# alehdaghi/vq-vae-2-pytorch

Measured on AMD Instinct MI355X. Metric: images/sec VQ-VAE-2 256px train step, higher is better.
Workload: dtype f32; 1 GPU; configs[1]: 256x256 FFHQ-shaped synthetic, default two-level VQ-VAE-2, batch 32/GPU; global_batch=32, image=256, n_embed=512, parallelism=dp1

## Files before the change

include/vq2.h:

```cpp
#ifndef VQ2_H
#define VQ2_H

#include <stddef.h>
#include <stdint.h>

#ifdef __cplusplus
extern "C" {
#endif

#define VQ2_OK 0
#define VQ2_ERR_INVALID 1
#define VQ2_ERR_UNSUPPORTED 2
#define VQ2_ERR_WORKSPACE 3
#define VQ2_ERR_LAUNCH 4

typedef void *vq2_stream_t;

#define VQ2_API_VERSION 6

int vq2_version(void);
const char *vq2_last_error(void);

int vq2_prof_enable(int level);
int vq2_prof_report(char *buf, size_t cap);

typedef struct vq2_conv_desc {
    int32_t N, H, W, Ci;
    int32_t Co;
    int32_t KH, KW, stride, pad;
    int32_t transposed;
    int32_t ldx, ldy;
    int32_t Cir, Cor;
} vq2_conv_desc;

#define VQ2_RELU_IN 1
#define VQ2_RELU_OUT 2

#define VQ2_PACK_FWD 0
#define VQ2_PACK_DGRAD 1
int vq2_pack_weight(const vq2_conv_desc *d, int which, const float *w, float *packed, vq2_stream_t stream);

typedef struct vq2_pack_job {
    const float *w;
    float *packed;
    int64_t offset;
    int64_t numel;
    int32_t Or, Ir, Op, Ip, KH, KW, mode, reserved;
} vq2_pack_job;
int vq2_pack_job_init(const vq2_conv_desc *d, int which, const float *w, float *packed, vq2_pack_job *job);
int vq2_pack_weights_batched(const vq2_pack_job *jobs_dev, int32_t njobs, int64_t total, vq2_stream_t stream);

int vq2_conv_fwd(const vq2_conv_desc *d, int flags, const float *x, const float *wp, const float *bias,
                 const float *residual, int32_t ldres, float *y, vq2_stream_t stream);

int vq2_resblock_supported(int32_t C, int32_t Cm);
int vq2_resblock_fwd(int32_t N, int32_t H, int32_t W, int32_t C, int32_t Cm, int flags, const float *x, int32_t ldx,
                     const float *w1p, const float *b1, const float *w2p, const float *b2, float *r, int32_t ldr,
                     float *y, int32_t ldy, vq2_stream_t stream);

size_t vq2_resblock_w2_workspace_bytes(int32_t N, int32_t H, int32_t W, int32_t C, int32_t Cm);
int vq2_resblock_bwd_data(int32_t N, int32_t H, int32_t W, int32_t C, int32_t Cm, const float *g, int32_t ldg,
                          const float *r, int32_t ldr, const float *x, int32_t ldx, const float *w2d, const float *w1d,
                          float *dh, int32_t lddh, float *dx, int32_t lddx, void *w2_ws, vq2_stream_t stream);

int vq2_conv_dgrad(const vq2_conv_desc *d, const float *dy, const float *wp, const float *mask, int32_t ldmask,
                   const float *residual, int32_t ldres, float *dx, int32_t lddx, vq2_stream_t stream);
#define VQ2_MASK_AFTER_RESIDUAL 4
int vq2_conv_dgrad_ex(const vq2_conv_desc *d, int flags, const float *dy, const float *wp, const float *mask,
                      int32_t ldmask, const float *residual, int32_t ldres, float *dx, int32_t lddx,
                      vq2_stream_t stream);

size_t vq2_conv_wgrad_workspace_bytes(const vq2_conv_desc *d);
int vq2_conv_wgrad(const vq2_conv_desc *d, int flags, const float *x, const float *dy, float *dw, float *db, void *ws,
                   size_t ws_bytes, vq2_stream_t stream);

typedef struct vq2_wgrad_job {
    const float *ws;
    float *dw;
    const float *bias_ws;
    float *db;
    int64_t unit_offset;
    int32_t O, I, Or, Ir, taps, S, n_units_w, n_units_b;
    int32_t swapped;
    int32_t bias_splits;
} vq2_wgrad_job;
int vq2_conv_wgrad_partial(const vq2_conv_desc *d, int flags, const float *x, const float *dy, float *db, void *ws,
                           size_t ws_bytes, vq2_stream_t stream);
int vq2_wgrad_job_init(const vq2_conv_desc *d, const void *ws, float *dw, float *db, vq2_wgrad_job *job);
int vq2_wgrad_reduce_batched(const vq2_wgrad_job *jobs_dev, int32_t njobs, int64_t total_units, vq2_stream_t stream);
int vq2_resblock_w2_job_init(int32_t N, int32_t H, int32_t W, int32_t C, int32_t Cm, const void *ws, float *dw, float *db,
                             vq2_wgrad_job *job);

size_t vq2_colsum_workspace_bytes(int64_t rows, int32_t C);
int vq2_colsum(const float *dy, int64_t rows, int32_t C, int32_t ld, float *db, void *ws, size_t ws_bytes,
               vq2_stream_t stream);

int vq2_nchw_to_nhwc(const float *src, float *dst, int32_t N, int32_t C, int32_t H, int32_t W, int32_t ld,
                     vq2_stream_t stream);
int vq2_nhwc_to_nchw(const float *src, float *dst, int32_t N, int32_t C, int32_t H, int32_t W, int32_t ld,
                     vq2_stream_t stream);

#define VQ2_U8_HWC 0
#define VQ2_U8_CHW 1
int vq2_u8_to_nhwc4(const uint8_t *src, int layout, int32_t N, int32_t C, int32_t Hs, int32_t Ws, int32_t y0,
                    int32_t x0, int32_t H, int32_t W, const float *lut ,
                    float *dst , vq2_stream_t stream);
int vq2_nhwc_to_u8(const float *src, int32_t ld, int32_t N, int32_t C, int32_t H, int32_t W,
                   const float *inv_s , const float *mean , uint8_t *dst, int layout,
                   int32_t Hc, int32_t Wc, int64_t pitch, int32_t cols, int32_t pad, int64_t image_pitch, vq2_stream_t stream);
int vq2_relu_bwd(const float *dy, int32_t lddy, const float *y, int32_t ldy, float *g, int32_t ldg, int64_t pixels,
                 int32_t C, vq2_stream_t stream);
int vq2_slice_copy(const float *src, int32_t lds, float *dst, int32_t ldd, int64_t pixels, int32_t C,
                   int accumulate, vq2_stream_t stream);

int vq2_vq_prepare(const float *embed, float *embedT, float *enorm, int32_t D, int32_t K, vq2_stream_t stream);
size_t vq2_vq_fwd_workspace_floats(int64_t M, int32_t D, int32_t K);
int vq2_vq_fwd(const float *x, int32_t ldx, const float *embed, const float *embedT, const float *enorm, int64_t M,
               int32_t D, int32_t K, int64_t *idx, float *out, int32_t ldo, float *ws, vq2_stream_t stream);
size_t vq2_vq_stats_workspace_bytes(int64_t M, int32_t D, int32_t K);
int vq2_vq_stats(const float *x, int32_t ldx, const int64_t *idx, int64_t M, int32_t D, int32_t K, float *counts,
                 float *sumsT, void *ws, size_t ws_bytes, vq2_stream_t stream);
int vq2_vq_loss(const float *loss_partial, int64_t M, int32_t D, float *diff, vq2_stream_t stream);
int vq2_vq_bwd(const float *g_out, int32_t ldg, const float *g_diff, const float *x, int32_t ldx,
               const int64_t *idx, const float *embedT, int64_t M, int32_t D, int32_t K, float *dx, int32_t lddx,
               vq2_stream_t stream);
int vq2_vq_ema_update(float *embed, float *cluster_size, float *embed_avg, const float *counts, const float *sumsT,
                      int32_t D, int32_t K, double decay, double eps, float *scratch ,
                      vq2_stream_t stream);
int vq2_vq_ema_update_prepare(float *embed, float *cluster_size, float *embed_avg, const float *counts,
                              const float *sumsT, int32_t D, int32_t K, double decay, double eps, float *scratch,
                              float *embedT, float *enorm, vq2_stream_t stream);
int vq2_vq_gather(const int64_t *idx, const float *embedT, int64_t M, int32_t D, int32_t K, float *out, int32_t ldo,
                  vq2_stream_t stream);

int vq2_instnorm_stats(const float *x, int32_t ldx, int32_t N, int64_t HW, int32_t C, double eps, float *mean,
                       float *rstd, vq2_stream_t stream);
int vq2_adain_fwd(const float *x, int32_t ldx, const float *mean, const float *rstd, const float *h, int32_t N,
                  int64_t HW, int32_t C, int flags, float *y, int32_t ldy, vq2_stream_t stream);
int vq2_adain_bwd(const float *dy, int32_t lddy, const float *y, int32_t ldy, const float *x, int32_t ldx,
                  const float *mean, const float *rstd, const float *h, int32_t N, int64_t HW, int32_t C, float *dh,
                  float *dx, int32_t lddx, vq2_stream_t stream);

size_t vq2_mse_workspace_bytes(int64_t numel);
int vq2_mse_fwd_bwd(const float *a, const float *b, int64_t numel, int64_t denom, const float *gscale, float *loss,
                    float *grad, void *ws, size_t ws_bytes, vq2_stream_t stream);
int vq2_stage1_loss(const float *a, const float *b, int64_t numel, int64_t denom, const float *latent, float weight,
                    float *recon, float *total, float *grad, void *ws, size_t ws_bytes, vq2_stream_t stream);
int vq2_adam_step(float *p, const float *g, float *m, float *v, int64_t n, double lr, double beta1, double beta2,
                  double eps, int32_t step, double grad_scale, vq2_stream_t stream);
int vq2_axpby(const float *a, const float *b, float alpha, float *dst, int64_t n, vq2_stream_t stream);
int vq2_scale(const float *src, const float *scalar, float alpha, float *dst, int64_t n, vq2_stream_t stream);

size_t vq2_sse_workspace_bytes(int32_t N, int32_t H, int32_t W, int32_t ld);
int vq2_sse_per_image(const float *a, const float *b, int32_t N, int32_t H, int32_t W, int32_t ld, float *sse, void *ws,
                      size_t ws_bytes, vq2_stream_t stream);
int vq2_index_hist(const int64_t *idx, int64_t M, int32_t K, int64_t *counts, int32_t *flag, vq2_stream_t stream);
int vq2_eval_accumulate(const float *sse, int32_t N, int64_t elems_per_image, const float *diff, double *acc,
                        vq2_stream_t stream);

#define VQ2_COMM_ID_BYTES 128
int vq2_comm_unique_id(void *id);
int vq2_comm_init(const void *id, int32_t rank, int32_t world);
int vq2_comm_world(void);
int vq2_comm_rank(void);
int vq2_comm_allreduce_sum(float *buf, int64_t count, vq2_stream_t stream);
int vq2_comm_broadcast(float *buf, int64_t count, int32_t root, vq2_stream_t stream);
int vq2_comm_destroy(void);

int vq2_debug_mfma_peak(float *scratch, int32_t blocks, int32_t iters, vq2_stream_t stream);
int vq2_debug_mfma_peak16(float *scratch, int32_t blocks, int32_t iters, vq2_stream_t stream);

#ifdef __cplusplus
}
#endif
#endif
```

vq-vae-2-pytorch_amd/_lib.py:

```python
import ctypes as C
import os

_HERE = os.path.dirname(os.path.abspath(__file__))
LIB_PATH = os.environ.get("VQ2_LIB") or os.path.join(_HERE, "libvq2.so")

c_f32p = C.c_void_p
c_stream = C.c_void_p


class ConvDesc(C.Structure):
    _fields_ = [(n, C.c_int32) for n in
                ("N", "H", "W", "Ci", "Co", "KH", "KW", "stride", "pad", "transposed", "ldx", "ldy", "Cir", "Cor")]


class PackJob(C.Structure):
    _fields_ = [("w", C.c_void_p), ("packed", C.c_void_p), ("offset", C.c_int64), ("numel", C.c_int64)] + \
               [(n, C.c_int32) for n in ("Or", "Ir", "Op", "Ip", "KH", "KW", "mode", "reserved")]


class WgradJob(C.Structure):
    _fields_ = [("ws", C.c_void_p), ("dw", C.c_void_p), ("bias_ws", C.c_void_p), ("db", C.c_void_p),
                ("unit_offset", C.c_int64)] + \
               [(n, C.c_int32) for n in ("O", "I", "Or", "Ir", "taps", "S", "n_units_w", "n_units_b", "swapped", "bias_splits")]


def _load():
    if not os.path.exists(LIB_PATH):
        raise ImportError(
            f"{LIB_PATH} not found: build it with `python -c 'import __graft_entry__ as g; g.build()'` "
            "(vq-vae-2-pytorch_amd/csrc/build.sh).  There is no CPU or eager fallback for this path.")
    import torch
    lib = C.CDLL(LIB_PATH)
    P, I32, I64, SZ, F, D = C.c_void_p, C.c_int32, C.c_int64, C.c_size_t, C.c_float, C.c_double
    DP = C.POINTER(ConvDesc)
    sig = {
        "vq2_version": (C.c_int, []),
        "vq2_last_error": (C.c_char_p, []),
        "vq2_prof_enable": (C.c_int, [C.c_int]),
        "vq2_prof_report": (C.c_int, [C.c_char_p, SZ]),
        "vq2_pack_weight": (C.c_int, [DP, C.c_int, P, P, P]),
        "vq2_pack_job_init": (C.c_int, [DP, C.c_int, P, P, C.POINTER(PackJob)]),
        "vq2_pack_weights_batched": (C.c_int, [P, I32, I64, P]),
        "vq2_conv_fwd": (C.c_int, [DP, C.c_int, P, P, P, P, I32, P, P]),
        "vq2_conv_dgrad": (C.c_int, [DP, P, P, P, I32, P, I32, P, I32, P]),
        "vq2_conv_dgrad_ex": (C.c_int, [DP, C.c_int, P, P, P, I32, P, I32, P, I32, P]),
        "vq2_conv_wgrad_workspace_bytes": (SZ, [DP]),
        "vq2_conv_wgrad": (C.c_int, [DP, C.c_int, P, P, P, P, P, SZ, P]),
        "vq2_conv_wgrad_partial": (C.c_int, [DP, C.c_int, P, P, P, P, SZ, P]),
        "vq2_wgrad_job_init": (C.c_int, [DP, P, P, P, C.POINTER(WgradJob)]),
        "vq2_wgrad_reduce_batched": (C.c_int, [P, I32, I64, P]),
        "vq2_colsum_workspace_bytes": (SZ, [I64, I32]),
        "vq2_colsum": (C.c_int, [P, I64, I32, I32, P, P, SZ, P]),
        "vq2_nchw_to_nhwc": (C.c_int, [P, P, I32, I32, I32, I32, I32, P]),
        "vq2_nhwc_to_nchw": (C.c_int, [P, P, I32, I32, I32, I32, I32, P]),
        "vq2_u8_to_nhwc4": (C.c_int, [P, C.c_int, I32, I32, I32, I32, I32, I32, I32, I32, P, P, P]),
        "vq2_nhwc_to_u8": (C.c_int, [P, I32, I32, I32, I32, I32, C.POINTER(F), C.POINTER(F), P, C.c_int, I32, I32, I64, I32,
                                     I32, I64, P]),
        "vq2_sse_workspace_bytes": (SZ, [I32, I32, I32, I32]),
        "vq2_sse_per_image": (C.c_int, [P, P, I32, I32, I32, I32, P, P, SZ, P]),
        "vq2_index_hist": (C.c_int, [P, I64, I32, P, P, P]),
        "vq2_eval_accumulate": (C.c_int, [P, I32, I64, P, P, P]),
        "vq2_relu_bwd": (C.c_int, [P, I32, P, I32, P, I32, I64, I32, P]),
        "vq2_resblock_supported": (C.c_int, [I32, I32]),
        "vq2_resblock_bwd_data": (C.c_int, [I32, I32, I32, I32, I32, P, I32, P, I32, P, I32, P, P, P, I32, P, I32, P, P]),
        "vq2_resblock_w2_workspace_bytes": (SZ, [I32, I32, I32, I32, I32]),
        "vq2_resblock_w2_job_init": (C.c_int, [I32, I32, I32, I32, I32, P, P, P, C.POINTER(WgradJob)]),
        "vq2_resblock_fwd": (C.c_int, [I32, I32, I32, I32, I32, C.c_int, P, I32, P, P, P, P, P, I32, P, I32, P]),
        "vq2_slice_copy": (C.c_int, [P, I32, P, I32, I64, I32, C.c_int, P]),
        "vq2_vq_prepare": (C.c_int, [P, P, P, I32, I32, P]),
        "vq2_vq_fwd_workspace_floats": (SZ, [I64, I32, I32]),
        "vq2_vq_fwd": (C.c_int, [P, I32, P, P, P, I64, I32, I32, P, P, I32, P, P]),
        "vq2_vq_stats_workspace_bytes": (SZ, [I64, I32, I32]),
        "vq2_vq_stats": (C.c_int, [P, I32, P, I64, I32, I32, P, P, P, SZ, P]),
        "vq2_vq_loss": (C.c_int, [P, I64, I32, P, P]),
        "vq2_vq_bwd": (C.c_int, [P, I32, P, P, I32, P, P, I64, I32, I32, P, I32, P]),
        "vq2_vq_ema_update": (C.c_int, [P, P, P, P, P, I32, I32, D, D, P, P]),
        "vq2_vq_ema_update_prepare": (C.c_int, [P, P, P, P, P, I32, I32, D, D, P, P, P, P]),
        "vq2_vq_gather": (C.c_int, [P, P, I64, I32, I32, P, I32, P]),
        "vq2_instnorm_stats": (C.c_int, [P, I32, I32, I64, I32, D, P, P, P]),
        "vq2_adain_fwd": (C.c_int, [P, I32, P, P, P, I32, I64, I32, C.c_int, P, I32, P]),
        "vq2_adain_bwd": (C.c_int, [P, I32, P, I32, P, I32, P, P, P, I32, I64, I32, P, P, I32, P]),
        "vq2_mse_workspace_bytes": (SZ, [I64]),
        "vq2_mse_fwd_bwd": (C.c_int, [P, P, I64, I64, P, P, P, P, SZ, P]),
        "vq2_stage1_loss": (C.c_int, [P, P, I64, I64, P, F, P, P, P, P, SZ, P]),
        "vq2_adam_step": (C.c_int, [P, P, P, P, I64, D, D, D, D, I32, D, P]),
        "vq2_axpby": (C.c_int, [P, P, F, P, I64, P]),
        "vq2_scale": (C.c_int, [P, P, F, P, I64, P]),
        "vq2_comm_unique_id": (C.c_int, [P]),
        "vq2_comm_init": (C.c_int, [P, I32, I32]),
        "vq2_comm_world": (C.c_int, []),
        "vq2_comm_rank": (C.c_int, []),
        "vq2_comm_allreduce_sum": (C.c_int, [P, I64, P]),
        "vq2_comm_broadcast": (C.c_int, [P, I64, I32, P]),
        "vq2_comm_destroy": (C.c_int, []),
        "vq2_debug_mfma_peak": (C.c_int, [P, I32, I32, P]),
        "vq2_debug_mfma_peak16": (C.c_int, [P, I32, I32, P]),
    }
    for name, (res, args) in sig.items():
        fn = getattr(lib, name)
        fn.restype = res
        fn.argtypes = args
    return lib, tuple(sig.keys())


def _header_api_version():
    import re
    hdr = os.path.join(os.path.dirname(_HERE), "include", "vq2.h")
    with open(hdr) as f:
        return int(re.search(r"#define\s+VQ2_API_VERSION\s+(\d+)", f.read()).group(1))


lib, EXPORTS = _load()
API_VERSION = _header_api_version()
if lib.vq2_version() != API_VERSION:
    raise ImportError(f"{LIB_PATH} implements ABI revision {lib.vq2_version()} but include/vq2.h declares "
                      f"{API_VERSION}: rebuild the library (vq-vae-2-pytorch_amd/csrc/build.sh)")


def check(code, what=""):
    if code != 0:
        msg = lib.vq2_last_error().decode(errors="replace")
        raise RuntimeError(f"libvq2 {what} failed (code {code}): {msg}")
```

vq-vae-2-pytorch_amd/csrc/vq2_conv.hip:

```cpp
#include "vq2_conv.h"

namespace vq2 {


template <int WAVES_M, int WAVES_N, int MT, int NT, int BK>
__global__ __launch_bounds__(256, (MT * NT == 4) ? (BK == 16 ? 3 : 2) : 1) void conv_gemm_kernel(const ConvGemmParams P) {
    constexpr int LDK = BK + 4;
    constexpr int BM = WAVES_M * MT * 32;
    constexpr int BN = WAVES_N * NT * 32;
    constexpr int KQ = BK / 4;
    constexpr int RPP = 256 / KQ;
    constexpr int A_LD = BM / RPP;
    constexpr int B_LD = (BN + RPP - 1) / RPP;
    static_assert(BM % RPP == 0 && (BN % RPP == 0 || BN < RPP), "tile vs staging shape");
    static_assert(WAVES_M * WAVES_N == 4, "4 waves per workgroup");
    extern __shared__ __attribute__((aligned(16))) float smem[];
    float *As = smem;
    float *Bs = smem + 2 * BM * LDK;

    const int tid = threadIdx.x;
    const int lane = tid & 63;
    const int wave = tid >> 6;
    const int wm = wave / WAVES_N;
    const int wn = wave % WAVES_N;
    const int ntiles = (P.Co + BN - 1) / BN;
    const int mtiles = (P.M + BM - 1) / BM;
    const int vid = xcd_remap(blockIdx.x, gridDim.x);
    const int n0 = (vid % ntiles) * BN;
    const int m0 = ((vid / ntiles) % mtiles) * BM;
    const int phase = vid / (ntiles * mtiles);

    int pad_h = P.pad_h, pad_w = P.pad_w, oh = 0, ow = 0, os = 1;
    const float *wp = P.w;
    if (P.phases == 4) {
        const int ph = phase >> 1, pw = phase & 1;
        pad_h = 1 - ph; pad_w = 1 - pw; oh = ph; ow = pw; os = 2;
        wp += (size_t)phase * P.Co * P.K;
    }

    const int lrow = tid / KQ;
    const int lk = (tid % KQ) * 4;
    int a_pix[A_LD], a_h[A_LD], a_w[A_LD];
    const int HoWo = P.Ho * P.Wo;
#pragma unroll
    for (int j = 0; j < A_LD; ++j) {
        const int m = m0 + lrow + RPP * j;
        if (m < P.M) {
            const int n = m / HoWo;
            const int r = m - n * HoWo;
            const int ho = r / P.Wo;
            const int wo = r - ho * P.Wo;
            a_h[j] = ho * P.stride - pad_h;
            a_w[j] = wo * P.stride - pad_w;
            a_pix[j] = (n * P.H + a_h[j]) * P.W + a_w[j];
        } else {
            a_h[j] = -(1 << 24); a_w[j] = 0; a_pix[j] = 0;
        }
    }
    int kglob = lk;
    int ci, kh, kw;
    {
        const int tap = kglob / P.Ci;
        ci = kglob - tap * P.Ci;
        kh = tap / P.KW;
        kw = tap - kh * P.KW;
    }

    float4 ra0[A_LD], rb0[B_LD];
    auto load_chunk = [&](float4 (&ra)[A_LD], float4 (&rb)[B_LD]) {
        const bool kv = kglob < P.K;
#pragma unroll
        for (int j = 0; j < A_LD; ++j) {
            const bool v = kv && (unsigned)(a_h[j] + kh) < (unsigned)P.H && (unsigned)(a_w[j] + kw) < (unsigned)P.W;
            float4 val = make_float4(0.f, 0.f, 0.f, 0.f);
            if (v) val = *reinterpret_cast<const float4 *>(P.x + (size_t)(a_pix[j] + kh * P.W + kw) * P.ldx + ci);
            ra[j] = val;
        }
#pragma unroll
        for (int j = 0; j < B_LD; ++j) {
            const int co = n0 + lrow + RPP * j;
            float4 val = make_float4(0.f, 0.f, 0.f, 0.f);
            if (kv && co < P.Co && lrow + RPP * j < BN) val = *reinterpret_cast<const float4 *>(wp + (size_t)co * P.K + kglob);
            rb[j] = val;
        }
    };
    auto advance_k = [&]() {
        kglob += BK;
        ci += BK;
        while (ci >= P.Ci) {
            ci -= P.Ci;
            if (++kw == P.KW) { kw = 0; ++kh; }
        }
    };
    auto store_chunk = [&](int buf, const float4 (&ra)[A_LD], const float4 (&rb)[B_LD]) {
        float *a = As + buf * BM * LDK;
        float *b = Bs + buf * BN * LDK;
#pragma unroll
        for (int j = 0; j < A_LD; ++j)
            *reinterpret_cast<float4 *>(a + (lrow + RPP * j) * LDK + lk) = P.relu_in ? relu4(ra[j]) : ra[j];
#pragma unroll
        for (int j = 0; j < B_LD; ++j)
            if (BN % RPP == 0 || lrow + RPP * j < BN) *reinterpret_cast<float4 *>(b + (lrow + RPP * j) * LDK + lk) = rb[j];
    };

    f32x16 acc[MT][NT];
#pragma unroll
    for (int i = 0; i < MT; ++i)
#pragma unroll
        for (int j = 0; j < NT; ++j)
#pragma unroll
            for (int r = 0; r < 16; ++r) acc[i][j][r] = 0.f;

    const int frag_row = lane & 31;
    const int frag_k = 4 * (lane >> 5);
    auto compute = [&](int buf) {
        const float *a = As + buf * BM * LDK + (wm * MT * 32 + frag_row) * LDK + frag_k;
        const float *b = Bs + buf * BN * LDK + (wn * NT * 32 + frag_row) * LDK + frag_k;
        float4 fa[2][MT], fb[2][NT];
#pragma unroll
        for (int i = 0; i < MT; ++i) fa[0][i] = *reinterpret_cast<const float4 *>(a + i * 32 * LDK);
#pragma unroll
        for (int j = 0; j < NT; ++j) fb[0][j] = *reinterpret_cast<const float4 *>(b + j * 32 * LDK);
#pragma unroll
        for (int k8 = 0; k8 < BK / 8; ++k8) {
            const int cur = k8 & 1, nxt = cur ^ 1;
            if (k8 + 1 < BK / 8) {
#pragma unroll
                for (int i = 0; i < MT; ++i) fa[nxt][i] = *reinterpret_cast<const float4 *>(a + i * 32 * LDK + (k8 + 1) * 8);
#pragma unroll
                for (int j = 0; j < NT; ++j) fb[nxt][j] = *reinterpret_cast<const float4 *>(b + j * 32 * LDK + (k8 + 1) * 8);
            }
#define VQ2_MFMA_STEP(C)                                                                                         \
    _Pragma("unroll") for (int i = 0; i < MT; ++i) _Pragma("unroll") for (int j = 0; j < NT; ++j)                 \
        acc[i][j] = __builtin_amdgcn_mfma_f32_32x32x2f32(fa[cur][i].C, fb[cur][j].C, acc[i][j], 0, 0, 0);
            __builtin_amdgcn_s_setprio(1);
            VQ2_MFMA_STEP(x) VQ2_MFMA_STEP(y) VQ2_MFMA_STEP(z) VQ2_MFMA_STEP(w)
            __builtin_amdgcn_s_setprio(0);
#undef VQ2_MFMA_STEP
        }
    };

    const int nchunks = (P.K + BK - 1) / BK;
    load_chunk(ra0, rb0);
    store_chunk(0, ra0, rb0);
    __syncthreads();
    for (int c = 0; c < nchunks; ++c) {
        const int buf = c & 1;
        if (c + 1 < nchunks) {
            advance_k();
            load_chunk(ra0, rb0);
        }
        compute(buf);
        if (c + 1 < nchunks) store_chunk(buf ^ 1, ra0, rb0);
        __syncthreads();
    }

    const float *__restrict__ maskp = P.mask;
    const float *__restrict__ resp = P.res;
    float *__restrict__ yp = P.y;
    const int colq = lane & 31;
    const int rowq = 4 * (lane >> 5);
#pragma unroll
    for (int j = 0; j < NT; ++j) {
        const int co = n0 + (wn * NT + j) * 32 + colq;
        const bool cv = co < P.Co;
        const float bv = (P.bias && co < P.nbias) ? P.bias[co] : 0.f;
#pragma unroll
        for (int i = 0; i < MT; ++i) {
            const int mb = m0 + (wm * MT + i) * 32 + rowq;
#pragma unroll
            for (int rb = 0; rb < 16; rb += 8) {
                int pix[8];
                bool ok[8];
#pragma unroll
                for (int q = 0; q < 8; ++q) {
                    const int r = rb + q;
                    const int m = mb + (r & 3) + 8 * (r >> 2);
                    ok[q] = cv && m < P.M;
                    if (os == 1) {
                        pix[q] = m;
                    } else {
                        const int n = m / HoWo;
                        const int rr = m - n * HoWo;
                        const int ho = rr / P.Wo;
                        const int wo = rr - ho * P.Wo;
                        pix[q] = (n * P.Hy + (ho * os + oh)) * P.Wy + (wo * os + ow);
                    }
                }
                float mk[8], rs[8];
                if (maskp) {
#pragma unroll
                    for (int q = 0; q < 8; ++q) mk[q] = ok[q] ? maskp[(size_t)pix[q] * P.ldm + co] : 0.f;
                }
                if (resp) {
#pragma unroll
                    for (int q = 0; q < 8; ++q) rs[q] = ok[q] ? resp[(size_t)pix[q] * P.ldr + co] : 0.f;
                }
#pragma unroll
                for (int q = 0; q < 8; ++q) {
                    float v = acc[i][j][rb + q] + bv;
                    if (maskp && !P.mask_after) v = (mk[q] > 0.f) ? v : 0.f;
                    if (resp) v += rs[q];
                    if (maskp && P.mask_after) v = (mk[q] > 0.f) ? v : 0.f;
                    v = relu_floor(v, P.relu_out ? 0 : (int)0x80000000);
                    if (ok[q]) yp[(size_t)pix[q] * P.ldy + co] = v;
                }
            }
        }
    }
}



template <int WAVES_M, int WAVES_N, int MT, int NT, int BK, bool PIPE, bool RELU_IN, bool OCC4 = false, bool UNI = OCC4, bool TAPIN = false>
__global__ __launch_bounds__(256, OCC4 ? 4 : ((MT * NT == 4) ? (BK == 16 ? 3 : 2) : 1)) void conv_gemm_fast_kernel(const ConvGemmParams P) {
    constexpr int LDK = BK + 4;
    constexpr int BM = WAVES_M * MT * 32;
    constexpr int BN = WAVES_N * NT * 32;
    constexpr int KQ = BK / 4;
    constexpr int RPP = 256 / KQ;
    constexpr int A_LD = BM / RPP;
    constexpr int B_LD = (BN + RPP - 1) / RPP;
    static_assert(BM % RPP == 0 && (BN % RPP == 0 || BN < RPP), "tile vs staging shape");
    extern __shared__ __attribute__((aligned(16))) float smem[];
    float *As = smem;
    float *Bs = smem + 2 * BM * LDK;
    int *tap_off = reinterpret_cast<int *>(smem + 2 * (BM + BN) * LDK);
    int *tap_khw = tap_off + 32;

    const int tid = threadIdx.x, lane = tid & 63, wave = tid >> 6;
    const int wm = wave / WAVES_N, wn = wave % WAVES_N;
    const int ntiles = (P.Co + BN - 1) / BN;
    const int mtiles = (P.M + BM - 1) / BM;
    const int vid = xcd_remap(blockIdx.x, gridDim.x);
    const int n0 = (vid % ntiles) * BN;
    const int m0 = ((vid / ntiles) % mtiles) * BM;
    const int phase = vid / (ntiles * mtiles);
    int pad_h = P.pad_h, pad_w = P.pad_w, oh = 0, ow = 0, os = 1;
    const float *wp = P.w;
    if (P.phases == 4) {
        const int ph = phase >> 1, pw = phase & 1;
        pad_h = 1 - ph; pad_w = 1 - pw; oh = ph; ow = pw; os = 2;
        wp += (size_t)phase * P.Co * P.K;
    }
    const int ntaps = P.KH * P.KW;
    if (!OCC4 && tid < ntaps) {
        const int kh = tid / P.KW, kw = tid - kh * P.KW;
        tap_off[tid] = (kh * P.W + kw) * P.ldx * 4;
        tap_khw[tid] = kh | (kw << 8);
    }
    const __amdgpu_buffer_rsrc_t rx =
        __builtin_amdgcn_make_buffer_rsrc(const_cast<float *>(P.x), 0, P.N * P.H * P.W * P.ldx * 4, RSRC_FLAGS);
    const __amdgpu_buffer_rsrc_t rw =
        __builtin_amdgcn_make_buffer_rsrc(const_cast<float *>(wp), 0, P.Co * P.K * 4, RSRC_FLAGS);

    const int lrow = tid / KQ;
    const int lk = (tid % KQ) * 4;
    const int HoWo = P.Ho * P.Wo;
    int a_base[A_LD];
    unsigned a_vw[A_LD];
#pragma unroll
    for (int j = 0; j < A_LD; ++j) {
        const int m = m0 + lrow + RPP * j;
        a_base[j] = 0; a_vw[j] = 0;
        if (m < P.M) {
            const int n = m / HoWo;
            const int r = m - n * HoWo;
            const int ho = r / P.Wo;
            const int wo = r - ho * P.Wo;
            const int hb = ho * P.stride - pad_h, wb = wo * P.stride - pad_w;
            a_base[j] = ((n * P.H + hb) * P.W + wb) * P.ldx * 4;
            unsigned hm = 0, wmk = 0;
            for (int q = 0; q < P.KH; ++q) hm |= ((unsigned)(hb + q) < (unsigned)P.H ? 1u : 0u) << q;
            for (int q = 0; q < P.KW; ++q) wmk |= ((unsigned)(wb + q) < (unsigned)P.W ? 1u : 0u) << q;
            for (int q = 0; q < P.KH; ++q)
                if ((hm >> q) & 1u) a_vw[j] |= wmk << (q * P.KW);
        }
    }
    int b_base[B_LD];
#pragma unroll
    for (int j = 0; j < B_LD; ++j) {
        const int co = n0 + lrow + RPP * j;
        b_base[j] = (co < P.Co && lrow + RPP * j < BN) ? co * P.K * 4 : -1;
    }
    int kglob = lk;
    int tap = kglob / P.Ci;
    int ci = kglob - tap * P.Ci;
    const int tstep = BK / P.Ci, cstep = BK - tstep * P.Ci;
    int u_tap = 0, u_kh = 0, u_kw = 0, u_cb = 0;
    bool b_ok[B_LD];
#pragma unroll
    for (int j = 0; j < B_LD; ++j) b_ok[j] = b_base[j] >= 0;
    int a_pen[A_LD];
    auto refresh_pen = [&]() {
#pragma unroll
        for (int j = 0; j < A_LD; ++j) a_pen[j] = ((a_vw[j] >> u_tap) & 1u) ? 0 : (int)0x80000000;
    };
    if (UNI) {
#pragma unroll
        for (int j = 0; j < A_LD; ++j) a_base[j] += lk * 4;
#pragma unroll
        for (int j = 0; j < B_LD; ++j) b_base[j] = b_ok[j] ? b_base[j] + lk * 4 : (int)0x80000000;
        refresh_pen();
    }
    __syncthreads();

    u32x4 ra[A_LD], rb[B_LD];
    int off_a[A_LD], off_b[B_LD];
    const bool k_aligned = (P.K % BK) == 0;
    auto prep_offsets = [&]() {
        if constexpr (UNI) {
            const int koff_s = ((u_kh * P.W + u_kw) * P.ldx + u_cb) * 4;
            const int kb_s = (u_tap * P.Ci + u_cb) * 4;
#pragma unroll
            for (int j = 0; j < A_LD; ++j) off_a[j] = a_base[j] + koff_s + a_pen[j];
#pragma unroll
            for (int j = 0; j < B_LD; ++j) off_b[j] = b_base[j] + kb_s;
            return;
        }
        const bool kv = k_aligned || tap < ntaps;
        const int tsel = kv ? tap : 0;
        const int koff = tap_off[tsel] + ci * 4;
#pragma unroll
        for (int j = 0; j < A_LD; ++j) {
            const bool v = kv && ((a_vw[j] >> tsel) & 1u) != 0u;
            off_a[j] = v ? a_base[j] + koff : OOB;
        }
#pragma unroll
        for (int j = 0; j < B_LD; ++j) off_b[j] = (kv && b_base[j] >= 0) ? b_base[j] + kglob * 4 : OOB;
    };
    auto issue_loads = [&]() {
#pragma unroll
        for (int j = 0; j < A_LD; ++j) ra[j] = __builtin_amdgcn_raw_buffer_load_b128(rx, off_a[j], 0, 0);
#pragma unroll
        for (int j = 0; j < B_LD; ++j) rb[j] = __builtin_amdgcn_raw_buffer_load_b128(rw, off_b[j], 0, 0);
    };
    auto load_chunk = [&]() { prep_offsets(); issue_loads(); };
    auto advance_k = [&]() {
        if constexpr (UNI) {
            if constexpr (TAPIN) {
                u_cb += BK;
                if ((u_cb & 31) == 0) {
                    u_cb -= 32;
                    ++u_tap;
                    if (++u_kw == P.KW) { u_kw = 0; ++u_kh; }
                    if (u_tap == ntaps) { u_tap = 0; u_kh = 0; u_kw = 0; u_cb += 32; }
                    refresh_pen();
                }
                return;
            }
            u_cb += BK;
            if (u_cb >= P.Ci) {
                u_cb = 0; ++u_tap;
                if (++u_kw == P.KW) { u_kw = 0; ++u_kh; }
                refresh_pen();
            }
            return;
        }
        kglob += BK;
        ci += cstep;
        tap += tstep;
        if (ci >= P.Ci) { ci -= P.Ci; ++tap; }
    };
    auto store_chunk = [&](int buf) {
        float *a = As + buf * BM * LDK;
        float *b = Bs + buf * BN * LDK;
#pragma unroll
        for (int j = 0; j < A_LD; ++j) {
            const float4 v = as_f4(ra[j]);
            *reinterpret_cast<float4 *>(a + (lrow + RPP * j) * LDK + lk) = RELU_IN ? relu4(v) : v;
        }
#pragma unroll
        for (int j = 0; j < B_LD; ++j)
            if (BN % RPP == 0 || lrow + RPP * j < BN) *reinterpret_cast<float4 *>(b + (lrow + RPP * j) * LDK + lk) = as_f4(rb[j]);
    };

    f32x16 acc[MT][NT];
#pragma unroll
    for (int i = 0; i < MT; ++i)
#pragma unroll
        for (int j = 0; j < NT; ++j)
#pragma unroll
            for (int r = 0; r < 16; ++r) acc[i][j][r] = 0.f;

    const int frag_row = lane & 31;
    const int frag_k = 4 * (lane >> 5);
    auto compute = [&](int buf, bool prep_next) {
        const float *a = As + buf * BM * LDK + (wm * MT * 32 + frag_row) * LDK + frag_k;
        const float *b = Bs + buf * BN * LDK + (wn * NT * 32 + frag_row) * LDK + frag_k;
        float4 fa[2][MT], fb[2][NT];
#pragma unroll
        for (int i = 0; i < MT; ++i) fa[0][i] = *reinterpret_cast<const float4 *>(a + i * 32 * LDK);
#pragma unroll
        for (int j = 0; j < NT; ++j) fb[0][j] = *reinterpret_cast<const float4 *>(b + j * 32 * LDK);
#pragma unroll
        for (int k8 = 0; k8 < BK / 8; ++k8) {
            const int cur = k8 & 1, nxt = cur ^ 1;
            if (k8 + 1 < BK / 8) {
#pragma unroll
                for (int i = 0; i < MT; ++i) fa[nxt][i] = *reinterpret_cast<const float4 *>(a + i * 32 * LDK + (k8 + 1) * 8);
#pragma unroll
                for (int j = 0; j < NT; ++j) fb[nxt][j] = *reinterpret_cast<const float4 *>(b + j * 32 * LDK + (k8 + 1) * 8);
            }
#define VQ2_MFMA_STEP(C)                                                                                         \
    _Pragma("unroll") for (int i = 0; i < MT; ++i) _Pragma("unroll") for (int j = 0; j < NT; ++j)                 \
        acc[i][j] = __builtin_amdgcn_mfma_f32_32x32x2f32(fa[cur][i].C, fb[cur][j].C, acc[i][j], 0, 0, 0);
            VQ2_MFMA_STEP(x) VQ2_MFMA_STEP(y) VQ2_MFMA_STEP(z) VQ2_MFMA_STEP(w)
#undef VQ2_MFMA_STEP
            if (PIPE && k8 == 0 && prep_next) { advance_k(); prep_offsets(); }
        }
    };

    const int nchunks = (P.K + BK - 1) / BK;
    load_chunk();
    store_chunk(0);
    __syncthreads();
    if constexpr (PIPE) {
        if (nchunks > 1) { advance_k(); prep_offsets(); }
        for (int c = 0; c < nchunks; ++c) {
            const int buf = c & 1;
            if (c + 1 < nchunks) issue_loads();
            compute(buf, c + 2 < nchunks);
            if (c + 1 < nchunks) store_chunk(buf ^ 1);
            __syncthreads();
        }
    } else {
        for (int c = 0; c < nchunks; ++c) {
            const int buf = c & 1;
            if (c + 1 < nchunks) {
                advance_k();
                load_chunk();
            }
            compute(buf, false);
            if (c + 1 < nchunks) store_chunk(buf ^ 1);
            __syncthreads();
        }
    }

    const int ybytes = P.N * P.Hy * P.Wy * 4;
    const __amdgpu_buffer_rsrc_t ry = __builtin_amdgcn_make_buffer_rsrc(P.y, 0, ybytes * P.ldy, RSRC_FLAGS);
    const __amdgpu_buffer_rsrc_t rmk =
        __builtin_amdgcn_make_buffer_rsrc(const_cast<float *>(P.mask ? P.mask : P.y), 0, P.mask ? ybytes * P.ldm : 0, RSRC_FLAGS);
    const __amdgpu_buffer_rsrc_t rrs =
        __builtin_amdgcn_make_buffer_rsrc(const_cast<float *>(P.res ? P.res : P.y), 0, P.res ? ybytes * P.ldr : 0, RSRC_FLAGS);
    const bool has_mask = P.mask != nullptr, has_res = P.res != nullptr;
    const bool mask_first = has_mask && !P.mask_after, mask_last = has_mask && P.mask_after;
    const int colq = lane & 31;
    const int rowq = 4 * (lane >> 5);
    const int ldy4 = P.ldy * 4, ldm4 = P.ldm * 4, ldr4 = P.ldr * 4;
#pragma unroll
    for (int i = 0; i < MT; ++i) {
        const int mt0 = m0 + (wm * MT + i) * 32;
        int pix_lane;
        {
            const int m = mt0 + colq;
            if (os == 1) {
                pix_lane = m;
            } else {
                const int n = m / HoWo;
                const int rr = m - n * HoWo;
                const int ho = rr / P.Wo;
                const int wo = rr - ho * P.Wo;
                pix_lane = (n * P.Hy + (ho * 2 + oh)) * P.Wy + (wo * 2 + ow);
            }
            if (m >= P.M) pix_lane = -1;
        }
#pragma unroll
        for (int j = 0; j < NT; ++j) {
            const int co = n0 + (wn * NT + j) * 32 + colq;
            const bool cv = co < P.Co;
            const float bv = (P.bias && co < P.nbias) ? P.bias[co] : 0.f;
            const int co4 = co * 4;
#pragma unroll
            for (int rb8 = 0; rb8 < 16; rb8 += 8) {
                int pix[8];
                float mk[8], rs[8];
#pragma unroll
                for (int q = 0; q < 8; ++q) {
                    const int r = rb8 + q;
                    const int rr = rowq + (r & 3) + 8 * (r >> 2);
                    pix[q] = (os == 1) ? ((mt0 + rr < P.M) ? mt0 + rr : -1) : __shfl(pix_lane, rr, 64);
                    if (!cv) pix[q] = -1;
                }
                if (has_mask) {
#pragma unroll
                    for (int q = 0; q < 8; ++q)
                        mk[q] = __uint_as_float(__builtin_amdgcn_raw_buffer_load_b32(rmk, pix[q] >= 0 ? pix[q] * ldm4 + co4 : OOB, 0, 0));
                }
                if (has_res) {
#pragma unroll
                    for (int q = 0; q < 8; ++q)
                        rs[q] = __uint_as_float(__builtin_amdgcn_raw_buffer_load_b32(rrs, pix[q] >= 0 ? pix[q] * ldr4 + co4 : OOB, 0, 0));
                }
#pragma unroll
                for (int q = 0; q < 8; ++q) {
                    float v = acc[i][j][rb8 + q] + bv;
                    if (mask_first) v = (mk[q] > 0.f) ? v : 0.f;
                    if (has_res) v += rs[q];
                    if (mask_last) v = (mk[q] > 0.f) ? v : 0.f;
                    v = relu_floor(v, P.relu_out ? 0 : (int)0x80000000);
                    __builtin_amdgcn_raw_buffer_store_b32(__float_as_uint(v), ry, pix[q] >= 0 ? pix[q] * ldy4 + co4 : OOB, 0, 0);
                }
            }
        }
    }
}

template <int WAVES_M, int WAVES_N, int MT, int NT, int BK, bool OCC4 = false>
static int launch_conv_gemm_fast(const ConvGemmParams &P, hipStream_t s) {
    constexpr int BM = WAVES_M * MT * 32, BN = WAVES_N * NT * 32;
    const size_t lds = (size_t)2 * (BM + BN) * (BK + 4) * sizeof(float) + (OCC4 ? 0 : 64 * sizeof(int));
    const unsigned nwg = ((P.M + BM - 1) / BM) * ((P.Co + BN - 1) / BN) * P.phases;
    const long gib = 1L << 30;
    const bool small = (long)P.N * P.H * P.W * P.ldx * 4 < gib && (long)P.Co * P.K * P.phases * 4 < gib;
    const bool uni = small && (OCC4 || (P.Ci % BK == 0 && P.K % BK == 0));
    const bool tap_inner = uni && P.KH * P.KW > 1 && P.Ci > 32 && P.Ci % 32 == 0;
    auto kern = P.relu_in ? (uni ? (tap_inner ? conv_gemm_fast_kernel<WAVES_M, WAVES_N, MT, NT, BK, true, true, OCC4, true, true>
                                              : conv_gemm_fast_kernel<WAVES_M, WAVES_N, MT, NT, BK, true, true, OCC4, true, false>)
                                 : conv_gemm_fast_kernel<WAVES_M, WAVES_N, MT, NT, BK, true, true, OCC4, OCC4>)
                          : (uni ? (tap_inner ? conv_gemm_fast_kernel<WAVES_M, WAVES_N, MT, NT, BK, true, false, OCC4, true, true>
                                              : conv_gemm_fast_kernel<WAVES_M, WAVES_N, MT, NT, BK, true, false, OCC4, true, false>)
                                 : conv_gemm_fast_kernel<WAVES_M, WAVES_N, MT, NT, BK, true, false, OCC4, OCC4>);
    allow_big_lds(kern, lds);
    dim3 grid(nwg);
    const char *name = "conv_gemm";
    if (prof_enabled())
        name = prof_label("conv_gemm<%dx%dx%d>|M=%d,N=%d,K=%d,k%d,s%d,ph%d,%s", BM, BN, BK, P.M, P.Co, P.K, P.KH, P.stride,
                          P.phases, tap_inner ? "tap" : uni ? "uni" : "var");
    ProfScope prof(name, P.flops, P.bytes, s, BM == 128 && BN == 128);
    hipLaunchKernelGGL(kern, grid, dim3(256), lds, s, P);
    return check_launch("conv_gemm_fast_kernel");
}

template <int WAVES_M, int WAVES_N, int MT, int NT, int BK>
static int launch_conv_gemm(const ConvGemmParams &P, hipStream_t s) {
    constexpr int BM = WAVES_M * MT * 32, BN = WAVES_N * NT * 32;
    const size_t lds = (size_t)2 * (BM + BN) * (BK + 4) * sizeof(float);
    auto kern = conv_gemm_kernel<WAVES_M, WAVES_N, MT, NT, BK>;
    allow_big_lds(kern, lds);
    dim3 grid(((P.M + BM - 1) / BM) * ((P.Co + BN - 1) / BN) * P.phases);
    const char *name = "conv_gemm";
    if (prof_enabled())
        name = prof_label("conv_gemm<%dx%dx%d>|M=%d,N=%d,K=%d,k%d,s%d,ph%d,gen", BM, BN, BK, P.M, P.Co, P.K, P.KH, P.stride,
                          P.phases);
    ProfScope prof(name, P.flops, P.bytes, s, BM == 128 && BN == 128 && BK == 32);
    hipLaunchKernelGGL(kern, grid, dim3(256), lds, s, P);
    return check_launch("conv_gemm_kernel");
}

namespace sp {
constexpr int TH = 8, TW = 16, PW = TW + 2, NPATCH = (TH + 2) * PW;
constexpr int CS = 16, LDK = CS + 4;
constexpr int A_F4 = NPATCH * CS / 4;
constexpr int A_FLOATS = NPATCH * LDK;
constexpr int B_ROWS = 4 * 64;
constexpr int B_FLOATS = B_ROWS * LDK;
constexpr size_t LDS_BYTES = (size_t)2 * (A_FLOATS + B_FLOATS) * sizeof(float);
constexpr int SOOB = 0x7F000000;
}

template <bool RELU_IN>
__global__ __launch_bounds__(256, 2) void subpixel_conv_kernel(const ConvGemmParams P) {
    using namespace sp;
    constexpr int A_LD = (A_F4 + 255) / 256;
    extern __shared__ __attribute__((aligned(16))) float smem[];
    float *As = smem;
    float *Bs = smem + 2 * A_FLOATS;
    const int tid = threadIdx.x, lane = tid & 63, wq = tid >> 6;
    const int l31 = lane & 31, fk = 4 * (lane >> 5), rowq = 4 * (lane >> 5);
    const int ncg = P.Co / 64;
    const int tiles_x = (P.W + TW - 1) / TW, tiles_y = (P.H + TH - 1) / TH;
    const int tiles = tiles_x * tiles_y;
    const int vid = xcd_remap(blockIdx.x, gridDim.x);
    const int cg = vid % ncg;
    const int tv = vid / ncg;
    const int n = tv / tiles;
    const int t = tv - n * tiles;
    const int tyi = t / tiles_x;
    const int y0 = tyi * TH, x0 = (t - tyi * tiles_x) * TW;
    const __amdgpu_buffer_rsrc_t rx =
        __builtin_amdgcn_make_buffer_rsrc(const_cast<float *>(P.x), 0, P.N * P.H * P.W * P.ldx * 4, RSRC_FLAGS);
    const __amdgpu_buffer_rsrc_t rw =
        __builtin_amdgcn_make_buffer_rsrc(const_cast<float *>(P.w), 0, 4 * P.Co * P.K * 4, RSRC_FLAGS);

    int a_off[A_LD], b_off[4];
#pragma unroll
    for (int j = 0; j < A_LD; ++j) {
        const int f = tid + 256 * j;
        a_off[j] = SOOB;
        if (f < A_F4) {
            const int pp = f >> 2;
            const int pr = pp / PW, pc = pp - pr * PW;
            const int gy = y0 - 1 + pr, gx = x0 - 1 + pc;
            if ((unsigned)gy < (unsigned)P.H && (unsigned)gx < (unsigned)P.W)
                a_off[j] = ((n * P.H + gy) * P.W + gx) * P.ldx * 4 + (f & 3) * 16;
        }
    }
#pragma unroll
    for (int j = 0; j < 4; ++j) {
        const int row = (tid >> 2) + 64 * j;
        b_off[j] = ((cg * 64 + (row & 63)) * P.K + (row >> 6) * P.Ci) * 4 + (tid & 3) * 16;
    }
    const int st_off = (tid >> 2) * LDK + (tid & 3) * 4;
    const int phase_stride = P.Co * P.K * 4;
    u32x4 ra[A_LD], rb[4];
    auto issue_a = [&](int s) {
#pragma unroll
        for (int j = 0; j < A_LD; ++j) ra[j] = __builtin_amdgcn_raw_buffer_load_b128(rx, a_off[j], s * CS * 4, 0);
    };
    auto issue_b = [&](int s, int ph) {
#pragma unroll
        for (int j = 0; j < 4; ++j) rb[j] = __builtin_amdgcn_raw_buffer_load_b128(rw, b_off[j], ph * phase_stride + s * CS * 4, 0);
    };
    auto store_a = [&](int buf) {
        float *a = As + buf * A_FLOATS + st_off;
#pragma unroll
        for (int j = 0; j < A_LD; ++j)
            if ((j + 1) * 256 <= A_F4 || tid + 256 * j < A_F4) {
                const float4 v = as_f4(ra[j]);
                *reinterpret_cast<float4 *>(a + j * 64 * LDK) = RELU_IN ? relu4(v) : v;
            }
    };
    auto store_b = [&](int buf) {
        float *b = Bs + buf * B_FLOATS + st_off;
#pragma unroll
        for (int j = 0; j < 4; ++j) *reinterpret_cast<float4 *>(b + j * 64 * LDK) = as_f4(rb[j]);
    };

    f32x16 acc[4][2];
#pragma unroll
    for (int p = 0; p < 4; ++p)
#pragma unroll
        for (int j = 0; j < 2; ++j)
#pragma unroll
            for (int r = 0; r < 16; ++r) acc[p][j][r] = 0.f;

    const int txr = l31 < 16 ? l31 : ((l31 + 14) & 15);
    const int a_frag = ((2 * wq + (l31 >> 4)) * PW + txr) * LDK + fk;
    const int b_frag = l31 * LDK + fk;
    const int NS = P.Ci / CS;

    issue_a(0);
    issue_b(0, 0);
    store_a(0);
    store_b(0);
    __syncthreads();
    for (int s = 0; s < NS; ++s) {
        const float *Ab = As + (s & 1) * A_FLOATS + a_frag;
#pragma unroll
        for (int p = 0; p < 4; ++p) {
            const bool last = (s + 1 == NS) && p == 3;
            if (!last) issue_b(p == 3 ? s + 1 : s, (p + 1) & 3);
            if (p == 0 && s + 1 < NS) issue_a(s + 1);
            __builtin_amdgcn_sched_barrier(0);
            {
                const float *Bb = Bs + (p & 1) * B_FLOATS + b_frag;
#pragma unroll
                for (int tap = 0; tap < 4; ++tap) {
                    const float *a = Ab + (((p >> 1) + (tap >> 1)) * PW + (p & 1) + (tap & 1)) * LDK;
                    const float *b = Bb + tap * 64 * LDK;
#pragma unroll
                    for (int k8 = 0; k8 < CS / 8; ++k8) {
                        const float4 fa = *reinterpret_cast<const float4 *>(a + 8 * k8);
#pragma unroll
                        for (int j = 0; j < 2; ++j) {
                            const float4 fb = *reinterpret_cast<const float4 *>(b + j * 32 * LDK + 8 * k8);
                            acc[p][j] = __builtin_amdgcn_mfma_f32_32x32x2f32(fa.x, fb.x, acc[p][j], 0, 0, 0);
                            acc[p][j] = __builtin_amdgcn_mfma_f32_32x32x2f32(fa.y, fb.y, acc[p][j], 0, 0, 0);
                            acc[p][j] = __builtin_amdgcn_mfma_f32_32x32x2f32(fa.z, fb.z, acc[p][j], 0, 0, 0);
                            acc[p][j] = __builtin_amdgcn_mfma_f32_32x32x2f32(fa.w, fb.w, acc[p][j], 0, 0, 0);
                        }
                    }
                }
            }
            __builtin_amdgcn_sched_barrier(0);
            if (!last) store_b((p + 1) & 1);
            if (p == 3 && s + 1 < NS) store_a((s + 1) & 1);
            __syncthreads();
        }
    }

    const int ybytes = P.N * P.Hy * P.Wy * 4;
    const __amdgpu_buffer_rsrc_t ry = __builtin_amdgcn_make_buffer_rsrc(P.y, 0, ybytes * P.ldy, RSRC_FLAGS);
    const __amdgpu_buffer_rsrc_t rmk =
        __builtin_amdgcn_make_buffer_rsrc(const_cast<float *>(P.mask ? P.mask : P.y), 0, P.mask ? ybytes * P.ldm : 0, RSRC_FLAGS);
    const __amdgpu_buffer_rsrc_t rrs =
        __builtin_amdgcn_make_buffer_rsrc(const_cast<float *>(P.res ? P.res : P.y), 0, P.res ? ybytes * P.ldr : 0, RSRC_FLAGS);
    const bool has_mask = P.mask != nullptr, has_res = P.res != nullptr;
    const bool mask_first = has_mask && !P.mask_after, mask_last = has_mask && P.mask_after;
    int pb_lane;
    {
        const int gy = y0 + 2 * wq + (l31 >> 4), gx = x0 + txr;
        pb_lane = (gy < P.H && gx < P.W) ? (n * P.Hy + 2 * gy) * P.Wy + 2 * gx : -1;
    }
    const int ldy4 = P.ldy * 4, ldm4 = P.ldm * 4, ldr4 = P.ldr * 4;
#pragma unroll
    for (int rb8 = 0; rb8 < 16; rb8 += 8) {
        int pb[8];
#pragma unroll
        for (int q = 0; q < 8; ++q) {
            const int r = rb8 + q;
            pb[q] = __shfl(pb_lane, rowq + (r & 3) + 8 * (r >> 2), 64);
        }
#pragma unroll
        for (int p = 0; p < 4; ++p) {
            const int poff = (p >> 1) * P.Wy + (p & 1);
#pragma unroll
            for (int j = 0; j < 2; ++j) {
                const int co = cg * 64 + j * 32 + l31;
                const float bv = (P.bias && co < P.nbias) ? P.bias[co] : 0.f;
                const int co4 = co * 4;
                float mk[8], rs[8];
                if (has_mask) {
#pragma unroll
                    for (int q = 0; q < 8; ++q)
                        mk[q] = __uint_as_float(__builtin_amdgcn_raw_buffer_load_b32(rmk, pb[q] >= 0 ? (pb[q] + poff) * ldm4 + co4 : SOOB, 0, 0));
                }
                if (has_res) {
#pragma unroll
                    for (int q = 0; q < 8; ++q)
                        rs[q] = __uint_as_float(__builtin_amdgcn_raw_buffer_load_b32(rrs, pb[q] >= 0 ? (pb[q] + poff) * ldr4 + co4 : SOOB, 0, 0));
                }
#pragma unroll
                for (int q = 0; q < 8; ++q) {
                    float v = acc[p][j][rb8 + q] + bv;
                    if (mask_first) v = (mk[q] > 0.f) ? v : 0.f;
                    if (has_res) v += rs[q];
                    if (mask_last) v = (mk[q] > 0.f) ? v : 0.f;
                    v = relu_floor(v, P.relu_out ? 0 : (int)0x80000000);
                    __builtin_amdgcn_raw_buffer_store_b32(__float_as_uint(v), ry, pb[q] >= 0 ? (pb[q] + poff) * ldy4 + co4 : SOOB, 0, 0);
                }
            }
        }
    }
}

static int launch_subpixel(const ConvGemmParams &P, hipStream_t s) {
    const int tiles = ((P.W + sp::TW - 1) / sp::TW) * ((P.H + sp::TH - 1) / sp::TH);
    dim3 grid(P.N * tiles * (P.Co / 64));
    const char *name = "subpixel_conv";
    if (prof_enabled()) name = prof_label("subpixel_conv|M=%d,N=%d,K=%d,ph4", P.M, P.Co, P.K);
    ProfScope prof(name, P.flops, P.bytes, s);
    auto kern = P.relu_in ? subpixel_conv_kernel<true> : subpixel_conv_kernel<false>;
    allow_big_lds(kern, sp::LDS_BYTES);
    hipLaunchKernelGGL(kern, grid, dim3(256), sp::LDS_BYTES, s, P);
    return check_launch("subpixel_conv_kernel");
}

namespace c4 {
constexpr int TH = 8, TW = 16;
constexpr int PH = 2 * TH + 2, PW = 2 * TW + 2;
constexpr int NP = PH * PW;
constexpr int P_LD = (NP + 255) / 256;
constexpr int COOB = 0x7F000000;
}

template <bool HAS_MASK, bool C4>
__global__ __launch_bounds__(256, 3) void conv_k4s2_c4_kernel(const ConvGemmParams P) {
    using namespace c4;
    __shared__ float4 patch[NP];
    const int tid = threadIdx.x, lane = tid & 63, wq = tid >> 6;
    const int l31 = lane & 31, h = lane >> 5;
    const int tiles_x = (P.Wo + TW - 1) / TW, tiles_y = (P.Ho + TH - 1) / TH;
    const int tiles = tiles_x * tiles_y, total = P.N * tiles;
    const __amdgpu_buffer_rsrc_t rx = __builtin_amdgcn_make_buffer_rsrc(const_cast<float *>(P.x), 0, P.N * P.H * P.W * P.ldx * 4, RSRC_FLAGS);
    const __amdgpu_buffer_rsrc_t rw = __builtin_amdgcn_make_buffer_rsrc(const_cast<float *>(P.w), 0, 64 * 64 * 4, RSRC_FLAGS);
    const int ybytes = P.N * P.Ho * P.Wo * 4;
    const __amdgpu_buffer_rsrc_t ry = __builtin_amdgcn_make_buffer_rsrc(P.y, 0, ybytes * P.ldy, RSRC_FLAGS);
    const __amdgpu_buffer_rsrc_t rmk = __builtin_amdgcn_make_buffer_rsrc(const_cast<float *>(HAS_MASK ? P.mask : P.y), 0,
                                                                         HAS_MASK ? ybytes * P.ldm : 0, RSRC_FLAGS);
    float4 wf[2][8];
#pragma unroll
    for (int j = 0; j < 2; ++j)
#pragma unroll
        for (int k8 = 0; k8 < 8; ++k8)
            wf[j][k8] = as_f4(__builtin_amdgcn_raw_buffer_load_b128(rw, ((j * 32 + l31) * 64 + 8 * k8 + 4 * h) * 4, 0, 0));
    __shared__ __attribute__((aligned(16))) float bias_s[64];
    if (tid < 64) bias_s[tid] = (P.bias && tid < P.nbias) ? P.bias[tid] : 0.f;
    const bool relu_in = P.relu_in != 0;
    u32x4 pr[P_LD];
    auto tile_of = [&](int v, int &n, int &y0, int &x0) {
        n = v / tiles;
        const int t = v - n * tiles;
        const int tyi = t / tiles_x;
        y0 = tyi * TH; x0 = (t - tyi * tiles_x) * TW;
    };
    auto issue_patch = [&](int v) {
        int n, y0, x0;
        tile_of(v, n, y0, x0);
#pragma unroll
        for (int q = 0; q < P_LD; ++q) {
            const int f = tid + 256 * q;
            const int prow = f / PW, pcol = f - prow * PW;
            const int gy = 2 * y0 - 1 + prow, gx = 2 * x0 - 1 + pcol;
            const bool ok = v < total && f < NP && (unsigned)gy < (unsigned)P.H && (unsigned)gx < (unsigned)P.W;
            pr[q] = __builtin_amdgcn_raw_buffer_load_b128(rx, ok ? ((n * P.H + gy) * P.W + gx) * P.ldx * 4 : COOB, 0, 0);
        }
    };
    auto store_patch = [&]() {
#pragma unroll
        for (int q = 0; q < P_LD; ++q) {
            const int f = tid + 256 * q;
            if (f < NP) patch[f] = relu_in ? relu4(as_f4(pr[q])) : as_f4(pr[q]);
        }
    };
    const int TPW = P.c4_tpw;
    const int v0 = xcd_remap(blockIdx.x, gridDim.x) * TPW;
    issue_patch(v0);
    const int ty = 2 * wq + (l31 >> 4), tx = l31 & 15;
    for (int it = 0; it < TPW; ++it) {
        const int v = v0 + it;
        if (v >= total) break;
        store_patch();
        __syncthreads();
        if (it + 1 < TPW) issue_patch(v + 1);
        int n, y0, x0;
        tile_of(v, n, y0, x0);
        f32x16 acc[2];
#pragma unroll
        for (int j = 0; j < 2; ++j)
#pragma unroll
            for (int r = 0; r < 16; ++r) acc[j][r] = 0.f;
        u32x4 mk[2][4];
        if (HAS_MASK) {
            const int oy = y0 + ty, ox = x0 + tx;
            const bool pv = oy < P.Ho && ox < P.Wo;
            const int pix = (n * P.Ho + oy) * P.Wo + ox;
#pragma unroll
            for (int j = 0; j < 2; ++j)
#pragma unroll
                for (int g = 0; g < 4; ++g)
                    mk[j][g] = __builtin_amdgcn_raw_buffer_load_b128(rmk, pv ? pix * P.ldm * 4 + (32 * j + 8 * g + 4 * h) * 4 : COOB, 0, 0);
            __builtin_amdgcn_sched_barrier(0);
        }
#pragma unroll
        for (int k8 = 0; k8 < 8; ++k8) {
            const float4 a = patch[(2 * ty + (k8 >> 1)) * PW + 2 * tx + 2 * (k8 & 1) + h];
#pragma unroll
            for (int j = 0; j < 2; ++j) {
                if (HAS_MASK) {
                    acc[j] = __builtin_amdgcn_mfma_f32_32x32x2f32(wf[j][k8].x, a.x, acc[j], 0, 0, 0);
                    acc[j] = __builtin_amdgcn_mfma_f32_32x32x2f32(wf[j][k8].y, a.y, acc[j], 0, 0, 0);
                    acc[j] = __builtin_amdgcn_mfma_f32_32x32x2f32(wf[j][k8].z, a.z, acc[j], 0, 0, 0);
                    if (C4) acc[j] = __builtin_amdgcn_mfma_f32_32x32x2f32(wf[j][k8].w, a.w, acc[j], 0, 0, 0);
                } else {
                    acc[j] = __builtin_amdgcn_mfma_f32_32x32x2f32(a.x, wf[j][k8].x, acc[j], 0, 0, 0);
                    acc[j] = __builtin_amdgcn_mfma_f32_32x32x2f32(a.y, wf[j][k8].y, acc[j], 0, 0, 0);
                    acc[j] = __builtin_amdgcn_mfma_f32_32x32x2f32(a.z, wf[j][k8].z, acc[j], 0, 0, 0);
                    if (C4) acc[j] = __builtin_amdgcn_mfma_f32_32x32x2f32(a.w, wf[j][k8].w, acc[j], 0, 0, 0);
                }
            }
        }
        const int relu_floor_bits = P.relu_out ? 0 : (int)0x80000000;
        if (HAS_MASK) {
            const int oy = y0 + ty, ox = x0 + tx;
            const bool pv = oy < P.Ho && ox < P.Wo;
            const int pix = (n * P.Ho + oy) * P.Wo + ox;
#pragma unroll
            for (int j = 0; j < 2; ++j)
#pragma unroll
                for (int g = 0; g < 4; ++g) {
                    const int co4 = (32 * j + 8 * g + 4 * h) * 4;
                    const float4 bv = *reinterpret_cast<const float4 *>(bias_s + 32 * j + 8 * g + 4 * h);
                    float4 o = make_float4(acc[j][4 * g] + bv.x, acc[j][4 * g + 1] + bv.y, acc[j][4 * g + 2] + bv.z,
                                           acc[j][4 * g + 3] + bv.w);
                    if (HAS_MASK) {
                        const float4 m = as_f4(mk[j][g]);
                        o.x = m.x > 0.f ? o.x : 0.f; o.y = m.y > 0.f ? o.y : 0.f; o.z = m.z > 0.f ? o.z : 0.f; o.w = m.w > 0.f ? o.w : 0.f;
                    }
                    o.x = relu_floor(o.x, relu_floor_bits); o.y = relu_floor(o.y, relu_floor_bits);
                    o.z = relu_floor(o.z, relu_floor_bits); o.w = relu_floor(o.w, relu_floor_bits);
                    u32x4 u;
                    u.x = __float_as_uint(o.x); u.y = __float_as_uint(o.y); u.z = __float_as_uint(o.z); u.w = __float_as_uint(o.w);
                    __builtin_amdgcn_raw_buffer_store_b128(u, ry, pv ? pix * P.ldy * 4 + co4 : COOB, 0, 0);
                }
        } else {
#pragma unroll
            for (int r = 0; r < 16; ++r) {
                const int pp = 4 * h + (r & 3) + 8 * (r >> 2);
                const int oy = y0 + 2 * wq + (pp >> 4), ox = x0 + (pp & 15);
                const bool pv = oy < P.Ho && ox < P.Wo;
                const int pix = (n * P.Ho + oy) * P.Wo + ox;
#pragma unroll
                for (int j = 0; j < 2; ++j) {
                    const int co4 = (32 * j + l31) * 4;
                    float v = acc[j][r] + bias_s[32 * j + l31];
                    if (HAS_MASK) {
                        const float m = __uint_as_float(__builtin_amdgcn_raw_buffer_load_b32(rmk, pv ? pix * P.ldm * 4 + co4 : COOB, 0, 0));
                        v = m > 0.f ? v : 0.f;
                    }
                    v = relu_floor(v, relu_floor_bits);
                    __builtin_amdgcn_raw_buffer_store_b32(__float_as_uint(v), ry, pv ? pix * P.ldy * 4 + co4 : COOB, 0, 0);
                }
            }
        }
        __syncthreads();
    }
}

namespace k64 {
constexpr int KC = 64, LDW = KC + 4;
constexpr int X_FLOATS = 32 * LDW;
constexpr int NWAVES = 8;
template <int NB> constexpr size_t lds_bytes() { return (size_t)(NB * 32 * LDW + NWAVES * X_FLOATS) * sizeof(float); }
}

template <int NB, bool RELU_IN>
__global__ __launch_bounds__(512, 2) void conv1x1_k64_kernel(const ConvGemmParams P) {
    using namespace k64;
    extern __shared__ __attribute__((aligned(16))) float smem[];
    float *Ws = smem;
    const int tid = threadIdx.x, lane = tid & 63, wave = tid >> 6;
    float *Xs = smem + NB * 32 * LDW + wave * X_FLOATS;

    const __amdgpu_buffer_rsrc_t rx =
        __builtin_amdgcn_make_buffer_rsrc(const_cast<float *>(P.x), 0, P.M * P.ldx * 4, RSRC_FLAGS);
    const __amdgpu_buffer_rsrc_t rw =
        __builtin_amdgcn_make_buffer_rsrc(const_cast<float *>(P.w), 0, P.Co * KC * 4, RSRC_FLAGS);
    for (int it = tid; it < NB * 32 * 16; it += 64 * NWAVES) {
        const u32x4 v = __builtin_amdgcn_raw_buffer_load_b128(rw, it * 16, 0, 0);
        *reinterpret_cast<float4 *>(Ws + (it >> 4) * LDW + (it & 15) * 4) = as_f4(v);
    }
    const int nblk = (P.M + 31) / 32, gw = blockIdx.x * NWAVES + wave, nwaves = gridDim.x * NWAVES;
    const int srow = lane >> 4, sq = lane & 15;
    u32x4 rx8[8];
    auto load_block = [&](int b) {
#pragma unroll
        for (int j = 0; j < 8; ++j) {
            const int m = b * 32 + srow + 4 * j;
            rx8[j] = __builtin_amdgcn_raw_buffer_load_b128(rx, (b < nblk && m < P.M) ? (m * P.ldx + 4 * sq) * 4 : OOB, 0, 0);
        }
    };
    auto store_block = [&](float *xs) {
#pragma unroll
        for (int j = 0; j < 8; ++j) {
            const float4 v = as_f4(rx8[j]);
            *reinterpret_cast<float4 *>(xs + (srow + 4 * j) * LDW + 4 * sq) = RELU_IN ? relu4(v) : v;
        }
    };
    const int ybytes = P.M * 4;
    const __amdgpu_buffer_rsrc_t ry = __builtin_amdgcn_make_buffer_rsrc(P.y, 0, ybytes * P.ldy, RSRC_FLAGS);
    const __amdgpu_buffer_rsrc_t rmk =
        __builtin_amdgcn_make_buffer_rsrc(const_cast<float *>(P.mask ? P.mask : P.y), 0, P.mask ? ybytes * P.ldm : 0, RSRC_FLAGS);
    const __amdgpu_buffer_rsrc_t rrs =
        __builtin_amdgcn_make_buffer_rsrc(const_cast<float *>(P.res ? P.res : P.y), 0, P.res ? ybytes * P.ldr : 0, RSRC_FLAGS);
    const bool has_mask = P.mask != nullptr, has_res = P.res != nullptr;
    const bool mask_first = has_mask && !P.mask_after, mask_last = has_mask && P.mask_after;
    const int colq = lane & 31, rowq = 4 * (lane >> 5), fk = 4 * (lane >> 5);
    const int ldy4 = P.ldy * 4, ldm4 = P.ldm * 4, ldr4 = P.ldr * 4;
    const int relu_bits = P.relu_out ? 0 : (int)0x80000000;
    float bv[NB];
#pragma unroll
    for (int j = 0; j < NB; ++j) bv[j] = (P.bias && j * 32 + colq < P.nbias) ? P.bias[j * 32 + colq] : 0.f;

    load_block(gw);
    __syncthreads();
    for (int b = gw; b < nblk; b += nwaves) {
        float *xs = Xs;
        store_block(xs);
        load_block(b + nwaves);
        f32x16 acc[NB];
#pragma unroll
        for (int j = 0; j < NB; ++j)
#pragma unroll
            for (int r = 0; r < 16; ++r) acc[j][r] = 0.f;
        const float *a = xs + colq * LDW + fk;
        const float *w = Ws + colq * LDW + fk;
#pragma unroll
        for (int k8 = 0; k8 < KC / 8; ++k8) {
            const float4 fa = *reinterpret_cast<const float4 *>(a + 8 * k8);
#pragma unroll
            for (int j = 0; j < NB; ++j) {
                const float4 fb = *reinterpret_cast<const float4 *>(w + j * 32 * LDW + 8 * k8);
                acc[j] = __builtin_amdgcn_mfma_f32_32x32x2f32(fa.x, fb.x, acc[j], 0, 0, 0);
                acc[j] = __builtin_amdgcn_mfma_f32_32x32x2f32(fa.y, fb.y, acc[j], 0, 0, 0);
                acc[j] = __builtin_amdgcn_mfma_f32_32x32x2f32(fa.z, fb.z, acc[j], 0, 0, 0);
                acc[j] = __builtin_amdgcn_mfma_f32_32x32x2f32(fa.w, fb.w, acc[j], 0, 0, 0);
            }
        }
        const int m0 = b * 32;
#pragma unroll
        for (int j = 0; j < NB; ++j) {
            const int co4 = (j * 32 + colq) * 4;
#pragma unroll
            for (int rb8 = 0; rb8 < 16; rb8 += 8) {
                int pix[8];
                float mk[8], rs[8];
#pragma unroll
                for (int q = 0; q < 8; ++q) {
                    const int r = rb8 + q;
                    const int m = m0 + rowq + (r & 3) + 8 * (r >> 2);
                    pix[q] = m < P.M ? m : -1;
                }
                if (has_mask) {
#pragma unroll
                    for (int q = 0; q < 8; ++q)
                        mk[q] = __uint_as_float(__builtin_amdgcn_raw_buffer_load_b32(rmk, pix[q] >= 0 ? pix[q] * ldm4 + co4 : OOB, 0, 0));
                }
                if (has_res) {
#pragma unroll
                    for (int q = 0; q < 8; ++q)
                        rs[q] = __uint_as_float(__builtin_amdgcn_raw_buffer_load_b32(rrs, pix[q] >= 0 ? pix[q] * ldr4 + co4 : OOB, 0, 0));
                }
#pragma unroll
                for (int q = 0; q < 8; ++q) {
                    float v = acc[j][rb8 + q] + bv[j];
                    if (mask_first) v = (mk[q] > 0.f) ? v : 0.f;
                    if (has_res) v += rs[q];
                    if (mask_last) v = (mk[q] > 0.f) ? v : 0.f;
                    v = relu_floor(v, relu_bits);
                    __builtin_amdgcn_raw_buffer_store_b32(__float_as_uint(v), ry, pix[q] >= 0 ? pix[q] * ldy4 + co4 : OOB, 0, 0);
                }
            }
        }
    }
}

static bool conv_k64_ok(const ConvGemmParams &P) {
    const long gib = 1L << 30;
    return P.phases == 1 && P.KH == 1 && P.KW == 1 && P.stride == 1 && P.pad_h == 0 && P.pad_w == 0 && P.Ci == 64 &&
           P.K == 64 && P.Co % 32 == 0 && P.Co >= 64 && P.Co <= 192 && P.M >= 16384 && P.ldx % 4 == 0 &&
           (long)P.M * P.ldx * 4 < gib && (long)P.M * P.ldy * 4 < gib && (long)P.M * (P.ldm > P.ldr ? P.ldm : P.ldr) * 4 < gib;
}

template <int NB>
static int launch_conv_k64_nb(const ConvGemmParams &P, hipStream_t s) {
    auto kern = P.relu_in ? conv1x1_k64_kernel<NB, true> : conv1x1_k64_kernel<NB, false>;
    const size_t lds = k64::lds_bytes<NB>();
    allow_big_lds(kern, lds);
    const int nblk = (P.M + 31) / 32;
    int grid = 256;
    if (grid * k64::NWAVES > nblk) grid = (nblk + k64::NWAVES - 1) / k64::NWAVES;
    const char *name = "conv1x1_k64";
    if (prof_enabled()) name = prof_label("conv1x1_k64|M=%d,N=%d,K=64", P.M, P.Co);
    ProfScope prof(name, P.flops, P.bytes, s);
    hipLaunchKernelGGL(kern, dim3(grid), dim3(64 * k64::NWAVES), lds, s, P);
    return check_launch("conv1x1_k64_kernel");
}

static int launch_conv_k64(const ConvGemmParams &P, hipStream_t s) {
    switch (P.Co / 32) {
        case 2: return launch_conv_k64_nb<2>(P, s);
        case 3: return launch_conv_k64_nb<3>(P, s);
        case 4: return launch_conv_k64_nb<4>(P, s);
        case 5: return launch_conv_k64_nb<5>(P, s);
        default: return launch_conv_k64_nb<6>(P, s);
    }
}

static bool conv_c4_ok(const ConvGemmParams &P) {
    const long big = 0x7F000000L / 4;
    return P.phases == 1 && P.KH == 4 && P.KW == 4 && P.stride == 2 && P.pad_h == 1 && P.pad_w == 1 && P.Ci == 4 &&
           P.Co == 64 && !P.res && P.H % 2 == 0 && P.W % 2 == 0 && P.ldy % 4 == 0 && (!P.mask || P.ldm % 4 == 0) &&
           (long)P.N * P.H * P.W * P.ldx < big && (long)P.N * P.Ho * P.Wo * (P.ldy > P.ldm ? P.ldy : P.ldm) < big &&
           (reinterpret_cast<uintptr_t>(P.y) & 15u) == 0 && (!P.mask || (reinterpret_cast<uintptr_t>(P.mask) & 15u) == 0);
}

static int launch_conv_c4(const ConvGemmParams &P, hipStream_t s) {
    const int tiles = ((P.Wo + c4::TW - 1) / c4::TW) * ((P.Ho + c4::TH - 1) / c4::TH) * P.N;
    const char *name = "conv_k4s2_c4";
    if (prof_enabled()) name = prof_label("conv_k4s2_c4|M=%d,N=%d,K=%d%s", P.M, P.Co, P.K, P.mask ? ",mask" : "");
    ProfScope prof(name, P.flops, P.bytes, s);
    const bool c4 = !(P.ci_real > 0 && P.ci_real <= 3);
    auto kern = P.mask ? (c4 ? conv_k4s2_c4_kernel<true, true> : conv_k4s2_c4_kernel<true, false>)
                       : (c4 ? conv_k4s2_c4_kernel<false, true> : conv_k4s2_c4_kernel<false, false>);
    ConvGemmParams Q = P;
    Q.c4_tpw = P.mask ? 8 : 4;
    hipLaunchKernelGGL(kern, dim3((tiles + Q.c4_tpw - 1) / Q.c4_tpw), dim3(256), 0, s, Q);
    return check_launch("conv_k4s2_c4_kernel");
}

static int run_conv_gemm(const ConvGemmParams &P, hipStream_t s) {
    const long wgs128 = (long)((P.M + 127) / 128) * ((P.Co + 127) / 128) * P.phases;
    const long lim = (1L << 29);
    const bool fast_ok = forms() > FORMS_GENERAL && P.KH * P.KW <= 32 && (long)P.N * P.H * P.W * P.ldx < lim &&
                         (long)P.N * P.Hy * P.Wy * P.ldy < lim && (long)P.N * P.Hy * P.Wy * (P.ldm > P.ldr ? P.ldm : P.ldr) < lim &&
                         (long)P.Co * P.K * P.phases < lim;
    if (fast_ok && conv_c4_ok(P)) return launch_conv_c4(P, s);
    if (fast_ok && conv_k64_ok(P)) return launch_conv_k64(P, s);
    if (fast_ok && wino3_ok(P)) return launch_wino3(P, s);
    const long big = 0x7F000000L / 4;
    const long sp_wgs = (long)P.N * ((P.W + sp::TW - 1) / sp::TW) * ((P.H + sp::TH - 1) / sp::TH) * (P.Co / 64);
    if (fast_ok && P.phases == 4 && P.Co % 64 == 0 && P.Ci % 16 == 0 && P.K == 4 * P.Ci &&
        (sp_wgs >= 512 || P.K >= 512) &&
        (long)P.N * P.H * P.W * P.ldx < big && (long)P.N * P.Hy * P.Wy * P.ldy < big &&
        (long)P.N * P.Hy * P.Wy * (P.ldm > P.ldr ? P.ldm : P.ldr) < big)
        return launch_subpixel(P, s);
    if (fast_ok) {
        if (wgs128 < 400 && P.Co > 32) {
            if (P.Co > 64) return launch_conv_gemm_fast<2, 2, 1, 2, 32>(P, s);
            return launch_conv_gemm_fast<2, 2, 1, 1, 32>(P, s);
        }
        if (P.Co > 64) {
            if (P.K <= 64) {
                if (P.Co > 128 && P.Co <= 192) return launch_conv_gemm_fast<2, 2, 1, 3, 16>(P, s);
                return launch_conv_gemm_fast<2, 2, 1, 2, 16>(P, s);
            }
            const bool below_gib = (long)P.N * P.H * P.W * P.ldx * 4 < (1L << 30) && (long)P.Co * P.K * P.phases * 4 < (1L << 30);
            if (P.Ci % 16 == 0 && below_gib && wgs128 > 512 && wgs128 <= 1024) return launch_conv_gemm_fast<2, 2, 2, 2, 16, true>(P, s);
            return launch_conv_gemm_fast<2, 2, 2, 2, 32>(P, s);
        }
        if (P.Co > 32) return launch_conv_gemm_fast<2, 2, 2, 1, 16>(P, s);
        return launch_conv_gemm_fast<4, 1, 1, 1, 32>(P, s);
    }
    if (wgs128 < 400 && P.Co > 32) {
        if (P.Co > 64) return launch_conv_gemm<2, 2, 1, 2, 16>(P, s);
        return launch_conv_gemm<2, 2, 1, 1, 16>(P, s);
    }
    if (P.Co > 64) return launch_conv_gemm<2, 2, 2, 2, 32>(P, s);
    if (P.Co > 32) return launch_conv_gemm<2, 2, 2, 1, 16>(P, s);
    return launch_conv_gemm<4, 1, 1, 1, 16>(P, s);
}

typedef float f32x4m __attribute__((ext_vector_type(4)));
namespace ctm {
constexpr int TH = 16, TW = 32, PW = TW + 2, NP = (TH + 2) * PW;
constexpr int CS = 8, LD = CS + 4;
constexpr int X_FLOATS = NP * LD, W_FLOATS = 64 * LD;
constexpr size_t LDS_BYTES = (size_t)2 * (X_FLOATS + W_FLOATS) * sizeof(float);
constexpr int COOB = 0x7F000000;
}

__global__ __launch_bounds__(256, 2) void convT_small_mfma_kernel(const float *__restrict__ x, int ldx,
                                                                  const float *__restrict__ wk,
                                                                  const float *__restrict__ bias, int nbias,
                                                                  float *__restrict__ y, int ldy, int N, int H, int W, int Ci,
                                                                  int relu_in) {
    using namespace ctm;
    extern __shared__ __attribute__((aligned(16))) float smem[];
    float *Xs = smem;
    float *Ws = smem + 2 * X_FLOATS;
    const int tid = threadIdx.x, lane = tid & 63, wq = tid >> 6;
    const int tiles_x = (W + TW - 1) / TW, tiles_y = (H + TH - 1) / TH;
    const int vid = xcd_remap(blockIdx.x, gridDim.x);
    const int n = vid / (tiles_x * tiles_y);
    const int tt = vid - n * tiles_x * tiles_y;
    const int i0 = (tt / tiles_x) * TH, j0 = (tt % tiles_x) * TW;
    const __amdgpu_buffer_rsrc_t rx = __builtin_amdgcn_make_buffer_rsrc(const_cast<float *>(x), 0, N * H * W * ldx * 4, RSRC_FLAGS);
    const __amdgpu_buffer_rsrc_t rw = __builtin_amdgcn_make_buffer_rsrc(const_cast<float *>(wk), 0, 64 * Ci * 4, RSRC_FLAGS);

    constexpr int QPR = CS / 4;
    constexpr int X_F4 = NP * QPR;
    constexpr int X_LD = (X_F4 + 255) / 256;
    int x_off[X_LD];
#pragma unroll
    for (int j = 0; j < X_LD; ++j) {
        const int f = tid + 256 * j;
        x_off[j] = COOB;
        if (f < X_F4) {
            const int pp = f / QPR;
            const int gi = i0 - 1 + pp / PW, gj = j0 - 1 + pp % PW;
            if ((unsigned)gi < (unsigned)H && (unsigned)gj < (unsigned)W) x_off[j] = ((n * H + gi) * W + gj) * ldx * 4 + (f % QPR) * 16;
        }
    }
    const bool w_act = tid < 64 * QPR;
    const int w_off = w_act ? (tid / QPR) * Ci * 4 + (tid % QPR) * 16 : COOB;
    const int st_off = (tid / QPR) * LD + (tid % QPR) * 4;
    u32x4 rxv[X_LD], rwv;
    auto issue = [&](int s) {
#pragma unroll
        for (int j = 0; j < X_LD; ++j) rxv[j] = __builtin_amdgcn_raw_buffer_load_b128(rx, x_off[j], s * CS * 4, 0);
        rwv = __builtin_amdgcn_raw_buffer_load_b128(rw, w_off, s * CS * 4, 0);
    };
    auto store = [&](int buf) {
        float *xs = Xs + buf * X_FLOATS + st_off;
#pragma unroll
        for (int j = 0; j < X_LD; ++j)
            if ((j + 1) * 256 <= X_F4 || tid + 256 * j < X_F4) {
                const float4 v = as_f4(rxv[j]);
                *reinterpret_cast<float4 *>(xs + j * (256 / QPR) * LD) = relu_in ? relu4(v) : v;
            }
        if (w_act) *reinterpret_cast<float4 *>(Ws + buf * W_FLOATS + st_off) = as_f4(rwv);
    };

    f32x4m acc[2][4];
#pragma unroll
    for (int u = 0; u < 2; ++u)
#pragma unroll
        for (int p = 0; p < 4; ++p) acc[u][p] = f32x4m{0.f, 0.f, 0.f, 0.f};
    const int a_base = ((4 * wq + (lane >> 5)) * PW + (lane & 31)) * LD;
    const int b_base = (lane & 3) * LD;
    const int NS = Ci / CS;
    issue(0);
    store(0);
    __syncthreads();
    for (int s = 0; s < NS; ++s) {
        const int buf = s & 1;
        if (s + 1 < NS) issue(s + 1);
        __builtin_amdgcn_sched_barrier(0);
        const float *xs = Xs + buf * X_FLOATS + a_base;
        const float *ws = Ws + buf * W_FLOATS + b_base;
#pragma unroll
        for (int kq = 0; kq < QPR; ++kq) {
            float4 av[2][9];
#pragma unroll
            for (int u = 0; u < 2; ++u)
#pragma unroll
                for (int nb = 0; nb < 9; ++nb)
                    av[u][nb] = *reinterpret_cast<const float4 *>(xs + ((2 * u + nb / 3) * PW + nb % 3) * LD + kq * 4);
#pragma unroll
            for (int ph = 0; ph < 2; ++ph)
#pragma unroll
                for (int pw = 0; pw < 2; ++pw)
#pragma unroll
                    for (int a = 0; a < 2; ++a)
#pragma unroll
                        for (int b = 0; b < 2; ++b) {
                            const int tap = (3 - 2 * a - ph) * 4 + (3 - 2 * b - pw);
                            const float4 bv = *reinterpret_cast<const float4 *>(ws + tap * 4 * LD + kq * 4);
#pragma unroll
                            for (int u = 0; u < 2; ++u) {
                                const float4 xv = av[u][(ph + a) * 3 + pw + b];
                                f32x4m c = acc[u][ph * 2 + pw];
                                c = __builtin_amdgcn_mfma_f32_4x4x1f32(xv.x, bv.x, c, 0, 0, 0);
                                c = __builtin_amdgcn_mfma_f32_4x4x1f32(xv.y, bv.y, c, 0, 0, 0);
                                c = __builtin_amdgcn_mfma_f32_4x4x1f32(xv.z, bv.z, c, 0, 0, 0);
                                c = __builtin_amdgcn_mfma_f32_4x4x1f32(xv.w, bv.w, c, 0, 0, 0);
                                acc[u][ph * 2 + pw] = c;
                            }
                        }
        }
        __builtin_amdgcn_sched_barrier(0);
        if (s + 1 < NS) store(buf ^ 1);
        __syncthreads();
    }
    const __amdgpu_buffer_rsrc_t ry = __builtin_amdgcn_make_buffer_rsrc(y, 0, N * 4 * H * W * ldy * 4, RSRC_FLAGS);
    const int co = lane & 3;
    const float bvs = (bias && co < nbias) ? bias[co] : 0.f;
#pragma unroll
    for (int u = 0; u < 2; ++u)
#pragma unroll
        for (int r = 0; r < 4; ++r) {
            const int pos = (lane & ~3) + r;
            const int gi = i0 + 4 * wq + 2 * u + (pos >> 5), gj = j0 + (pos & 31);
            const bool ok = gi < H && gj < W;
#pragma unroll
            for (int p = 0; p < 4; ++p) {
                const int pix = (n * 2 * H + 2 * gi + (p >> 1)) * (2 * W) + 2 * gj + (p & 1);
                __builtin_amdgcn_raw_buffer_store_b32(__float_as_uint(acc[u][p][r] + bvs), ry, ok ? (pix * ldy + co) * 4 : COOB, 0, 0);
            }
        }
}

static bool use_convT_small(const vq2_conv_desc *d) {
    return d->transposed && d->Co == 4 && d->Cor >= 1 && d->Cor <= 3 && d->Ci % 16 == 0;
}

static int check_desc(const vq2_conv_desc *d) {
    VQ2_REQUIRE(d != nullptr, "conv desc is null");
    if (int e = check_forms()) return e;
    VQ2_REQUIRE(d->N > 0 && d->H > 0 && d->W > 0 && d->Ci > 0 && d->Co > 0, "conv desc: non-positive dims");
    VQ2_REQUIRE(d->Ci % 4 == 0 && d->Co % 4 == 0, "conv desc: Ci=%d, Co=%d must be multiples of 4", d->Ci, d->Co);
    VQ2_REQUIRE(d->ldx >= d->Ci && d->ldx % 4 == 0, "conv desc: ldx=%d must be >= Ci and a multiple of 4", d->ldx);
    VQ2_REQUIRE(d->ldy >= d->Co && d->ldy % 4 == 0, "conv desc: ldy=%d must be >= Co and a multiple of 4", d->ldy);
    VQ2_REQUIRE(d->Cir >= 0 && d->Cir <= d->Ci && d->Cor >= 0 && d->Cor <= d->Co, "conv desc: Cir/Cor out of range");
    if (d->transposed) {
        VQ2_REQUIRE(d->KH == 4 && d->KW == 4 && d->stride == 2 && d->pad == 1,
                    "conv-transpose supports k4 s2 p1 only (vqvae.py:150-160,191-193)");
    } else {
        VQ2_REQUIRE(d->KH >= 1 && d->KH <= 7 && d->KW == d->KH, "conv: square kernel 1..7 required");
        VQ2_REQUIRE(d->stride == 1 || d->stride == 2, "conv: stride 1 or 2");
        VQ2_REQUIRE(d->pad >= 0 && d->pad < d->KH, "conv: 0 <= pad < KH");
        VQ2_REQUIRE(d->H + 2 * d->pad >= d->KH && d->W + 2 * d->pad >= d->KW, "conv: kernel larger than padded input");
        if (d->stride == 2) VQ2_REQUIRE(d->KH == 4 && d->pad == 1 && d->H % 2 == 0 && d->W % 2 == 0,
                                        "stride-2 conv supports k4 p1 on even sizes (vqvae.py:105,107,114)");
    }
    int Ho, Wo;
    if (d->transposed) { Ho = 2 * d->H; Wo = 2 * d->W; }
    else { Ho = (d->H + 2 * d->pad - d->KH) / d->stride + 1; Wo = (d->W + 2 * d->pad - d->KW) / d->stride + 1; }
    const int64_t lim = (int64_t)1 << 31;
    VQ2_REQUIRE((int64_t)d->N * d->H * d->W * d->ldx < lim && (int64_t)d->N * Ho * Wo * d->ldy < lim,
                "conv: tensor exceeds 2^31 elements (int32 indexing)");
    return VQ2_OK;
}

static void out_dims(const vq2_conv_desc *d, int &Ho, int &Wo) {
    if (d->transposed) { Ho = 2 * d->H; Wo = 2 * d->W; }
    else { Ho = (d->H + 2 * d->pad - d->KH) / d->stride + 1; Wo = (d->W + 2 * d->pad - d->KW) / d->stride + 1; }
}

}

using namespace vq2;

static int pack_job_of(const vq2_conv_desc *d, int which, vq2_pack_job *j) {
    const int cir = d->Cir ? d->Cir : d->Ci, cor = d->Cor ? d->Cor : d->Co;
    j->KH = d->KH; j->KW = d->KW;
    if (which == VQ2_PACK_FWD && use_convT_small(d)) {
        j->mode = 3; j->Or = d->Ci; j->Ir = cor; j->Op = d->Ci; j->Ip = 4;
    } else if (!d->transposed) {
        j->Or = cor; j->Ir = cir; j->Op = d->Co; j->Ip = d->Ci;
        j->mode = (which == VQ2_PACK_FWD) ? 0 : ((d->stride == 1) ? 1 : 2);
    } else {
        j->Or = cir; j->Ir = cor; j->Op = d->Ci; j->Ip = d->Co;
        j->mode = (which == VQ2_PACK_FWD) ? 2 : 0;
    }
    j->numel = (int64_t)j->Op * j->Ip * j->KH * j->KW;
    return VQ2_OK;
}

__device__ __forceinline__ float pack_elem(const float *__restrict__ w, int t, int Or, int Ir, int Op, int Ip, int KH,
                                           int KW, int mode) {
    const int taps = KH * KW;
    int o, i, kh, kw;
    if (mode == 0) {
        i = t % Ip; const int tap = (t / Ip) % taps; o = t / (Ip * taps);
        kh = tap / KW; kw = tap % KW;
    } else if (mode == 1) {
        o = t % Op; const int tapf = (t / Op) % taps; i = t / (Op * taps);
        kh = KH - 1 - tapf / KW; kw = KW - 1 - tapf % KW;
    } else if (mode == 2) {
        o = t % Op; const int ab = (t / Op) % 4; i = (t / (Op * 4)) % Ip; const int phase = t / (Op * 4 * Ip);
        kh = 3 - 2 * (ab >> 1) - (phase >> 1); kw = 3 - 2 * (ab & 1) - (phase & 1);
    } else {
        o = t % Op; i = (t / Op) % 4; const int tap = t / (4 * Op);
        kh = tap / 4; kw = tap % 4;
    }
    return (o < Or && i < Ir) ? w[((o * Ir + i) * KH + kh) * KW + kw] : 0.f;
}

__global__ __launch_bounds__(256) void pack_batched_kernel(const vq2_pack_job *__restrict__ jobs, int njobs, int64_t total) {
    for (int64_t g = (int64_t)blockIdx.x * 256 + threadIdx.x; g < total; g += (int64_t)gridDim.x * 256) {
        int lo = 0, hi = njobs - 1;
        while (lo < hi) {
            const int mid = (lo + hi + 1) >> 1;
            if (jobs[mid].offset <= g) lo = mid; else hi = mid - 1;
        }
        const vq2_pack_job j = jobs[lo];
        const int t = (int)(g - j.offset);
        j.packed[t] = pack_elem(j.w, t, j.Or, j.Ir, j.Op, j.Ip, j.KH, j.KW, j.mode);
    }
}

extern "C" int vq2_pack_job_init(const vq2_conv_desc *d, int which, const float *w, float *packed, vq2_pack_job *job) {
    if (int e = check_desc(d)) return e;
    VQ2_REQUIRE(w && packed && job, "pack_job_init: null pointer");
    VQ2_REQUIRE(which == VQ2_PACK_FWD || which == VQ2_PACK_DGRAD, "pack_job_init: bad `which`");
    job->w = w; job->packed = packed; job->offset = 0;
    return pack_job_of(d, which, job);
}

extern "C" int vq2_pack_weights_batched(const vq2_pack_job *jobs_dev, int32_t njobs, int64_t total, vq2_stream_t stream) {
    VQ2_REQUIRE(jobs_dev && njobs > 0 && total > 0, "pack_weights_batched: bad arguments");
    const int64_t b = (total + 255) / 256;
    hipLaunchKernelGGL(pack_batched_kernel, dim3((unsigned)(b > 2048 ? 2048 : b)), dim3(256), 0, to_stream(stream), jobs_dev,
                       njobs, total);
    return check_launch("pack_batched_kernel");
}

__global__ void pack_single_kernel(const float *__restrict__ w, float *__restrict__ p, int Or, int Ir, int Op, int Ip,
                                   int KH, int KW, int mode, int total) {
    for (int t = blockIdx.x * blockDim.x + threadIdx.x; t < total; t += gridDim.x * blockDim.x)
        p[t] = pack_elem(w, t, Or, Ir, Op, Ip, KH, KW, mode);
}

extern "C" int vq2_pack_weight(const vq2_conv_desc *d, int which, const float *w, float *packed, vq2_stream_t stream) {
    vq2_pack_job j;
    if (int e = vq2_pack_job_init(d, which, w, packed, &j)) return e;
    const int total = (int)j.numel;
    const int blocks = (total + 255) / 256 < 1024 ? (total + 255) / 256 : 1024;
    hipLaunchKernelGGL(pack_single_kernel, dim3(blocks), dim3(256), 0, to_stream(stream), w, packed, j.Or, j.Ir, j.Op, j.Ip,
                       j.KH, j.KW, j.mode, total);
    return check_launch("pack_single_kernel");
}

extern "C" int vq2_conv_fwd(const vq2_conv_desc *d, int flags, const float *x, const float *wp, const float *bias,
                            const float *residual, int32_t ldres, float *y, vq2_stream_t stream) {
    if (int e = check_desc(d)) return e;
    VQ2_REQUIRE(x && wp && y, "conv_fwd: null pointer");
    VQ2_REQUIRE(aligned16(x) && aligned16(wp) && aligned16(y), "conv_fwd: pointers must be 16-byte aligned");
    VQ2_REQUIRE(!residual || (ldres >= d->Co), "conv_fwd: ldres < Co");
    if (use_convT_small(d)) {
        if (residual || (flags & VQ2_RELU_OUT) || d->N > 65535)
            return set_error(VQ2_ERR_UNSUPPORTED, "conv_fwd: a conv-transpose to <= 3 channels takes neither a residual nor "
                             "ReLU-out, and at most 65535 images per launch (split the batch)");
        if (!((double)d->N * 4 * d->H * d->W * d->ldy * 4 < (double)ctm::COOB && (double)d->N * d->H * d->W * d->ldx * 4 < (double)ctm::COOB))
            return set_error(VQ2_ERR_UNSUPPORTED, "conv_fwd: a conv-transpose to <= 4 channels is limited to tensors below %d bytes "
                             "(split the batch)", ctm::COOB);
        hipStream_t s = to_stream(stream);
        const int cor = d->Cor ? d->Cor : d->Co;
        const char *name = "convT_small";
        if (prof_enabled()) name = prof_label("convT_small|N=%d,H=%d,W=%d,Ci=%d", d->N, d->H, d->W, d->Ci);
        ProfScope prof(name, 2.0 * d->N * d->H * d->W * 16.0 * d->Ci * cor,
                       4.0 * ((double)d->N * d->H * d->W * d->Ci + 4.0 * d->N * d->H * d->W * cor), s);
        const int g = ((d->W + ctm::TW - 1) / ctm::TW) * ((d->H + ctm::TH - 1) / ctm::TH) * d->N;
        allow_big_lds(convT_small_mfma_kernel, ctm::LDS_BYTES);
        hipLaunchKernelGGL(convT_small_mfma_kernel, dim3(g), dim3(256), ctm::LDS_BYTES, s, x, d->ldx, wp, bias, cor, y,
                           d->ldy, d->N, d->H, d->W, d->Ci, (flags & VQ2_RELU_IN) != 0);
        return check_launch("convT_small_mfma_kernel");
    }
    ConvGemmParams P{};
    P.x = x; P.w = wp; P.bias = bias; P.mask = nullptr; P.res = residual; P.y = y;
    P.N = d->N; P.H = d->H; P.W = d->W; P.Ci = d->Ci; P.ldx = d->ldx;
    P.Co = d->Co; P.ldy = d->ldy; P.ldr = ldres; P.ldm = 0;
    P.relu_in = (flags & VQ2_RELU_IN) != 0; P.relu_out = (flags & VQ2_RELU_OUT) != 0;
    P.nbias = d->Cor ? d->Cor : d->Co;
    P.ci_real = d->Cir ? d->Cir : d->Ci;
    out_dims(d, P.Hy, P.Wy);
    if (!d->transposed) {
        P.KH = d->KH; P.KW = d->KW; P.stride = d->stride; P.pad_h = P.pad_w = d->pad;
        P.Ho = P.Hy; P.Wo = P.Wy; P.phases = 1;
    } else {
        P.KH = 2; P.KW = 2; P.stride = 1; P.pad_h = P.pad_w = 1;
        P.Ho = d->H; P.Wo = d->W; P.phases = 4;
    }
    P.K = P.KH * P.KW * P.Ci; P.M = P.N * P.Ho * P.Wo;
    {
        const double cir = d->Cir ? d->Cir : d->Ci, cor = d->Cor ? d->Cor : d->Co;
        const double pix_in = (double)d->N * d->H * d->W, pix_out = (double)d->N * P.Hy * P.Wy;
        const double macs = d->transposed ? pix_in * 16.0 * cir * cor : pix_out * d->KH * d->KW * cir * cor;
        P.flops = 2.0 * macs;
        P.bytes = 4.0 * (pix_in * cir + pix_out * cor * (residual ? 2.0 : 1.0) + cir * cor * d->KH * d->KW);
    }
    return run_conv_gemm(P, to_stream(stream));
}

extern "C" int vq2_conv_dgrad(const vq2_conv_desc *d, const float *dy, const float *wp, const float *mask,
                              int32_t ldmask, const float *residual, int32_t ldres, float *dx, int32_t lddx,
                              vq2_stream_t stream) {
    return vq2_conv_dgrad_ex(d, 0, dy, wp, mask, ldmask, residual, ldres, dx, lddx, stream);
}

extern "C" int vq2_conv_dgrad_ex(const vq2_conv_desc *d, int flags, const float *dy, const float *wp, const float *mask,
                                 int32_t ldmask, const float *residual, int32_t ldres, float *dx, int32_t lddx,
                                 vq2_stream_t stream) {
    if (int e = check_desc(d)) return e;
    VQ2_REQUIRE((flags & ~VQ2_MASK_AFTER_RESIDUAL) == 0, "conv_dgrad: unknown flag");
    VQ2_REQUIRE(dy && wp && dx, "conv_dgrad: null pointer");
    VQ2_REQUIRE(aligned16(dy) && aligned16(wp) && aligned16(dx), "conv_dgrad: pointers must be 16-byte aligned");
    VQ2_REQUIRE(lddx >= d->Ci && lddx % 4 == 0, "conv_dgrad: lddx=%d must be >= Ci and a multiple of 4", lddx);
    VQ2_REQUIRE((!mask || ldmask >= d->Ci) && (!residual || ldres >= d->Ci), "conv_dgrad: ldmask/ldres < Ci");
    int Hy, Wy;
    out_dims(d, Hy, Wy);
    ConvGemmParams P{};
    P.x = dy; P.w = wp; P.bias = nullptr; P.mask = mask; P.res = residual; P.y = dx;
    P.N = d->N; P.H = Hy; P.W = Wy; P.Ci = d->Co; P.ldx = d->ldy;
    P.Co = d->Ci; P.ldy = lddx; P.ldm = ldmask; P.ldr = ldres;
    P.relu_in = 0; P.relu_out = 0;
    P.ci_real = d->Cor ? d->Cor : d->Co;
    P.mask_after = (flags & VQ2_MASK_AFTER_RESIDUAL) != 0;
    P.Hy = d->H; P.Wy = d->W;
    if (!d->transposed && d->stride == 1) {
        P.KH = d->KH; P.KW = d->KW; P.stride = 1; P.pad_h = P.pad_w = d->KH - 1 - d->pad;
        P.Ho = d->H; P.Wo = d->W; P.phases = 1;
    } else if (!d->transposed) {
        P.KH = 2; P.KW = 2; P.stride = 1; P.pad_h = P.pad_w = 1;
        P.Ho = Hy; P.Wo = Wy; P.phases = 4;
    } else {
        P.KH = 4; P.KW = 4; P.stride = 2; P.pad_h = P.pad_w = 1;
        P.Ho = d->H; P.Wo = d->W; P.phases = 1;
    }
    P.K = P.KH * P.KW * P.Ci; P.M = P.N * P.Ho * P.Wo;
    {
        const double cir = d->Cir ? d->Cir : d->Ci, cor = d->Cor ? d->Cor : d->Co;
        const double pix_in = (double)d->N * d->H * d->W, pix_out = (double)d->N * Hy * Wy;
        const double macs = d->transposed ? pix_in * 16.0 * cir * cor : pix_out * d->KH * d->KW * cir * cor;
        P.flops = 2.0 * macs;
        P.bytes = 4.0 * (pix_out * cor + pix_in * cir * (1.0 + (mask ? 1.0 : 0.0) + (residual ? 1.0 : 0.0)) +
                         cir * cor * d->KH * d->KW);
    }
    return run_conv_gemm(P, to_stream(stream));
}
```

vq-vae-2-pytorch_amd/csrc/vq2_elem.hip:

```cpp
#include "vq2_common.h"

namespace vq2 {

static inline int grid_for(int64_t work_items, int cap = 4096) {
    int64_t b = (work_items + 255) / 256;
    return (int)(b < 1 ? 1 : (b > cap ? cap : b));
}

__global__ __launch_bounds__(256) void nchw_to_nhwc_kernel(const float *__restrict__ src, float *__restrict__ dst, int C,
                                                           int HW, int ld) {
    __shared__ float tile[32][33];
    const int n = blockIdx.z, p0 = blockIdx.x * 32, c0 = blockIdx.y * 32;
    const int tx = threadIdx.x & 31, ty = threadIdx.x >> 5;
    for (int j = ty; j < 32; j += 8) {
        const int c = c0 + j, p = p0 + tx;
        tile[j][tx] = (c < C && p < HW) ? src[((size_t)n * C + c) * HW + p] : 0.f;
    }
    __syncthreads();
    for (int j = ty; j < 32; j += 8) {
        const int p = p0 + j, c = c0 + tx;
        if (p < HW && c < ld) dst[((size_t)n * HW + p) * ld + c] = tile[tx][j];
    }
}

__global__ __launch_bounds__(256) void nhwc_to_nchw_kernel(const float *__restrict__ src, float *__restrict__ dst, int C,
                                                           int HW, int ld) {
    __shared__ float tile[32][33];
    const int n = blockIdx.z, p0 = blockIdx.x * 32, c0 = blockIdx.y * 32;
    const int tx = threadIdx.x & 31, ty = threadIdx.x >> 5;
    for (int j = ty; j < 32; j += 8) {
        const int p = p0 + j, c = c0 + tx;
        tile[j][tx] = (p < HW && c < C) ? src[((size_t)n * HW + p) * ld + c] : 0.f;
    }
    __syncthreads();
    for (int j = ty; j < 32; j += 8) {
        const int c = c0 + j, p = p0 + tx;
        if (c < C && p < HW) dst[((size_t)n * C + c) * HW + p] = tile[tx][j];
    }
}

__global__ void nchw_to_nhwc4_kernel(const float *__restrict__ src, float4 *__restrict__ dst, int C, int64_t HW,
                                     int64_t total) {
    for (int64_t g = (int64_t)blockIdx.x * blockDim.x + threadIdx.x; g < total; g += (int64_t)gridDim.x * blockDim.x) {
        const int64_t n = g / HW, p = g - n * HW;
        const float *s = src + n * C * HW + p;
        float4 v = make_float4(0.f, 0.f, 0.f, 0.f);
        v.x = s[0];
        if (C > 1) v.y = s[HW];
        if (C > 2) v.z = s[2 * HW];
        if (C > 3) v.w = s[3 * HW];
        dst[g] = v;
    }
}

__global__ void nhwc4_to_nchw_kernel(const float4 *__restrict__ src, float *__restrict__ dst, int C, int64_t HW,
                                     int64_t total) {
    for (int64_t g = (int64_t)blockIdx.x * blockDim.x + threadIdx.x; g < total; g += (int64_t)gridDim.x * blockDim.x) {
        const int64_t n = g / HW, p = g - n * HW;
        const float4 v = src[g];
        float *d = dst + n * C * HW + p;
        d[0] = v.x;
        if (C > 1) d[HW] = v.y;
        if (C > 2) d[2 * HW] = v.z;
        if (C > 3) d[3 * HW] = v.w;
    }
}

__global__ void relu_bwd_kernel(const float *__restrict__ dy, int lddy, const float *__restrict__ y, int ldy,
                                float *__restrict__ g, int ldg, int64_t pixels, int C4) {
    const int64_t total = pixels * C4;
    for (int64_t t = (int64_t)blockIdx.x * blockDim.x + threadIdx.x; t < total; t += (int64_t)gridDim.x * blockDim.x) {
        const int64_t p = t / C4;
        const int c = (int)(t - p * C4) * 4;
        const float4 a = *reinterpret_cast<const float4 *>(dy + p * lddy + c);
        const float4 b = *reinterpret_cast<const float4 *>(y + p * ldy + c);
        float4 o;
        o.x = b.x > 0.f ? a.x : 0.f; o.y = b.y > 0.f ? a.y : 0.f; o.z = b.z > 0.f ? a.z : 0.f; o.w = b.w > 0.f ? a.w : 0.f;
        *reinterpret_cast<float4 *>(g + p * ldg + c) = o;
    }
}

__global__ void slice_copy_kernel(const float *__restrict__ src, int lds_, float *__restrict__ dst, int ldd,
                                  int64_t pixels, int C4, int accumulate) {
    const int64_t total = pixels * C4;
    for (int64_t t = (int64_t)blockIdx.x * blockDim.x + threadIdx.x; t < total; t += (int64_t)gridDim.x * blockDim.x) {
        const int64_t p = t / C4;
        const int c = (int)(t - p * C4) * 4;
        float4 v = *reinterpret_cast<const float4 *>(src + p * lds_ + c);
        float4 *o = reinterpret_cast<float4 *>(dst + p * ldd + c);
        if (accumulate) { const float4 w = *o; v.x += w.x; v.y += w.y; v.z += w.z; v.w += w.w; }
        *o = v;
    }
}

constexpr int MSE_BLOCKS = 1024;

__global__ __launch_bounds__(256) void mse_partial_kernel(const float *__restrict__ a, const float *__restrict__ b,
                                                          int64_t n, float coef, const float *__restrict__ gscale,
                                                          float *__restrict__ grad, float *__restrict__ part) {
    __shared__ float wsum[4];
    const float gs = coef * (gscale ? gscale[0] : 1.f);
    float s = 0.f;
    const int64_t n4 = n / 4;
    for (int64_t i = (int64_t)blockIdx.x * 256 + threadIdx.x; i < n4; i += (int64_t)gridDim.x * 256) {
        const float4 x = reinterpret_cast<const float4 *>(a)[i], y = reinterpret_cast<const float4 *>(b)[i];
        const float d0 = x.x - y.x, d1 = x.y - y.y, d2 = x.z - y.z, d3 = x.w - y.w;
        s += d0 * d0; s += d1 * d1; s += d2 * d2; s += d3 * d3;
        if (grad) reinterpret_cast<float4 *>(grad)[i] = make_float4(gs * d0, gs * d1, gs * d2, gs * d3);
    }
    if (blockIdx.x == 0 && threadIdx.x < (n & 3)) {
        const int64_t i = n4 * 4 + threadIdx.x;
        const float d = a[i] - b[i];
        s += d * d;
        if (grad) grad[i] = gs * d;
    }
    s = wave_sum(s);
    if ((threadIdx.x & 63) == 0) wsum[threadIdx.x >> 6] = s;
    __syncthreads();
    if (threadIdx.x == 0) part[blockIdx.x] = (wsum[0] + wsum[1]) + (wsum[2] + wsum[3]);
}

__global__ void mse_final_kernel(const float *__restrict__ part, int nparts, float denom, float *__restrict__ loss,
                                 const float *__restrict__ latent, float weight, float *__restrict__ total) {
    __shared__ float red[256];
    float s = 0.f;
    for (int i = threadIdx.x; i < nparts; i += 256) s += part[i];
    red[threadIdx.x] = s;
    __syncthreads();
    for (int o = 128; o > 0; o >>= 1) {
        if ((int)threadIdx.x < o) red[threadIdx.x] += red[threadIdx.x + o];
        __syncthreads();
    }
    if (threadIdx.x == 0) {
        const float l = red[0] / denom;
        loss[0] = l;
        if (latent) total[0] = l + weight * latent[0];
    }
}

__global__ void adam_kernel(float *__restrict__ p, const float *__restrict__ g, float *__restrict__ m,
                            float *__restrict__ v, int64_t n, float w1, float b2, float w2, float bc2_sqrt, float eps,
                            float neg_step, float gscale) {
    for (int64_t i = (int64_t)blockIdx.x * blockDim.x + threadIdx.x; i < n; i += (int64_t)gridDim.x * blockDim.x) {
        const float gi = g[i] * gscale;
        float mi = m[i], vi = v[i];
        mi = mi + w1 * (gi - mi);
        vi = vi * b2 + (w2 * gi) * gi;
        const float denom = sqrtf(vi) / bc2_sqrt + eps;
        p[i] = p[i] + neg_step * (mi / denom);
        m[i] = mi;
        v[i] = vi;
    }
}

__global__ void axpby_kernel(const float *__restrict__ a, const float *__restrict__ b, float alpha,
                             float *__restrict__ dst, int64_t n) {
    for (int64_t i = (int64_t)blockIdx.x * blockDim.x + threadIdx.x; i < n; i += (int64_t)gridDim.x * blockDim.x)
        dst[i] = a[i] + alpha * b[i];
}

__global__ void scale_kernel(const float *__restrict__ src, const float *__restrict__ scalar, float alpha,
                             float *__restrict__ dst, int64_t n) {
    const float s = scalar[0] * alpha;
    for (int64_t i = (int64_t)blockIdx.x * blockDim.x + threadIdx.x; i < n; i += (int64_t)gridDim.x * blockDim.x)
        dst[i] = src[i] * s;
}

constexpr int U8_TILE = 1024;

struct U8Params {
    const uint8_t *src; const float *lut; float4 *dst;
    int64_t total;
    int64_t ntiles;
    int C, H, W, Hs, Ws, y0, x0;
};

template <int LAYOUT>
__device__ __forceinline__ int64_t u8_src_offset(const U8Params &P, int64_t grow, int x) {
    const int64_t n = grow / P.H;
    const int y = (int)(grow - n * P.H) + P.y0;
    if (LAYOUT == VQ2_U8_HWC) return ((n * P.Hs + y) * P.Ws + P.x0 + x) * P.C;
    return (n * P.C * P.Hs + y) * P.Ws + P.x0 + x;
}

template <int LAYOUT, bool DWORD>
__global__ __launch_bounds__(256) void u8_to_nhwc4_kernel(const U8Params P) {
    __shared__ float lut[4 * 256];
    __shared__ uint32_t stage[DWORD ? U8_TILE : 1];
    const int t = threadIdx.x, C = P.C;
    for (int i = t; i < C * 256; i += 256) lut[i] = P.lut[i];
    __syncthreads();
    const int64_t plane = (int64_t)P.Hs * P.Ws;
    for (int64_t tile = blockIdx.x; tile < P.ntiles; tile += gridDim.x) {
        const int64_t tile0 = tile * U8_TILE;
        if (DWORD) {
            if (LAYOUT == VQ2_U8_HWC) {
                const uint32_t rowb = (uint32_t)P.W * C;
                const int64_t s0 = tile0 * C, row0 = s0 / rowb;
                const uint32_t off0 = (uint32_t)(s0 - row0 * rowb);
                for (int k = 0; k < C; ++k) {
                    const uint32_t d = t + 256 * k;
                    if (s0 + 4 * (int64_t)d < P.total * C) {
                        const uint32_t u = off0 + 4 * d, r = u / rowb;
                        const int64_t o = u8_src_offset<LAYOUT>(P, row0 + r, 0) + (u - r * rowb);
                        stage[d] = *reinterpret_cast<const uint32_t *>(P.src + o);
                    }
                }
            } else if (tile0 + 4 * t < P.total) {
                const int64_t row0 = tile0 / P.W;
                const uint32_t u = (uint32_t)(tile0 - row0 * P.W) + 4 * t, r = u / (uint32_t)P.W;
                const int64_t o = u8_src_offset<LAYOUT>(P, row0 + r, (int)(u - r * (uint32_t)P.W));
                for (int c = 0; c < C; ++c)
                    stage[c * (U8_TILE / 4) + t] = *reinterpret_cast<const uint32_t *>(P.src + o + c * plane);
            }
            __syncthreads();
        }
        const uint8_t *sb = reinterpret_cast<const uint8_t *>(stage);
#pragma unroll
        for (int j = 0; j < U8_TILE / 256; ++j) {
            const int q = j * 256 + t;
            const int64_t g = tile0 + q;
            if (g >= P.total) break;
            uint32_t b[4] = {0, 0, 0, 0};
            if (DWORD) {
                for (int c = 0; c < C; ++c) b[c] = LAYOUT == VQ2_U8_HWC ? sb[q * C + c] : sb[c * U8_TILE + q];
            } else {
                const int64_t grow = g / P.W;
                const int64_t o = u8_src_offset<LAYOUT>(P, grow, (int)(g - grow * P.W));
                for (int c = 0; c < C; ++c) b[c] = P.src[o + (LAYOUT == VQ2_U8_HWC ? c : c * plane)];
            }
            float4 v = make_float4(0.f, 0.f, 0.f, 0.f);
            v.x = lut[b[0]];
            if (C > 1) v.y = lut[256 + b[1]];
            if (C > 2) v.z = lut[512 + b[2]];
            if (C > 3) v.w = lut[768 + b[3]];
            P.dst[g] = v;
        }
        if (DWORD) __syncthreads();
    }
}

}

using namespace vq2;

static const char NCHW4_LABEL[] = "nchw_to_nhwc4|N=%d,H=%d,W=%d,C=%d";
static const char U8_LABEL[] = "u8_to_nhwc4|N=%d,H=%d,W=%d,C=%d,%s,%s";

extern "C" int vq2_nchw_to_nhwc(const float *src, float *dst, int32_t N, int32_t C, int32_t H, int32_t W, int32_t ld,
                                vq2_stream_t stream) {
    VQ2_REQUIRE(src && dst && N > 0 && C > 0 && H > 0 && W > 0 && ld >= C, "nchw_to_nhwc: bad arguments");
    if (ld == 4 && aligned16(dst)) {
        const int64_t HW4 = (int64_t)H * W, total = HW4 * N;
        ProfScope prof(prof_level() ? prof_label(NCHW4_LABEL, N, H, W, C) : "", 0.0, (double)total * (4 * C + 16),
                       to_stream(stream));
        hipLaunchKernelGGL(nchw_to_nhwc4_kernel, dim3(grid_for(total)), dim3(256), 0, to_stream(stream), src,
                           reinterpret_cast<float4 *>(dst), C, HW4, total);
        return check_launch("nchw_to_nhwc4_kernel");
    }
    VQ2_REQUIRE(N <= 65535, "nchw_to_nhwc: batch > 65535");
    const int HW = H * W;
    dim3 grid((HW + 31) / 32, (ld + 31) / 32, N);
    hipLaunchKernelGGL(nchw_to_nhwc_kernel, grid, dim3(256), 0, to_stream(stream), src, dst, C, HW, ld);
    return check_launch("nchw_to_nhwc_kernel");
}

extern "C" int vq2_u8_to_nhwc4(const uint8_t *src, int layout, int32_t N, int32_t C, int32_t Hs, int32_t Ws, int32_t y0,
                               int32_t x0, int32_t H, int32_t W, const float *lut, float *dst, vq2_stream_t stream) {
    VQ2_REQUIRE(src && lut && dst, "u8_to_nhwc4: null pointer");
    VQ2_REQUIRE(layout == VQ2_U8_HWC || layout == VQ2_U8_CHW, "u8_to_nhwc4: layout %d is neither VQ2_U8_HWC nor VQ2_U8_CHW", layout);
    VQ2_REQUIRE(C >= 1 && C <= 4, "u8_to_nhwc4: %d channels (1..4 fit the 4-float pixel)", C);
    VQ2_REQUIRE(N > 0 && Hs > 0 && Ws > 0 && H > 0 && W > 0, "u8_to_nhwc4: non-positive dimension");
    VQ2_REQUIRE(y0 >= 0 && x0 >= 0 && (int64_t)y0 + H <= Hs && (int64_t)x0 + W <= Ws,
                "u8_to_nhwc4: crop %dx%d at (%d, %d) leaves the %dx%d source", H, W, y0, x0, Hs, Ws);
    VQ2_REQUIRE(aligned16(dst), "u8_to_nhwc4: dst must be 16-byte aligned");
    VQ2_REQUIRE((int64_t)Ws * C < (1 << 30), "u8_to_nhwc4: source rows of 2^30 bytes and more are not supported");
    U8Params P;
    P.src = src; P.lut = lut; P.dst = reinterpret_cast<float4 *>(dst);
    P.total = (int64_t)N * H * W;
    P.ntiles = (P.total + U8_TILE - 1) / U8_TILE;
    P.C = C; P.H = H; P.W = W; P.Hs = Hs; P.Ws = Ws; P.y0 = y0; P.x0 = x0;
    const bool hwc = layout == VQ2_U8_HWC;
    const int unit = hwc ? C : 1;
    const bool dword = (reinterpret_cast<uintptr_t>(src) & 3u) == 0 && ((int64_t)W * unit) % 4 == 0 &&
                       ((int64_t)x0 * unit) % 4 == 0 && ((int64_t)Ws * unit) % 4 == 0;
    hipStream_t s = to_stream(stream);
    ProfScope prof(prof_level() ? prof_label(U8_LABEL, N, H, W, C, hwc ? "hwc" : "chw", dword ? "dword" : "byte") : "",
                   0.0, (double)P.total * (C + 16), s);
    const dim3 grid((unsigned)(P.ntiles < 2048 ? P.ntiles : 2048)), block(256);
    if (hwc && dword) hipLaunchKernelGGL((u8_to_nhwc4_kernel<VQ2_U8_HWC, true>), grid, block, 0, s, P);
    else if (hwc) hipLaunchKernelGGL((u8_to_nhwc4_kernel<VQ2_U8_HWC, false>), grid, block, 0, s, P);
    else if (dword) hipLaunchKernelGGL((u8_to_nhwc4_kernel<VQ2_U8_CHW, true>), grid, block, 0, s, P);
    else hipLaunchKernelGGL((u8_to_nhwc4_kernel<VQ2_U8_CHW, false>), grid, block, 0, s, P);
    return check_launch("u8_to_nhwc4_kernel");
}

extern "C" int vq2_nhwc_to_nchw(const float *src, float *dst, int32_t N, int32_t C, int32_t H, int32_t W, int32_t ld,
                                vq2_stream_t stream) {
    VQ2_REQUIRE(src && dst && N > 0 && C > 0 && H > 0 && W > 0 && ld >= C, "nhwc_to_nchw: bad arguments");
    if (ld == 4 && aligned16(src)) {
        const int64_t HW4 = (int64_t)H * W, total = HW4 * N;
        hipLaunchKernelGGL(nhwc4_to_nchw_kernel, dim3(grid_for(total)), dim3(256), 0, to_stream(stream),
                           reinterpret_cast<const float4 *>(src), dst, C, HW4, total);
        return check_launch("nhwc4_to_nchw_kernel");
    }
    VQ2_REQUIRE(N <= 65535, "nhwc_to_nchw: batch > 65535");
    const int HW = H * W;
    dim3 grid((HW + 31) / 32, (C + 31) / 32, N);
    hipLaunchKernelGGL(nhwc_to_nchw_kernel, grid, dim3(256), 0, to_stream(stream), src, dst, C, HW, ld);
    return check_launch("nhwc_to_nchw_kernel");
}

extern "C" int vq2_relu_bwd(const float *dy, int32_t lddy, const float *y, int32_t ldy, float *g, int32_t ldg,
                            int64_t pixels, int32_t C, vq2_stream_t stream) {
    VQ2_REQUIRE(dy && y && g && pixels > 0 && C > 0 && C % 4 == 0, "relu_bwd: need C %% 4 == 0");
    VQ2_REQUIRE(lddy >= C && ldy >= C && ldg >= C && lddy % 4 == 0 && ldy % 4 == 0 && ldg % 4 == 0,
                "relu_bwd: bad pixel strides");
    VQ2_REQUIRE(aligned16(dy) && aligned16(y) && aligned16(g), "relu_bwd: pointers must be 16-byte aligned");
    hipLaunchKernelGGL(relu_bwd_kernel, dim3(grid_for(pixels * (C / 4))), dim3(256), 0, to_stream(stream), dy, lddy, y,
                       ldy, g, ldg, pixels, C / 4);
    return check_launch("relu_bwd_kernel");
}

extern "C" int vq2_slice_copy(const float *src, int32_t lds_, float *dst, int32_t ldd, int64_t pixels, int32_t C,
                              int accumulate, vq2_stream_t stream) {
    VQ2_REQUIRE(src && dst && pixels > 0 && C > 0 && C % 4 == 0 && lds_ >= C && ldd >= C && lds_ % 4 == 0 && ldd % 4 == 0,
                "slice_copy: bad arguments");
    VQ2_REQUIRE(aligned16(src) && aligned16(dst), "slice_copy: pointers must be 16-byte aligned");
    hipLaunchKernelGGL(slice_copy_kernel, dim3(grid_for(pixels * (C / 4))), dim3(256), 0, to_stream(stream), src, lds_,
                       dst, ldd, pixels, C / 4, accumulate);
    return check_launch("slice_copy_kernel");
}

extern "C" size_t vq2_mse_workspace_bytes(int64_t numel) { return numel > 0 ? MSE_BLOCKS * sizeof(float) : 0; }

static int mse_impl(const float *a, const float *b, int64_t numel, int64_t denom, const float *gscale, float *loss,
                    float *grad, const float *latent, float weight, float *total, void *ws, size_t ws_bytes,
                    vq2_stream_t stream);

extern "C" int vq2_mse_fwd_bwd(const float *a, const float *b, int64_t numel, int64_t denom, const float *gscale,
                               float *loss, float *grad, void *ws, size_t ws_bytes, vq2_stream_t stream) {
    return mse_impl(a, b, numel, denom, gscale, loss, grad, nullptr, 0.f, nullptr, ws, ws_bytes, stream);
}

extern "C" int vq2_stage1_loss(const float *a, const float *b, int64_t numel, int64_t denom, const float *latent,
                               float weight, float *recon, float *total, float *grad, void *ws, size_t ws_bytes,
                               vq2_stream_t stream) {
    VQ2_REQUIRE(latent && total, "stage1_loss: null pointer");
    return mse_impl(a, b, numel, denom, nullptr, recon, grad, latent, weight, total, ws, ws_bytes, stream);
}

static int mse_impl(const float *a, const float *b, int64_t numel, int64_t denom, const float *gscale, float *loss,
                    float *grad, const float *latent, float weight, float *total, void *ws, size_t ws_bytes,
                    vq2_stream_t stream) {
    VQ2_REQUIRE(a && b && loss && ws && numel > 0 && denom > 0, "mse: bad arguments");
    VQ2_REQUIRE(aligned16(a) && aligned16(b) && (!grad || aligned16(grad)), "mse: pointers must be 16-byte aligned");
    VQ2_REQUIRE(ws_bytes >= MSE_BLOCKS * sizeof(float), "mse: workspace too small");
    const int blocks = grid_for(numel / 4 + 1, MSE_BLOCKS);
    hipStream_t s = to_stream(stream);
    hipLaunchKernelGGL(mse_partial_kernel, dim3(blocks), dim3(256), 0, s, a, b, numel, (float)(2.0 / (double)denom),
                       gscale, grad, static_cast<float *>(ws));
    if (int e = check_launch("mse_partial_kernel")) return e;
    hipLaunchKernelGGL(mse_final_kernel, dim3(1), dim3(256), 0, s, static_cast<const float *>(ws), blocks,
                       (float)denom, loss, latent, weight, total);
    return check_launch("mse_final_kernel");
}

extern "C" int vq2_adam_step(float *p, const float *g, float *m, float *v, int64_t n, double lr, double beta1,
                             double beta2, double eps, int32_t step, double grad_scale, vq2_stream_t stream) {
    VQ2_REQUIRE(p && g && m && v && n > 0 && step >= 1, "adam: bad arguments");
    const double bc1 = 1.0 - pow(beta1, (double)step);
    const double bc2 = 1.0 - pow(beta2, (double)step);
    const double step_size = lr / bc1;
    const double bc2_sqrt = sqrt(bc2);
    hipLaunchKernelGGL(adam_kernel, dim3(grid_for(n)), dim3(256), 0, to_stream(stream), p, g, m, v, n,
                       (float)(1.0 - beta1), (float)beta2, (float)(1.0 - beta2), (float)bc2_sqrt, (float)eps,
                       (float)(-step_size), (float)grad_scale);
    return check_launch("adam_kernel");
}

extern "C" int vq2_axpby(const float *a, const float *b, float alpha, float *dst, int64_t n, vq2_stream_t stream) {
    VQ2_REQUIRE(a && b && dst && n > 0, "axpby: bad arguments");
    hipLaunchKernelGGL(axpby_kernel, dim3(grid_for(n)), dim3(256), 0, to_stream(stream), a, b, alpha, dst, n);
    return check_launch("axpby_kernel");
}

extern "C" int vq2_scale(const float *src, const float *scalar, float alpha, float *dst, int64_t n,
                         vq2_stream_t stream) {
    VQ2_REQUIRE(src && scalar && dst && n > 0, "scale: bad arguments");
    hipLaunchKernelGGL(scale_kernel, dim3(grid_for(n)), dim3(256), 0, to_stream(stream), src, scalar, alpha, dst, n);
    return check_launch("scale_kernel");
}

__global__ __launch_bounds__(256) void mfma_peak_kernel(float *out, int iters, float seed) {
    f32x16 acc[4];
#pragma unroll
    for (int i = 0; i < 4; ++i)
#pragma unroll
        for (int r = 0; r < 16; ++r) acc[i][r] = 0.f;
    float a = seed + threadIdx.x * 1e-3f, b = seed - threadIdx.x * 2e-3f;
    for (int it = 0; it < iters; ++it) {
#pragma unroll
        for (int u = 0; u < 8; ++u) {
#pragma unroll
            for (int i = 0; i < 4; ++i) acc[i] = __builtin_amdgcn_mfma_f32_32x32x2f32(a, b, acc[i], 0, 0, 0);
            a += 1e-6f;
        }
    }
    float s = 0.f;
#pragma unroll
    for (int i = 0; i < 4; ++i)
#pragma unroll
        for (int r = 0; r < 16; ++r) s += acc[i][r];
    if (s == 123.456f) out[0] = s;
}

typedef float f32x4v __attribute__((ext_vector_type(4)));
__global__ __launch_bounds__(256) void mfma_peak16_kernel(float *out, int iters, float seed) {
    f32x4v acc[16];
#pragma unroll
    for (int i = 0; i < 16; ++i) acc[i] = f32x4v{0.f, 0.f, 0.f, 0.f};
    float a = seed + threadIdx.x * 1e-3f, b = seed - threadIdx.x * 2e-3f;
    for (int it = 0; it < iters; ++it) {
#pragma unroll
        for (int u = 0; u < 4; ++u) {
#pragma unroll
            for (int i = 0; i < 16; ++i) acc[i] = __builtin_amdgcn_mfma_f32_16x16x4f32(a, b, acc[i], 0, 0, 0);
            a += 1e-6f;
        }
    }
    float s = 0.f;
#pragma unroll
    for (int i = 0; i < 16; ++i) s += acc[i][0] + acc[i][1] + acc[i][2] + acc[i][3];
    if (s == 123.456f) out[0] = s;
}

extern "C" int vq2_debug_mfma_peak16(float *scratch, int32_t blocks, int32_t iters, vq2_stream_t stream) {
    VQ2_REQUIRE(scratch && blocks > 0 && iters > 0, "mfma_peak16: bad arguments");
    hipLaunchKernelGGL(mfma_peak16_kernel, dim3(blocks), dim3(256), 0, to_stream(stream), scratch, iters, 0.5f);
    return check_launch("mfma_peak16_kernel");
}

extern "C" int vq2_debug_mfma_peak(float *scratch, int32_t blocks, int32_t iters, vq2_stream_t stream) {
    VQ2_REQUIRE(scratch && blocks > 0 && iters > 0, "mfma_peak: bad arguments");
    hipLaunchKernelGGL(mfma_peak_kernel, dim3(blocks), dim3(256), 0, to_stream(stream), scratch, iters, 0.5f);
    return check_launch("mfma_peak_kernel");
}
```

vq-vae-2-pytorch_amd/ops.py:

```python
from dataclasses import dataclass
import ctypes as C
import os

import torch
from torch.autograd import Function

from ._lib import lib, check, ConvDesc, PackJob, WgradJob

VQ2_RELU_IN = 1
VQ2_RELU_OUT = 2
VQ2_MASK_AFTER_RESIDUAL = 4
PACK_FWD = 0
PACK_DGRAD = 1



def _stream():
    return C.c_void_p(torch.cuda.current_stream().cuda_stream)


def _p(t):
    return None if t is None else C.c_void_p(t.data_ptr())


def ceil4(c):
    return (c + 3) // 4 * 4


def _require_cuda(t, what):
    if not (isinstance(t, torch.Tensor) and t.is_cuda and t.dtype == torch.float32):
        raise RuntimeError(f"vqvae2_amd: {what} must be a float32 tensor on the MI355X (got "
                           f"{getattr(t, 'dtype', type(t))} on {getattr(t, 'device', '?')}); "
                           "this package has no CPU path")


def is_nhwc_dense(t):
    if t.dim() != 4 or t.stride(3) != 1:
        return False
    n, h, w, c = t.shape
    ld = t.stride(2)
    if w == 1:
        ld = t.stride(1) if h > 1 else (t.stride(0) if n > 1 else c)
    return (ld >= c and ld % 4 == 0 and (w == 1 or t.stride(2) == ld) and (h == 1 or t.stride(1) == w * ld)
            and (n == 1 or t.stride(0) == h * w * ld) and t.data_ptr() % 16 == 0)


def ld_of(t):
    n, h, w, c = t.shape
    if w > 1:
        return t.stride(2)
    if h > 1:
        return t.stride(1)
    if n > 1:
        return t.stride(0)
    return c


def as_nhwc(t):
    _require_cuda(t, "activation")
    if is_nhwc_dense(t):
        return t
    return t.contiguous()


def packed(t):
    if t.is_contiguous():
        return t
    t = as_nhwc(t)
    if t.is_contiguous():
        return t
    n, h, w, c = t.shape
    out = torch.empty((n, h, w, c), device=t.device, dtype=torch.float32)
    check(lib.vq2_slice_copy(_p(t), ld_of(t), _p(out), c, n * h * w, c, 0, _stream()), "slice_copy")
    return out


@dataclass(frozen=True)
class ConvSpec:
    transposed: bool
    cin: int
    cout: int
    k: int
    stride: int
    pad: int

    @property
    def ci(self):
        return ceil4(self.cin)

    @property
    def co(self):
        return ceil4(self.cout)

    def out_hw(self, h, w):
        if self.transposed:
            return 2 * h, 2 * w
        return (h + 2 * self.pad - self.k) // self.stride + 1, (w + 2 * self.pad - self.k) // self.stride + 1


def _desc(spec, n, h, w, ldx, ldy):
    d = ConvDesc()
    d.N, d.H, d.W, d.Ci, d.Co = n, h, w, spec.ci, spec.co
    d.KH = d.KW = spec.k
    d.stride, d.pad, d.transposed = spec.stride, spec.pad, int(spec.transposed)
    d.ldx, d.ldy = ldx, ldy
    d.Cir, d.Cor = spec.cin, spec.cout
    return d


def touch_weights(params):
    for p in params:
        p._vq2_epoch = getattr(p, "_vq2_epoch", 0) + 1


def _pack_version(spec, weight):
    return (weight.data_ptr(), weight._version, getattr(weight, "_vq2_epoch", 0), spec)


def packed_weight(spec, weight, which):
    packs = weight.__dict__.setdefault("_vq2_packs", {})
    ver = _pack_version(spec, weight)
    hit = packs.get(which)
    if hit is not None and hit[0] == ver:
        return hit[1]
    _require_cuda(weight, "weight")
    wsrc = weight.detach()
    if not wsrc.is_contiguous():
        wsrc = wsrc.contiguous()
    n = spec.ci * spec.co * spec.k * spec.k
    buf = hit[1] if (hit is not None and hit[1].numel() == n and hit[1].device == weight.device) else \
        torch.empty(n, device=weight.device, dtype=torch.float32)
    d = _desc(spec, 1, max(spec.k, 2), max(spec.k, 2), spec.ci, spec.co)
    check(lib.vq2_pack_weight(C.byref(d), which, _p(wsrc), _p(buf), _stream()), "pack_weight")
    packs[which] = (ver, buf)
    return buf


class PackPlan:

    def __init__(self, layers):
        import numpy as np
        jobs = []
        for spec, weight, needs_dgrad in layers:
            for which in ((PACK_FWD, PACK_DGRAD) if needs_dgrad else (PACK_FWD,)):
                jobs.append((spec, weight, which))
        n = sum(s.ci * s.co * s.k * s.k for s, _, _ in jobs)
        dev = jobs[0][1].device
        self.flat = torch.empty(n, device=dev, dtype=torch.float32)
        self.entries = []
        arr = (PackJob * len(jobs))()
        off = 0
        for i, (spec, weight, which) in enumerate(jobs):
            numel = spec.ci * spec.co * spec.k * spec.k
            buf = self.flat[off:off + numel]
            d = _desc(spec, 1, max(spec.k, 2), max(spec.k, 2), spec.ci, spec.co)
            if not weight.is_contiguous():
                raise RuntimeError("PackPlan: weights must be contiguous")
            check(lib.vq2_pack_job_init(C.byref(d), which, _p(weight), _p(buf), C.byref(arr[i])), "pack_job_init")
            arr[i].offset = off
            assert arr[i].numel == numel
            self.entries.append((spec, weight, which, buf))
            off += numel
        self.total = off
        raw = np.frombuffer(bytes(arr), dtype=np.uint8).copy()
        self.jobs_dev = torch.from_numpy(raw).to(dev)
        self.njobs = len(jobs)
        self._ptrs = [w.data_ptr() for _, w, _, _ in self.entries]

    def run(self):
        if any(w.data_ptr() != p for (_, w, _, _), p in zip(self.entries, self._ptrs)):
            raise RuntimeError("PackPlan: a parameter was re-allocated; rebuild the plan")
        check(lib.vq2_pack_weights_batched(_p(self.jobs_dev), self.njobs, self.total, _stream()), "pack_batched")
        for spec, weight, which, buf in self.entries:
            weight.__dict__.setdefault("_vq2_packs", {})[which] = (_pack_version(spec, weight), buf)


def conv_forward(spec, x, weight, bias, flags=0, residual=None, out=None):
    n, h, w, c = x.shape
    if c != spec.ci:
        raise RuntimeError(f"conv_forward: input has {c} channels, expected {spec.ci}")
    ho, wo = spec.out_hw(h, w)
    if out is None:
        out = torch.empty((n, ho, wo, spec.co), device=x.device, dtype=torch.float32)
    elif tuple(out.shape) != (n, ho, wo, spec.co) or not is_nhwc_dense(out):
        raise RuntimeError("conv_forward: bad `out` buffer")
    d = _desc(spec, n, h, w, ld_of(x), ld_of(out))
    wp = packed_weight(spec, weight, PACK_FWD)
    ldres = ld_of(residual) if residual is not None else 0
    check(lib.vq2_conv_fwd(C.byref(d), flags, _p(x), _p(wp), _p(bias), _p(residual), ldres, _p(out), _stream()),
          "conv_fwd")
    return out


def conv_dgrad(spec, xshape, dy, weight, mask=None, residual=None, out=None, mask_after=False):
    n, h, w, _ = xshape
    if out is None:
        out = torch.empty((n, h, w, spec.ci), device=dy.device, dtype=torch.float32)
    d = _desc(spec, n, h, w, spec.ci, ld_of(dy))
    wp = packed_weight(spec, weight, PACK_DGRAD)
    check(lib.vq2_conv_dgrad_ex(C.byref(d), VQ2_MASK_AFTER_RESIDUAL if mask_after else 0, _p(dy), _p(wp), _p(mask),
                                ld_of(mask) if mask is not None else 0, _p(residual),
                                ld_of(residual) if residual is not None else 0, _p(out), ld_of(out), _stream()),
          "conv_dgrad")
    return out


def _grad_slot(param):
    slot = getattr(param, "_vq2_grad", None) if param is not None else None
    if slot is not None and param.grad is None:
        return slot.view_as(slot)
    return None if param is None else torch.empty_like(param, memory_format=torch.contiguous_format)


class WgradBatch:

    def __init__(self):
        self.entries = {}
        self.order = []
        self.tables = {}
        self.dirty = True

    def launch(self, spec, x, dy, relu_in, weight, bias, want_db, side):
        n, h, w, _ = x.shape
        key = (id(weight), n, h, w, ld_of(x), ld_of(dy), relu_in)
        d = _desc(spec, n, h, w, ld_of(x), ld_of(dy))
        ent = self.entries.get(key)
        if ent is None:
            nbytes = lib.vq2_conv_wgrad_workspace_bytes(C.byref(d))
            ws = torch.empty(max(nbytes // 4, 4), device=x.device, dtype=torch.float32)
            dw = weight._vq2_grad
            db = bias._vq2_grad if (bias is not None and want_db) else None
            job = WgradJob()
            check(lib.vq2_wgrad_job_init(C.byref(d), _p(ws), _p(dw), _p(db), C.byref(job)), "wgrad_job_init")
            ent = {"ws": ws, "nbytes": nbytes, "job": job, "dw": dw, "db": db, "used": False}
            self.entries[key] = ent
            self.dirty = True
        if n * h * w <= WGRAD_STREAM_MAX_PIXELS:
            side.wait_event(torch.cuda.current_stream().record_event())
            with torch.cuda.stream(side):
                check(lib.vq2_conv_wgrad_partial(C.byref(d), VQ2_RELU_IN if relu_in else 0, _p(x), _p(dy), _p(ent["db"]),
                                                 _p(ent["ws"]), ent["nbytes"], _stream()), "conv_wgrad_partial")
            x.record_stream(side)
            dy.record_stream(side)
        else:
            check(lib.vq2_conv_wgrad_partial(C.byref(d), VQ2_RELU_IN if relu_in else 0, _p(x), _p(dy), _p(ent["db"]),
                                             _p(ent["ws"]), ent["nbytes"], _stream()), "conv_wgrad_partial")
        if not ent["used"]:
            ent["used"] = True
            self.order.append(key)
        dw, db = ent["dw"], ent["db"]
        return dw.view_as(dw), (None if db is None else db.view_as(db))

    def resblock_w2(self, n, h, w, c, cm, weight, bias):
        key = (id(weight), n, h, w, "rbw2")
        ent = self.entries.get(key)
        if ent is None:
            nbytes = lib.vq2_resblock_w2_workspace_bytes(n, h, w, c, cm)
            ws = torch.empty(max(nbytes // 4, 4), device=weight.device, dtype=torch.float32)
            dw, db = weight._vq2_grad, bias._vq2_grad
            job = WgradJob()
            check(lib.vq2_resblock_w2_job_init(n, h, w, c, cm, _p(ws), _p(dw), _p(db), C.byref(job)), "resblock_w2_job_init")
            ent = {"ws": ws, "nbytes": nbytes, "job": job, "dw": dw, "db": db, "used": False}
            self.entries[key] = ent
            self.dirty = True
        if not ent["used"]:
            ent["used"] = True
            self.order.append(key)
        return ent["ws"], ent["dw"].view_as(ent["dw"]), ent["db"].view_as(ent["db"])

    def flush(self):
        if not self.order:
            return
        sig = tuple(self.order)
        if self.dirty:
            self.tables = {}
            self.dirty = False
        tab = self.tables.get(sig)
        if tab is None:
            import numpy as np
            arr = (WgradJob * len(self.order))()
            off = 0
            for i, key in enumerate(self.order):
                job = self.entries[key]["job"]
                job.unit_offset = off
                arr[i] = job
                off += job.n_units_w + job.n_units_b
            raw = np.frombuffer(bytes(arr), dtype=np.uint8).copy()
            tab = (torch.from_numpy(raw).to(self.entries[self.order[0]]["ws"].device), off)
            self.tables[sig] = tab
        check(lib.vq2_wgrad_reduce_batched(_p(tab[0]), len(self.order), tab[1], _stream()), "wgrad_reduce_batched")
        for key in self.order:
            self.entries[key]["used"] = False
        self.order = []


class StepContext:

    def __init__(self, wgrad_stream):
        self.batch = WgradBatch()
        self.stream = wgrad_stream
        self.active = False


def _step_ctx(weight):
    ctx = getattr(weight, "_vq2_ctx", None)
    return ctx if (ctx is not None and ctx.active) else None


WGRAD_STREAM_MAX_PIXELS = 40000


def conv_wgrad(spec, x, dy, relu_in, weight, bias=None, want_dw=True, want_db=True):
    n, h, w, _ = x.shape
    d = _desc(spec, n, h, w, ld_of(x), ld_of(dy))
    nbytes = lib.vq2_conv_wgrad_workspace_bytes(C.byref(d))
    sc = _step_ctx(weight)
    if sc is not None and getattr(weight, "_vq2_grad", None) is not None and weight.grad is None and \
            (bias is None or (getattr(bias, "_vq2_grad", None) is not None and bias.grad is None)) and \
            (bias is None or bias.numel() == spec.cout):
        dw, db = sc.batch.launch(spec, x, dy, relu_in, weight, bias, want_db, sc.stream)
        return (dw if want_dw else None), db
    dw = _grad_slot(weight)
    db = _grad_slot(bias) if (bias is not None and want_db) else None
    if sc is not None and getattr(weight, "_vq2_grad", None) is not None and dw.data_ptr() == weight._vq2_grad.data_ptr():
        side = sc.stream
        side.wait_event(torch.cuda.current_stream().record_event())
        with torch.cuda.stream(side):
            ws = torch.empty(max(nbytes // 4, 4), device=x.device, dtype=torch.float32)
            check(lib.vq2_conv_wgrad(C.byref(d), VQ2_RELU_IN if relu_in else 0, _p(x), _p(dy), _p(dw), _p(db), _p(ws),
                                     nbytes, _stream()), "conv_wgrad")
        x.record_stream(side)
        dy.record_stream(side)
        return (dw if want_dw else None), db
    ws = torch.empty(max(nbytes // 4, 4), device=x.device, dtype=torch.float32)
    check(lib.vq2_conv_wgrad(C.byref(d), VQ2_RELU_IN if relu_in else 0, _p(x), _p(dy), _p(dw), _p(db), _p(ws), nbytes,
                             _stream()), "conv_wgrad")
    return (dw if want_dw else None), db


def relu_bwd(dy, y):
    n, h, w, c = dy.shape
    g = torch.empty((n, h, w, c), device=dy.device, dtype=torch.float32)
    check(lib.vq2_relu_bwd(_p(dy), ld_of(dy), _p(y), ld_of(y), _p(g), c, n * h * w, c, _stream()), "relu_bwd")
    return g


def add_(a, b, alpha=1.0):
    a, b = packed(a), packed(b)
    out = torch.empty_like(a)
    check(lib.vq2_axpby(_p(a), _p(b), float(alpha), _p(out), a.numel(), _stream()), "axpby")
    return out


class NchwToNhwc(Function):

    @staticmethod
    def forward(ctx, x):
        _require_cuda(x, "input")
        n, c, h, w = x.shape
        ctx.c = c
        xc = x if x.is_contiguous() else x.contiguous()
        out = torch.empty((n, h, w, ceil4(c)), device=x.device, dtype=torch.float32)
        check(lib.vq2_nchw_to_nhwc(_p(xc), _p(out), n, c, h, w, ceil4(c), _stream()), "nchw_to_nhwc")
        return out

    @staticmethod
    def backward(ctx, g):
        g = as_nhwc(g)
        n, h, w, cp = g.shape
        out = torch.empty((n, ctx.c, h, w), device=g.device, dtype=torch.float32)
        check(lib.vq2_nhwc_to_nchw(_p(g), _p(out), n, ctx.c, h, w, ld_of(g), _stream()), "nhwc_to_nchw")
        return out


class NhwcToNchw(Function):

    @staticmethod
    def forward(ctx, x, c):
        n, h, w, cp = x.shape
        ctx.cp = cp
        out = torch.empty((n, c, h, w), device=x.device, dtype=torch.float32)
        check(lib.vq2_nhwc_to_nchw(_p(x), _p(out), n, c, h, w, ld_of(x), _stream()), "nhwc_to_nchw")
        return out

    @staticmethod
    def backward(ctx, g):
        n, c, h, w = g.shape
        gc = g if g.is_contiguous() else g.contiguous()
        out = torch.empty((n, h, w, ctx.cp), device=g.device, dtype=torch.float32)
        check(lib.vq2_nchw_to_nhwc(_p(gc), _p(out), n, c, h, w, ctx.cp, _stream()), "nchw_to_nhwc")
        return out, None


def to_nhwc(x):
    _require_cuda(x, "input")
    if x.dim() != 4:
        raise RuntimeError("expected a 4-D NCHW tensor")
    c = x.shape[1]
    if c % 4 == 0:
        v = x.permute(0, 2, 3, 1)
        if is_nhwc_dense(v):
            return v
    return NchwToNhwc.apply(x)


U8_LAYOUTS = {"hwc": 0, "chw": 1}


def u8_to_nhwc4(img, lut, layout, box=None):
    if not (isinstance(img, torch.Tensor) and img.is_cuda and img.dtype == torch.uint8):
        raise RuntimeError(f"vqvae2_amd: 8-bit image batch must be a uint8 tensor on the MI355X (got "
                           f"{getattr(img, 'dtype', type(img))} on {getattr(img, 'device', '?')}); "
                           "this package has no CPU path")
    if layout not in U8_LAYOUTS:
        raise ValueError(f"layout must be 'hwc' or 'chw', not {layout!r}")
    if img.dim() != 4 or not img.is_contiguous():
        raise RuntimeError("expected a contiguous 4-D uint8 batch")
    n, hs, ws, c = img.shape if layout == "hwc" else (img.shape[0], img.shape[2], img.shape[3], img.shape[1])
    _require_cuda(lut, "normalisation table")
    if tuple(lut.shape) != (c, 256) or not lut.is_contiguous() or lut.device != img.device:
        raise RuntimeError(f"normalisation table of shape {tuple(lut.shape)} for a batch of {c} channels")
    y0, x0, h, w = (0, 0, hs, ws) if box is None else box
    out = torch.empty((n, h, w, 4), device=img.device, dtype=torch.float32)
    check(lib.vq2_u8_to_nhwc4(_p(img), U8_LAYOUTS[layout], n, c, hs, ws, y0, x0, h, w, _p(lut), _p(out), _stream()),
          "u8_to_nhwc4")
    return out


def nhwc_to_u8(x, c, inv_s, mean, layout, canvas=None, cols=1, pad=0):
    _require_cuda(x, "activation")
    if layout not in U8_LAYOUTS:
        raise ValueError(f"layout must be 'hwc' or 'chw', not {layout!r}")
    if not is_nhwc_dense(x):
        raise RuntimeError("nhwc_to_u8: expected a dense NHWC tensor")
    n, h, w, cp = x.shape
    if not 1 <= c <= min(cp, 4) or len(inv_s) != c or len(mean) != c:
        raise RuntimeError(f"nhwc_to_u8: {c} channels with {len(inv_s)} / {len(mean)} statistics from a tensor of {cp} lanes")
    hwc = layout == "hwc"
    if canvas is None:
        out = torch.empty((n, h, w, c) if hwc else (n, c, h, w), device=x.device, dtype=torch.uint8)
        hc, wc, cols, pad, image_pitch = h, w, 1, 0, h * w * c
    else:
        out = canvas
        if not (isinstance(out, torch.Tensor) and out.dtype == torch.uint8 and out.device == x.device and out.dim() == 3
                and out.is_contiguous() and out.shape[2 if hwc else 0] == c):
            raise RuntimeError(f"nhwc_to_u8: the canvas must be a contiguous uint8 tensor on {x.device} with {c} channels "
                               f"in layout '{layout}'")
        hc, wc = (out.shape[0], out.shape[1]) if hwc else (out.shape[1], out.shape[2])
        image_pitch = 0
    fa = (C.c_float * c)(*inv_s)
    fm = (C.c_float * c)(*mean)
    check(lib.vq2_nhwc_to_u8(_p(x), ld_of(x), n, c, h, w, fa, fm, _p(out), U8_LAYOUTS[layout], hc, wc,
                             wc * (c if hwc else 1), int(cols), int(pad), image_pitch, _stream()), "nhwc_to_u8")
    return out


def sse_per_image(a, b):
    _require_cuda(a, "reconstruction")
    _require_cuda(b, "target")
    if a.shape != b.shape or not (is_nhwc_dense(a) and is_nhwc_dense(b)) or ld_of(a) != ld_of(b) or ld_of(a) != a.shape[3]:
        raise RuntimeError("sse_per_image: two packed NHWC tensors of one shape expected")
    n, h, w, ld = a.shape
    out = torch.empty(n, device=a.device, dtype=torch.float32)
    nbytes = lib.vq2_sse_workspace_bytes(n, h, w, ld)
    ws = torch.empty(max(nbytes // 4, 1), device=a.device, dtype=torch.float32)
    check(lib.vq2_sse_per_image(_p(a), _p(b), n, h, w, ld, _p(out), _p(ws), nbytes, _stream()), "sse_per_image")
    return out


def index_hist(idx, counts, flag):
    if not (idx.is_cuda and idx.dtype == torch.int64 and counts.dtype == torch.int64 and flag.dtype == torch.int32
            and counts.is_contiguous() and counts.device == idx.device and flag.device == idx.device):
        raise RuntimeError("index_hist: int64 indices and counts and an int32 flag on one GPU expected; no CPU path")
    ic = idx if idx.is_contiguous() else idx.contiguous()
    check(lib.vq2_index_hist(_p(ic), ic.numel(), counts.numel(), _p(counts), _p(flag), _stream()), "index_hist")


def eval_accumulate(sse, elems_per_image, diff, acc):
    if not (acc.dtype == torch.float64 and acc.numel() == 4 and acc.is_contiguous() and acc.is_cuda):
        raise RuntimeError("eval_accumulate: the accumulator is a float64 [4] tensor on the GPU")
    d = diff.detach().reshape(-1)
    if d.numel() != 1 or d.dtype != torch.float32:
        raise RuntimeError("eval_accumulate: the latent loss is one float32 value")
    check(lib.vq2_eval_accumulate(_p(sse), sse.numel(), int(elems_per_image), _p(d), _p(acc), _stream()), "eval_accumulate")


def from_nhwc(y, c):
    if y.shape[3] == c:
        return y.permute(0, 3, 1, 2)
    return NhwcToNchw.apply(y, c)


class ReluFn(Function):

    @staticmethod
    def forward(ctx, x):
        x = as_nhwc(x)
        y = relu_bwd(x, x)
        ctx.save_for_backward(y)
        return y

    @staticmethod
    def backward(ctx, g):
        (y,) = ctx.saved_tensors
        return relu_bwd(as_nhwc(g), y)


class GradStash:

    def __init__(self, strict=False):
        self.tensor = None
        self.closed = False
        self.strict = strict

    def put(self, t):
        if self.closed:
            return False
        self.tensor = t
        return True

    def take(self):
        t, self.tensor, self.closed = self.tensor, None, True
        return t


class ConvFn(Function):

    @staticmethod
    def forward(ctx, x, weight, bias, residual, spec, flags, out, grad_stash=None, mask_input=False, premasked=False):
        ctx.grad_stash, ctx.mask_input, ctx.premasked = grad_stash, mask_input, premasked
        x = as_nhwc(x)
        if residual is not None:
            residual = as_nhwc(residual)
        y = conv_forward(spec, x, weight, bias, flags, residual, out)
        ctx.spec, ctx.flags = spec, flags
        ctx.has_res = residual is not None
        ctx.has_bias = bias is not None
        ctx.save_for_backward(x, weight, y if (flags & VQ2_RELU_OUT) else None, bias)
        if out is not None:
            y = y.view_as(y)
        return y

    @staticmethod
    def backward(ctx, dy):
        x, weight, y, bias = ctx.saved_tensors
        spec, flags = ctx.spec, ctx.flags
        g = as_nhwc(dy)
        if (flags & VQ2_RELU_OUT) and not ctx.premasked:
            g = relu_bwd(g, y)
        relu_in = bool(flags & VQ2_RELU_IN)
        dx = dw = db = dres = None
        if ctx.needs_input_grad[0]:
            other = ctx.grad_stash.take() if ctx.grad_stash is not None else None
            dx = conv_dgrad(spec, x.shape, g, weight, mask=x if (relu_in or ctx.mask_input) else None, residual=other,
                            mask_after=ctx.mask_input)
        if ctx.needs_input_grad[1] or (ctx.has_bias and ctx.needs_input_grad[2]):
            dw, db = conv_wgrad(spec, x, g, relu_in, weight, bias, ctx.needs_input_grad[1],
                                ctx.has_bias and ctx.needs_input_grad[2])
        if ctx.has_res and ctx.needs_input_grad[3]:
            dres = g
        return dx, dw, db, dres, None, None, None, None, None, None


def conv_op(x, weight, bias, spec, relu_in=False, relu_out=False, residual=None, out=None, grad_stash=None,
            mask_input=False, premasked=False):
    flags = (VQ2_RELU_IN if relu_in else 0) | (VQ2_RELU_OUT if relu_out else 0)
    if grad_stash is not None and relu_in and not mask_input:
        grad_stash.closed = True
        grad_stash = None
    return ConvFn.apply(x, weight, bias, residual, spec, flags, out, grad_stash, mask_input, premasked)


_FORMS = os.environ.get("VQ2_FORMS", "all")
if _FORMS not in ("all", "direct", "general"):
    raise ValueError(f"VQ2_FORMS={_FORMS!r}: expected all, direct or general")

RESBLOCK_FUSED = [_FORMS != "general"]


class ResBlockFn(Function):

    @staticmethod
    def forward(ctx, x, w1, b1, w2, b2, spec1, spec2, relu_out, out, premasked=False):
        ctx.premasked = premasked
        x = as_nhwc(x)
        n, h, w, c = x.shape
        if RESBLOCK_FUSED[0] and lib.vq2_resblock_supported(c, spec1.co) and spec1.k == 3 and spec2.k == 1:
            r = torch.empty((n, h, w, spec1.co), device=x.device, dtype=torch.float32)
            y = out if out is not None else torch.empty((n, h, w, c), device=x.device, dtype=torch.float32)
            if tuple(y.shape) != (n, h, w, c) or not is_nhwc_dense(y):
                raise RuntimeError("ResBlock: bad `out` buffer")
            check(lib.vq2_resblock_fwd(n, h, w, c, spec1.co, VQ2_RELU_OUT if relu_out else 0, _p(x), ld_of(x),
                                       _p(packed_weight(spec1, w1, PACK_FWD)), _p(b1),
                                       _p(packed_weight(spec2, w2, PACK_FWD)), _p(b2), _p(r), ld_of(r), _p(y), ld_of(y),
                                       _stream()), "resblock_fwd")
        else:
            r = conv_forward(spec1, x, w1, b1, VQ2_RELU_IN | VQ2_RELU_OUT)
            y = conv_forward(spec2, r, w2, b2, VQ2_RELU_OUT if relu_out else 0, residual=x, out=out)
        ctx.spec1, ctx.spec2, ctx.relu_out = spec1, spec2, relu_out
        ctx.save_for_backward(x, r, w1, w2, y if relu_out else None, b1, b2)
        if out is not None:
            y = y.view_as(y)
        return y

    @staticmethod
    def backward(ctx, dy):
        x, r, w1, w2, y, b1, b2 = ctx.saved_tensors
        s1, s2 = ctx.spec1, ctx.spec2
        g = as_nhwc(dy)
        if ctx.relu_out and not ctx.premasked:
            g = relu_bwd(g, y)
        n, h, w, c = x.shape
        if RESBLOCK_FUSED[0] and ctx.needs_input_grad[0] and lib.vq2_resblock_supported(c, s1.co) and s1.k == 3 and s2.k == 1:
            dh = torch.empty((n, h, w, s1.co), device=x.device, dtype=torch.float32)
            dx = torch.empty((n, h, w, c), device=x.device, dtype=torch.float32)
            sc = _step_ctx(w2)
            w2_ws = None
            if (sc is not None and ctx.needs_input_grad[3] and ctx.needs_input_grad[4] and
                    getattr(w2, "_vq2_grad", None) is not None and getattr(b2, "_vq2_grad", None) is not None and
                    w2.grad is None and b2.grad is None):
                w2_ws, dw2, db2 = sc.batch.resblock_w2(n, h, w, c, s1.co, w2, b2)
            check(lib.vq2_resblock_bwd_data(n, h, w, c, s1.co, _p(g), ld_of(g), _p(r), ld_of(r), _p(x), ld_of(x),
                                            _p(packed_weight(s2, w2, PACK_DGRAD)), _p(packed_weight(s1, w1, PACK_DGRAD)),
                                            _p(dh), ld_of(dh), _p(dx), ld_of(dx), _p(w2_ws), _stream()), "resblock_bwd_data")
            if w2_ws is not None:
                dw1, db1 = conv_wgrad(s1, x, dh, True, w1, b1, ctx.needs_input_grad[1], ctx.needs_input_grad[2])
                return dx, dw1, db1, dw2, db2, None, None, None, None, None
        else:
            dh = conv_dgrad(s2, r.shape, g, w2, mask=r)
            dx = conv_dgrad(s1, x.shape, dh, w1, mask=x, residual=g) if ctx.needs_input_grad[0] else None
        dw2, db2 = conv_wgrad(s2, r, g, False, w2, b2, ctx.needs_input_grad[3], ctx.needs_input_grad[4])
        dw1, db1 = conv_wgrad(s1, x, dh, True, w1, b1, ctx.needs_input_grad[1], ctx.needs_input_grad[2])
        return dx, dw1, db1, dw2, db2, None, None, None, None, None


class CatViewFn(Function):

    @staticmethod
    def forward(ctx, a, b, buf, stash=None):
        ctx.ca = a.shape[3]
        ctx.stash = stash
        return buf.view_as(buf)

    @staticmethod
    def backward(ctx, g):
        g = as_nhwc(g)
        gb = g[..., ctx.ca:]
        if ctx.stash is not None:
            if ctx.stash.put(gb):
                gb = None
            elif ctx.stash.strict:
                raise RuntimeError("GradStash: the consumer that applies b's ReLU mask ran before this gradient arrived")
        return g[..., :ctx.ca], gb, None, None


class CatFn(Function):

    @staticmethod
    def forward(ctx, a, b):
        a, b = as_nhwc(a), as_nhwc(b)
        n, h, w, ca = a.shape
        cb = b.shape[3]
        if tuple(b.shape[:3]) != (n, h, w):
            raise RuntimeError("CatFn: spatial sizes differ")
        out = torch.empty((n, h, w, ca + cb), device=a.device, dtype=torch.float32)
        pix = n * h * w
        check(lib.vq2_slice_copy(_p(a), ld_of(a), _p(out), ca + cb, pix, ca, 0, _stream()), "slice_copy")
        check(lib.vq2_slice_copy(_p(b), ld_of(b), _p(out[..., ca:]), ca + cb, pix, cb, 0, _stream()), "slice_copy")
        ctx.ca = ca
        return out

    @staticmethod
    def backward(ctx, g):
        g = as_nhwc(g)
        return g[..., :ctx.ca], g[..., ctx.ca:]


class AdaINFn(Function):

    @staticmethod
    def forward(ctx, x, h, relu, eps):
        x = as_nhwc(x)
        n, hh, w, c = x.shape
        _require_cuda(h, "AdaIN style projection")
        h2 = h.reshape(n, 2 * c)
        if not h2.is_contiguous():
            h2 = h2.contiguous()
        mean = torch.empty((n, c), device=x.device, dtype=torch.float32)
        rstd = torch.empty((n, c), device=x.device, dtype=torch.float32)
        y = torch.empty((n, hh, w, c), device=x.device, dtype=torch.float32)
        check(lib.vq2_instnorm_stats(_p(x), ld_of(x), n, hh * w, c, float(eps), _p(mean), _p(rstd), _stream()), "instnorm_stats")
        check(lib.vq2_adain_fwd(_p(x), ld_of(x), _p(mean), _p(rstd), _p(h2), n, hh * w, c, VQ2_RELU_OUT if relu else 0,
                                _p(y), c, _stream()), "adain_fwd")
        ctx.save_for_backward(x, mean, rstd, h2, y if relu else None)
        ctx.h_shape = h.shape
        return y

    @staticmethod
    def backward(ctx, dy):
        x, mean, rstd, h2, y = ctx.saved_tensors
        n, hh, w, c = x.shape
        g = as_nhwc(dy)
        dh = torch.empty((n, 2 * c), device=x.device, dtype=torch.float32)
        dx = torch.empty((n, hh, w, c), device=x.device, dtype=torch.float32)
        check(lib.vq2_adain_bwd(_p(g), ld_of(g), _p(y), c, _p(x), ld_of(x), _p(mean), _p(rstd), _p(h2), n, hh * w, c,
                                _p(dh), _p(dx), c, _stream()), "adain_bwd")
        return dx, dh.reshape(ctx.h_shape), None, None


class FanOutFn(Function):

    @staticmethod
    def forward(ctx, x):
        return x.view_as(x), x.view_as(x)

    @staticmethod
    def backward(ctx, g1, g2):
        if g1 is None:
            return g2
        if g2 is None:
            return g1
        return add_(as_nhwc(g1), as_nhwc(g2))


class AddScalarsFn(Function):

    @staticmethod
    def forward(ctx, a, b):
        out = torch.empty(1, device=a.device, dtype=torch.float32)
        check(lib.vq2_axpby(_p(a), _p(b), 1.0, _p(out), 1, _stream()), "axpby")
        return out

    @staticmethod
    def backward(ctx, g):
        return g.reshape(()), g.reshape(())


def vq_prepare(embed):
    d, k = embed.shape
    embed_t = torch.empty((k, d), device=embed.device, dtype=torch.float32)
    enorm = torch.empty(k, device=embed.device, dtype=torch.float32)
    check(lib.vq2_vq_prepare(_p(embed), _p(embed_t), _p(enorm), d, k, _stream()), "vq_prepare")
    return embed_t, enorm


def vq_stats_numel(k, d):
    return (k + 3) // 4 * 4 + k * d


def vq_stats_views(stats, k, d):
    if stats.numel() != vq_stats_numel(k, d) or not stats.is_contiguous():
        raise RuntimeError(f"vq statistics buffer must be contiguous with {vq_stats_numel(k, d)} floats (K={k}, D={d})")
    off = (k + 3) // 4 * 4
    return stats[:k], stats[off:]


def vq_stats_alloc(k, d, device):
    stats = torch.empty(vq_stats_numel(k, d), device=device, dtype=torch.float32)
    if k % 4:
        stats[k:(k + 3) // 4 * 4].zero_()
    return stats


class QuantizeFn(Function):

    @staticmethod
    def forward(ctx, x, embed, want_stats, stats_buf, out_buf, prep=None, stats_stream=None):
        x = as_nhwc(x)
        n, h, w, d = x.shape
        k = embed.shape[1]
        m = n * h * w
        embed_t, enorm = prep if prep is not None else vq_prepare(embed)
        idx = torch.empty((n, h, w), device=x.device, dtype=torch.int64)
        if out_buf is None:
            out = torch.empty((n, h, w, d), device=x.device, dtype=torch.float32)
        else:
            if tuple(out_buf.shape) != (n, h, w, d) or not is_nhwc_dense(out_buf):
                raise RuntimeError("QuantizeFn: bad output buffer")
            out = out_buf.view_as(out_buf)
        part = torch.empty(lib.vq2_vq_fwd_workspace_floats(m, d, k), device=x.device, dtype=torch.float32)
        check(lib.vq2_vq_fwd(_p(x), ld_of(x), _p(embed), _p(embed_t), _p(enorm), m, d, k, _p(idx), _p(out), ld_of(out),
                             _p(part), _stream()), "vq_fwd")
        stats = None
        if want_stats:
            if stats_buf is not None:
                stats = stats_buf.view_as(stats_buf)
            else:
                stats = vq_stats_alloc(k, d, x.device)
            counts, sums_t = vq_stats_views(stats, k, d)
            nbytes = lib.vq2_vq_stats_workspace_bytes(m, d, k)
            ws = torch.empty(nbytes // 4, device=x.device, dtype=torch.int32)
            if stats_stream is not None and stats_buf is not None:
                stats_stream.wait_event(torch.cuda.current_stream().record_event())
                with torch.cuda.stream(stats_stream):
                    check(lib.vq2_vq_stats(_p(x), ld_of(x), _p(idx), m, d, k, _p(counts), _p(sums_t), _p(ws), nbytes,
                                           _stream()), "vq_stats")
                for tns in (x, idx, ws):
                    tns.record_stream(stats_stream)
            else:
                check(lib.vq2_vq_stats(_p(x), ld_of(x), _p(idx), m, d, k, _p(counts), _p(sums_t), _p(ws), nbytes,
                                       _stream()), "vq_stats")
        diff = torch.empty((), device=x.device, dtype=torch.float32)
        check(lib.vq2_vq_loss(_p(part), m, d, _p(diff), _stream()), "vq_loss")
        ctx.save_for_backward(x, idx, embed_t)
        ctx.k = k
        ctx.set_materialize_grads(False)
        ctx.mark_non_differentiable(idx)
        if stats is not None:
            ctx.mark_non_differentiable(stats)
        return out, diff, idx, stats

    @staticmethod
    def backward(ctx, g_out, g_diff, _gi, _gs):
        x, idx, embed_t = ctx.saved_tensors
        n, h, w, d = x.shape
        if g_out is None and g_diff is None:
            return None, None, None, None, None, None, None
        if g_out is not None:
            g_out = as_nhwc(g_out)
        if g_diff is not None and not g_diff.is_contiguous():
            g_diff = g_diff.contiguous()
        dx = torch.empty((n, h, w, d), device=x.device, dtype=torch.float32)
        check(lib.vq2_vq_bwd(_p(g_out), ld_of(g_out) if g_out is not None else d, _p(g_diff), _p(x), ld_of(x),
                             _p(idx), _p(embed_t), n * h * w, d, ctx.k, _p(dx), d, _stream()), "vq_bwd")
        return dx, None, None, None, None, None, None


def vq_ema_update(embed, cluster_size, embed_avg, stats, decay, eps, prep_out=None):
    d, k = embed.shape
    counts, sums_t = vq_stats_views(stats, k, d)
    scratch = torch.empty(4, device=embed.device, dtype=torch.float32)
    if prep_out is not None:
        check(lib.vq2_vq_ema_update_prepare(_p(embed), _p(cluster_size), _p(embed_avg), _p(counts), _p(sums_t), d, k,
                                            float(decay), float(eps), _p(scratch), _p(prep_out[0]), _p(prep_out[1]),
                                            _stream()), "vq_ema_update_prepare")
        return True
    check(lib.vq2_vq_ema_update(_p(embed), _p(cluster_size), _p(embed_avg), _p(counts), _p(sums_t), d, k,
                                float(decay), float(eps), _p(scratch), _stream()), "vq_ema_update")
    return False


def vq_gather(idx, embed, prep=None):
    d, k = embed.shape
    embed_t, _ = prep if prep is not None else vq_prepare(embed)
    idx_c = idx.contiguous()
    m = idx_c.numel()
    out = torch.empty((*idx.shape, d), device=embed.device, dtype=torch.float32)
    check(lib.vq2_vq_gather(_p(idx_c), _p(embed_t), m, d, k, _p(out), d, _stream()), "vq_gather")
    return out


def _scale_by(src, scalar, alpha=1.0):
    out = torch.empty_like(src)
    sc = scalar.reshape(1) if scalar.is_contiguous() else scalar.contiguous().reshape(1)
    check(lib.vq2_scale(_p(src), _p(sc), float(alpha), _p(out), src.numel(), _stream()), "scale")
    return out


class MseLossFn(Function):

    @staticmethod
    def forward(ctx, a, b):
        _require_cuda(a, "mse input")
        ac = a if a.is_contiguous() else a.contiguous()
        bc = b if b.is_contiguous() else b.contiguous()
        n = ac.numel()
        loss = torch.empty((), device=a.device, dtype=torch.float32)
        grad = torch.empty_like(ac) if ctx.needs_input_grad[0] else None
        ws = torch.empty(lib.vq2_mse_workspace_bytes(n) // 4, device=a.device, dtype=torch.float32)
        check(lib.vq2_mse_fwd_bwd(_p(ac), _p(bc), n, n, None, _p(loss), _p(grad), _p(ws), ws.numel() * 4, _stream()),
              "mse_fwd_bwd")
        ctx.save_for_backward(grad)
        return loss

    @staticmethod
    def backward(ctx, g):
        (grad,) = ctx.saved_tensors
        return (None if grad is None else _scale_by(grad, g)), None


def mse_loss(a, b):
    return MseLossFn.apply(a, b)


def stage1_loss_and_seeds(dec, diff, img, weight, denom):
    dc, ic = dec.detach(), img.detach()
    if not (dc.is_contiguous() and ic.is_contiguous()) or diff.numel() != 1:
        raise RuntimeError("stage1_loss_and_seeds: contiguous dec/img and the [1]-shaped latent loss expected")
    n = dc.numel()
    recon = torch.empty((), device=dc.device, dtype=torch.float32)
    loss = torch.empty((), device=dc.device, dtype=torch.float32)
    grad = torch.empty_like(dc)
    latent = diff.detach().reshape(())
    ws = torch.empty(lib.vq2_mse_workspace_bytes(n) // 4, device=dc.device, dtype=torch.float32)
    check(lib.vq2_stage1_loss(_p(dc), _p(ic), n, int(denom), _p(latent), float(weight), _p(recon), _p(loss), _p(grad),
                              _p(ws), ws.numel() * 4, _stream()), "stage1_loss")
    key = (dc.device, float(weight), tuple(diff.shape))
    seed = _DIFF_SEEDS.get(key)
    if seed is None:
        seed = _DIFF_SEEDS[key] = torch.full(tuple(diff.shape), float(weight), device=dc.device, dtype=torch.float32)
    return loss, recon, latent, grad, seed


_DIFF_SEEDS = {}


class Stage1LossFn(Function):

    @staticmethod
    def forward(ctx, dec, diff, img, weight, denom=None):
        _require_cuda(dec, "dec")
        dc = dec if dec.is_contiguous() else dec.contiguous()
        ic = img if img.is_contiguous() else img.contiguous()
        n = dc.numel()
        denom = n if denom is None else int(denom)
        recon = torch.empty((), device=dec.device, dtype=torch.float32)
        grad = torch.empty_like(dc) if ctx.needs_input_grad[0] else None
        ws = torch.empty(lib.vq2_mse_workspace_bytes(n) // 4, device=dec.device, dtype=torch.float32)
        check(lib.vq2_mse_fwd_bwd(_p(dc), _p(ic), n, denom, None, _p(recon), _p(grad), _p(ws), ws.numel() * 4,
                                  _stream()), "mse_fwd_bwd")
        if diff.numel() != 1:
            raise RuntimeError("stage1 loss expects the [1]-shaped latent loss of VQVAE.forward")
        latent = diff.detach().reshape(())
        loss = torch.empty((), device=dec.device, dtype=torch.float32)
        check(lib.vq2_axpby(_p(recon), _p(latent.contiguous()), float(weight), _p(loss), 1, _stream()), "axpby")
        ctx.save_for_backward(grad)
        ctx.weight = weight
        ctx.diff_shape = diff.shape
        ctx.set_materialize_grads(False)
        ctx.mark_non_differentiable(recon, latent)
        return loss, recon, latent

    @staticmethod
    def backward(ctx, g, _gr, _gl):
        (grad,) = ctx.saved_tensors
        if g is None:
            return None, None, None, None, None
        d_dec = None if grad is None else _scale_by(grad, g)
        d_diff = _scale_by(torch.ones(ctx.diff_shape, device=g.device), g, ctx.weight) if ctx.needs_input_grad[1] else None
        return d_dec, d_diff, None, None, None
```

vq-vae-2-pytorch_amd/optim.py:

```python
import ctypes as C
from math import cos, pi

import torch

from . import ops
from ._lib import lib, check


class ParamArena:

    def __init__(self, params, extra=0, last=()):
        params = [p for p in params if p.requires_grad]
        if not params:
            raise ValueError("ParamArena: no parameters")
        self.registration_order = list(params)
        tail_ids = {id(p) for p in last}
        params = [p for p in params if id(p) not in tail_ids] + [p for p in params if id(p) in tail_ids]
        dev = params[0].device
        if dev.type != "cuda":
            raise RuntimeError("ParamArena: parameters must live on the MI355X (model.cuda() first)")
        self.params = params
        sizes = [(p.numel() + 3) // 4 * 4 for p in params]
        self.n = sum(sizes)
        self.flat_p = torch.zeros(self.n, device=dev, dtype=torch.float32)
        self.n_extra = (extra + 3) // 4 * 4
        self.flat_g = torch.zeros(self.n_extra + self.n, device=dev, dtype=torch.float32)
        self.extra = self.flat_g[:extra]
        self.gp = self.flat_g[self.n_extra:]
        self.offset = {}
        off = 0
        with torch.no_grad():
            for p, sz in zip(params, sizes):
                view = self.flat_p[off:off + p.numel()].view(p.shape)
                view.copy_(p.data)
                p.data = view
                p._vq2_grad = self.gp[off:off + p.numel()].view(p.shape)
                self.offset[id(p)] = off
                off += sz
        ops.touch_weights(params)

    def canonical(self, flat):
        return torch.cat([flat[self.offset[id(p)]:self.offset[id(p)] + p.numel()] for p in self.registration_order])

    def from_canonical(self, src, dst):
        off = 0
        for p in self.registration_order:
            dst[self.offset[id(p)]:self.offset[id(p)] + p.numel()].copy_(src[off:off + p.numel()])
            off += p.numel()
        if off != src.numel():
            raise RuntimeError("ParamArena: state vector belongs to a different model")

    def grads_ready(self):
        return all(p.grad is not None and p.grad.data_ptr() == p._vq2_grad.data_ptr() for p in self.params)

    def zero_grad(self):
        for p in self.params:
            p.grad = None


class FusedAdam(torch.optim.Optimizer):

    def __init__(self, params, lr=3e-4, betas=(0.9, 0.999), eps=1e-8, arena=None):
        super().__init__(params, dict(lr=lr, betas=betas, eps=eps))
        self.arena = arena
        self.grad_scale = 1.0
        self._t = 0
        if arena is not None:
            self._m = torch.zeros(arena.n, device=arena.flat_p.device)
            self._v = torch.zeros(arena.n, device=arena.flat_p.device)

    @torch.no_grad()
    def step(self, closure=None):
        s = ops._stream()
        group = self.param_groups[0]
        lr, (b1, b2), eps = group["lr"], group["betas"], group["eps"]
        if self.arena is not None:
            if len(self.param_groups) != 1:
                raise RuntimeError("FusedAdam: a ParamArena supports a single param group")
            if not self.arena.grads_ready():
                missing = [i for i, p in enumerate(self.arena.params)
                           if p.grad is None or p.grad.data_ptr() != p._vq2_grad.data_ptr()]
                raise RuntimeError(f"FusedAdam: {len(missing)} gradient(s) did not land in the flat arena (first: "
                                   f"parameter #{missing[0]}); every arena parameter must receive exactly one "
                                   "gradient per step (zero_grad() before each backward)")
            self._t += 1
            a = self.arena
            check(lib.vq2_adam_step(ops._p(a.flat_p), ops._p(a.gp), ops._p(self._m), ops._p(self._v), a.n,
                                    lr, b1, b2, eps, self._t, self.grad_scale, s), "adam_step")
        else:
            for group in self.param_groups:
                lr, (b1, b2), eps = group["lr"], group["betas"], group["eps"]
                for p in group["params"]:
                    if p.grad is None:
                        continue
                    st = self.state[p]
                    if not st:
                        st["step"] = 0
                        st["exp_avg"] = torch.zeros_like(p, memory_format=torch.contiguous_format)
                        st["exp_avg_sq"] = torch.zeros_like(p, memory_format=torch.contiguous_format)
                    st["step"] += 1
                    g = p.grad if p.grad.is_contiguous() else p.grad.contiguous()
                    check(lib.vq2_adam_step(ops._p(p.data), ops._p(g), ops._p(st["exp_avg"]),
                                            ops._p(st["exp_avg_sq"]), p.numel(), lr, b1, b2, eps, st["step"],
                                            self.grad_scale, s), "adam_step")
        ops.touch_weights(p for g in self.param_groups for p in g["params"])
        return None


_ANNEAL = {
    "linear": lambda start, end, u: start + u * (end - start),
    "cos": lambda start, end, u: end + (start - end) / 2 * (cos(pi * u) + 1),
}


class CycleScheduler:

    def __init__(self, optimizer, lr_max, n_iter, momentum=(0.95, 0.85), divider=25, warmup_proportion=0.3,
                 phase=("linear", "cos")):
        self.optimizer = optimizer
        self.momentum = momentum
        warm = int(n_iter * warmup_proportion)
        self.lengths = (warm, n_iter - warm)
        self.anneal = (_ANNEAL[phase[0]], _ANNEAL[phase[1]])
        lo = lr_max / divider
        self.lr_ends = ((lo, lr_max), (lr_max, lo / 1e4))
        self.mom_ends = None if momentum is None else ((momentum[0], momentum[1]), (momentum[1], momentum[0]))
        self.t = 0

    def values(self, t):
        seg = 0 if t <= self.lengths[0] else 1
        done = t if seg == 0 else t - self.lengths[0]
        if self.lengths[seg] == 0:
            raise ZeroDivisionError("CycleScheduler: a schedule segment has no iterations (n_iter too small)")
        u = done / self.lengths[seg]
        lr = self.anneal[seg](*self.lr_ends[seg], u)
        mom = None
        if self.mom_ends is not None:
            mom = self.anneal[seg](*self.mom_ends[seg], u)
        return lr, mom

    def step(self):
        if self.lengths[0] == 0:
            raise ZeroDivisionError("CycleScheduler: the warm-up segment has no iterations (n_iter too small)")
        self.t += 1
        lr, mom = self.values(self.t)
        for group in self.optimizer.param_groups:
            group["lr"] = lr
            if mom is not None:
                if "betas" in group:
                    group["betas"] = (mom, group["betas"][1])
                else:
                    group["momentum"] = mom
        if self.t >= self.lengths[0] + self.lengths[1]:
            self.t = 0
        return lr, mom

    def state_dict(self):
        return {"t": self.t}

    def load_state_dict(self, sd):
        self.t = int(sd["t"])
```

vq-vae-2-pytorch_amd/train.py:

```python
import os

import torch
from torch import distributed as dist

from . import distributed as dist_fn
from . import ops
from .optim import CycleScheduler, FusedAdam, ParamArena

LATENT_LOSS_WEIGHT = 0.25


def stage1_loss(dec, diff, img, latent_loss_weight=LATENT_LOSS_WEIGHT):
    return ops.Stage1LossFn.apply(dec, diff, img, latent_loss_weight)


class Stage1Trainer:

    def __init__(self, model, lr=3e-4, sched=None, n_iter=None, betas=(0.9, 0.999), eps=1e-8, normalizer=None):
        self.model = model
        self.normalizer = normalizer
        live = model.live_parameters() if hasattr(model, "live_parameters") else list(model.parameters())
        self.quantizers = [m for m in model.modules() if type(m).__name__ == "Quantize"]
        extra = sum(ops.vq_stats_numel(q.n_embed, q.dim) for q in self.quantizers)
        enc_b = getattr(model, "enc_b", None)
        self.arena = ParamArena(live, extra=extra, last=list(enc_b.parameters()) if enc_b is not None else ())
        off = 0
        for q in self.quantizers:
            n = ops.vq_stats_numel(q.n_embed, q.dim)
            q.deferred_stats = self.arena.extra[off:off + n]
            off += n
        self.optimizer = FusedAdam(live, lr=lr, betas=betas, eps=eps, arena=self.arena)
        self.scheduler = None
        if sched == "cycle":
            self.scheduler = CycleScheduler(self.optimizer, lr, n_iter=n_iter, momentum=None, warmup_proportion=0.05)
        if os.environ.get("VQ2_MAIN_PRIO", "1") != "0" and torch.cuda.current_stream().priority == 0:
            hp = torch.cuda.Stream(priority=-1)
            hp.wait_stream(torch.cuda.current_stream())
            torch.cuda.set_stream(hp)
        wgrad_stream = torch.cuda.Stream()
        self.ctx = ops.StepContext(wgrad_stream)
        for p in self.arena.params:
            p._vq2_ctx = self.ctx
        for q in self.quantizers:
            q.stats_stream = wgrad_stream
        layers = []
        for name, mod in model.named_modules():
            if hasattr(mod, "spec") and hasattr(mod, "weight") and not name.startswith("dec_ir"):
                layers.append((mod.spec, mod.weight, name != "enc_b.blocks.0"))
        self.pack_plan = ops.PackPlan(layers)

        self.world = dist_fn.get_world_size()
        forced = os.environ.get("VQ2_DP_FORCE", "0") != "0" and dist.is_available() and dist.is_initialized()
        self.dp = self.world > 1 or forced
        self.optimizer.grad_scale = 1.0 / self.world
        self.comm_stream = torch.cuda.Stream() if self.dp else None
        self.comm = dist_fn.data_comm() if self.dp else None
        if self.dp:
            self._sync_initial_state()
        self.pack_plan.run()
        self.early_buckets = 0
        self.bucket_bytes = {}
        self._sent = []
        self._hooks_seen = {}
        self.buckets = []
        split = getattr(model, "quantize_conv_b", None)
        enc_t = getattr(model, "enc_t", None)
        if split is not None and enc_b is not None and enc_t is not None:
            a = self.arena
            off = lambda p: a.n_extra + a.offset[id(p)]
            lo_tail = off(split.weight)
            lo_head = min(off(p) for p in enc_b.parameters())
            total = a.flat_g.numel()
            inside = lambda lo, hi: [p for p in a.params if lo <= off(p) < hi]
            self.buckets = [("tail", lo_tail, lo_head, inside(lo_tail, lo_head)),
                            ("middle", 0, lo_tail, inside(0, lo_tail)),
                            ("head", lo_head, total, inside(lo_head, total))]
            self.bucket_bytes = {name: 4 * (hi - lo) for name, lo, hi, _ in self.buckets}
            for prm in (split.weight, split.bias):
                prm.register_post_accumulate_grad_hook(lambda _p: self._group_done("tail", 2))
            if self.dp:
                first = enc_t.blocks[0]
                for prm in (first.weight, first.bias):
                    prm.register_post_accumulate_grad_hook(lambda _p: self._group_done("middle", 2))

    def _sync_initial_state(self):
        with torch.no_grad():
            self.comm.broadcast(self.arena.flat_p, 0)
            inside = {id(p) for p in self.arena.params}
            for t in list(self.model.parameters()) + list(self.model.buffers()):
                if id(t) not in inside:
                    self.comm.broadcast(t.detach(), 0)
        ops.touch_weights(self.arena.params)
        for q in self.quantizers:
            q.invalidate_prepared()

    def _group_done(self, name, need):
        seen = self._hooks_seen[name] = self._hooks_seen.get(name, 0) + 1
        if seen != need:
            return
        _, lo, hi, params = next(b for b in self.buckets if b[0] == name)
        if not all(p.grad is not None and p.grad.data_ptr() == p._vq2_grad.data_ptr() for p in params):
            return
        side = self.ctx.stream
        side.wait_event(torch.cuda.current_stream().record_event())
        with torch.cuda.stream(side):
            self.ctx.batch.flush()
            ev = side.record_event()
        if not self.dp:
            return
        with torch.cuda.stream(self.comm_stream):
            self.comm_stream.wait_event(ev)
            self.comm.all_reduce(self.arena.flat_g[lo:hi])
        self._sent.append((lo, hi))
        self.early_buckets += 1

    def _unsent_slices(self):
        out, pos = [], 0
        for lo, hi in sorted(self._sent):
            if lo > pos:
                out.append((pos, lo))
            pos = max(pos, hi)
        if pos < self.arena.flat_g.numel():
            out.append((pos, self.arena.flat_g.numel()))
        return out

    def step(self, img, return_dec=False):
        model = self.model
        u8 = getattr(img, "dtype", None) == torch.uint8
        if u8 and self.normalizer is None:
            raise TypeError("Stage1Trainer.step: a uint8 batch needs Stage1Trainer(..., normalizer=ImageNormalizer(...))")
        model.train()
        self.arena.zero_grad()
        if u8 and hasattr(model, "forward_nhwc"):
            x = self.normalizer(img)
            n, channels, h, w = self.normalizer.out_shape(img)
            dec, diff = model.forward_nhwc(x)
            loss, recon, latent, d_dec, d_diff = ops.stage1_loss_and_seeds(dec, diff, x, LATENT_LOSS_WEIGHT, n * channels * h * w)
            roots, seeds = (dec, diff), (d_dec, d_diff)
        elif hasattr(model, "forward_nhwc"):
            x = ops.to_nhwc(img)
            channels = img.shape[1]
            dec, diff = model.forward_nhwc(x)
            loss, recon, latent, d_dec, d_diff = ops.stage1_loss_and_seeds(dec, diff, x, LATENT_LOSS_WEIGHT, img.numel())
            roots, seeds = (dec, diff), (d_dec, d_diff)
        else:
            if u8:
                img = self.normalizer.nchw(img)
            dec, diff = model(img)
            loss, recon, latent = stage1_loss(dec, diff, img)
            roots, seeds = (loss,), (None,)
        self._sent, self._hooks_seen = [], {}
        self.ctx.active = True
        try:
            torch.autograd.backward(roots, seeds)
        finally:
            self.ctx.active = False
        torch.cuda.current_stream().wait_stream(self.ctx.stream)
        self.ctx.batch.flush()
        if self.dp:
            if not self.arena.grads_ready():
                raise RuntimeError("Stage1Trainer: a gradient did not land in the flat arena")
            ev = torch.cuda.current_stream().record_event()
            with torch.cuda.stream(self.comm_stream):
                self.comm_stream.wait_event(ev)
                for lo, hi in self._unsent_slices():
                    self.comm.all_reduce(self.arena.flat_g[lo:hi])
            torch.cuda.current_stream().wait_stream(self.comm_stream)
        for q in self.quantizers:
            q.apply_deferred_update()
        if self.scheduler is not None:
            self.scheduler.step()
        self.optimizer.step()
        self.pack_plan.run()
        out = {"loss": loss.detach(), "recon": recon, "latent": latent}
        if return_dec:
            d = dec.detach()
            out["dec"] = ops.from_nhwc(d, channels) if hasattr(model, "forward_nhwc") else d
        return out

    def evaluate(self, batches, sample=None):
        from .evaluate import Evaluator
        ev = Evaluator(self.model, self.normalizer)
        for img in batches:
            ev.update(img)
        out = ev.result()
        if sample is not None:
            out["sample"] = self.sample_grid(sample)
        return out

    def sample_grid(self, sample):
        if self.normalizer is None:
            raise TypeError("Stage1Trainer.sample_grid needs Stage1Trainer(..., normalizer=ImageNormalizer(...)): its "
                            "statistics are the ones the grid inverts")
        from .evaluate import eval_mode
        model = self.model
        if not hasattr(model, "forward_nhwc"):
            raise TypeError(f"Stage1Trainer.sample_grid: {type(model).__name__} has no forward_nhwc")
        with torch.no_grad():
            x = self.normalizer(sample) if sample.dtype == torch.uint8 else ops.to_nhwc(sample)
            with eval_mode(model):
                dec, _ = model.forward_nhwc(x)
            return self.normalizer.inverse().grid([x, dec], nrow=x.shape[0], nhwc=True)

    def state_dict(self):
        group = self.optimizer.param_groups[0]
        return {"model": {k: v.detach().clone() for k, v in self.model.state_dict().items()},
                "adam_m": self.arena.canonical(self.optimizer._m), "adam_v": self.arena.canonical(self.optimizer._v),
                "adam_t": self.optimizer._t,
                "lr": group["lr"], "betas": tuple(group["betas"]),
                "scheduler": None if self.scheduler is None else self.scheduler.state_dict()}

    def load_state_dict(self, sd):
        full = "model" in sd and isinstance(sd["model"], dict)
        model_sd = sd["model"] if full else sd
        model_sd = {(k[len("module."):] if k.startswith("module.") else k): v for k, v in model_sd.items()}
        self.model.load_state_dict(model_sd)
        ops.touch_weights(self.arena.params)
        if full:
            n_real = sum(p.numel() for p in self.arena.params)
            if sd["adam_m"].numel() == self.optimizer._m.numel() and sd["adam_m"].numel() != n_real:
                raise RuntimeError("Stage1Trainer.load_state_dict: optimizer state uses the pre-round-3 padded layout; "
                                   "re-save it with that version or resume from the model weights alone")
            if sd["adam_m"].numel() != n_real:
                raise RuntimeError("Stage1Trainer.load_state_dict: optimizer state belongs to a different model")
            dev = self.optimizer._m.device
            self.arena.from_canonical(sd["adam_m"].to(dev), self.optimizer._m)
            self.arena.from_canonical(sd["adam_v"].to(dev), self.optimizer._v)
            self.optimizer._t = int(sd["adam_t"])
            for group in self.optimizer.param_groups:
                group["lr"], group["betas"] = sd["lr"], tuple(sd["betas"])
            if (self.scheduler is None) != (sd.get("scheduler") is None):
                raise RuntimeError("Stage1Trainer.load_state_dict: checkpoint and trainer disagree about --sched")
            if self.scheduler is not None:
                self.scheduler.load_state_dict(sd["scheduler"])
        self.pack_plan.run()
```

Baseline: 5473 images/s.

## Fuse MSE loss into final convT epilogue and weight packing into Adam

Adds a loss epilogue to the final small conv-transpose kernel. It computes the squared error, the gradient and per-block partial sums while writing the output, so a separate MSE pass over the reconstruction is no longer needed. It also adds an Adam variant that scatters each updated weight straight into its forward and dgrad packed panels, using a binary search over a range table. This removes the separate pack_plan.run() after each optimizer step. The trade-offs are extra per-element work in Adam (a table search and scattered stores), more registers in the loss-epilogue kernel, and extra plumbing that must detect when the fused path applies.

```diff
diff --git a/include/vq2.h b/include/vq2.h
--- a/include/vq2.h
+++ b/include/vq2.h
@@ -16,7 +16,7 @@
 
 typedef void *vq2_stream_t;
 
-#define VQ2_API_VERSION 6
+#define VQ2_API_VERSION 7
 
 int vq2_version(void);
 const char *vq2_last_error(void);
@@ -52,6 +52,13 @@
 
 int vq2_conv_fwd(const vq2_conv_desc *d, int flags, const float *x, const float *wp, const float *bias,
                  const float *residual, int32_t ldres, float *y, vq2_stream_t stream);
+
+size_t vq2_conv_fwd_mse_workspace_bytes(const vq2_conv_desc *d);
+int vq2_conv_fwd_mse(const vq2_conv_desc *d, int flags, const float *x, const float *wp, const float *bias, float *y,
+                     const float *target, int64_t denom, const float *gscale, float *grad, void *ws, size_t ws_bytes,
+                     vq2_stream_t stream);
+int vq2_mse_finish(const float *partials, int32_t nparts, int64_t denom, const float *latent, float weight, float *loss,
+                   float *total, vq2_stream_t stream);
 
 int vq2_resblock_supported(int32_t C, int32_t Cm);
 int vq2_resblock_fwd(int32_t N, int32_t H, int32_t W, int32_t C, int32_t Cm, int flags, const float *x, int32_t ldx,
@@ -148,6 +155,17 @@
                     float *recon, float *total, float *grad, void *ws, size_t ws_bytes, vq2_stream_t stream);
 int vq2_adam_step(float *p, const float *g, float *m, float *v, int64_t n, double lr, double beta1, double beta2,
                   double eps, int32_t step, double grad_scale, vq2_stream_t stream);
+typedef struct vq2_adam_pack_range {
+    int64_t begin;
+    int64_t numel;
+    float *fwd;
+    float *dgrad;
+    int32_t Ir, Op, Ip, KH, KW, mode_fwd, mode_dgrad, reserved;
+} vq2_adam_pack_range;
+int vq2_adam_pack_range_init(const vq2_pack_job *fwd, const vq2_pack_job *dgrad, int64_t begin, vq2_adam_pack_range *r);
+int vq2_adam_step_pack(float *p, const float *g, float *m, float *v, int64_t n, double lr, double beta1, double beta2,
+                       double eps, int32_t step, double grad_scale, const vq2_adam_pack_range *ranges_dev,
+                       int32_t nranges, vq2_stream_t stream);
 int vq2_axpby(const float *a, const float *b, float alpha, float *dst, int64_t n, vq2_stream_t stream);
 int vq2_scale(const float *src, const float *scalar, float alpha, float *dst, int64_t n, vq2_stream_t stream);
 
diff --git a/vq-vae-2-pytorch_amd/_lib.py b/vq-vae-2-pytorch_amd/_lib.py
--- a/vq-vae-2-pytorch_amd/_lib.py
+++ b/vq-vae-2-pytorch_amd/_lib.py
@@ -16,6 +16,11 @@
 class PackJob(C.Structure):
     _fields_ = [("w", C.c_void_p), ("packed", C.c_void_p), ("offset", C.c_int64), ("numel", C.c_int64)] + \
                [(n, C.c_int32) for n in ("Or", "Ir", "Op", "Ip", "KH", "KW", "mode", "reserved")]
+
+
+class AdamPackRange(C.Structure):
+    _fields_ = [("begin", C.c_int64), ("numel", C.c_int64), ("fwd", C.c_void_p), ("dgrad", C.c_void_p)] + \
+               [(n, C.c_int32) for n in ("Ir", "Op", "Ip", "KH", "KW", "mode_fwd", "mode_dgrad", "reserved")]
 
 
 class WgradJob(C.Structure):
@@ -42,6 +47,9 @@
         "vq2_pack_job_init": (C.c_int, [DP, C.c_int, P, P, C.POINTER(PackJob)]),
         "vq2_pack_weights_batched": (C.c_int, [P, I32, I64, P]),
         "vq2_conv_fwd": (C.c_int, [DP, C.c_int, P, P, P, P, I32, P, P]),
+        "vq2_conv_fwd_mse_workspace_bytes": (SZ, [DP]),
+        "vq2_conv_fwd_mse": (C.c_int, [DP, C.c_int, P, P, P, P, P, I64, P, P, P, SZ, P]),
+        "vq2_mse_finish": (C.c_int, [P, I32, I64, P, F, P, P, P]),
         "vq2_conv_dgrad": (C.c_int, [DP, P, P, P, I32, P, I32, P, I32, P]),
         "vq2_conv_dgrad_ex": (C.c_int, [DP, C.c_int, P, P, P, I32, P, I32, P, I32, P]),
         "vq2_conv_wgrad_workspace_bytes": (SZ, [DP]),
@@ -84,6 +92,8 @@
         "vq2_mse_fwd_bwd": (C.c_int, [P, P, I64, I64, P, P, P, P, SZ, P]),
         "vq2_stage1_loss": (C.c_int, [P, P, I64, I64, P, F, P, P, P, P, SZ, P]),
         "vq2_adam_step": (C.c_int, [P, P, P, P, I64, D, D, D, D, I32, D, P]),
+        "vq2_adam_pack_range_init": (C.c_int, [C.POINTER(PackJob), C.POINTER(PackJob), I64, C.POINTER(AdamPackRange)]),
+        "vq2_adam_step_pack": (C.c_int, [P, P, P, P, I64, D, D, D, D, I32, D, P, I32, P]),
         "vq2_axpby": (C.c_int, [P, P, F, P, I64, P]),
         "vq2_scale": (C.c_int, [P, P, F, P, I64, P]),
         "vq2_comm_unique_id": (C.c_int, [P]),
diff --git a/vq-vae-2-pytorch_amd/csrc/vq2_conv.hip b/vq-vae-2-pytorch_amd/csrc/vq2_conv.hip
--- a/vq-vae-2-pytorch_amd/csrc/vq2_conv.hip
+++ b/vq-vae-2-pytorch_amd/csrc/vq2_conv.hip
@@ -1121,11 +1121,16 @@
 constexpr int COOB = 0x7F000000;
 }
 
+struct ConvTLoss {
+    const float *target; const float *gscale; float *grad; float *part; float coef;
+};
+
+template <bool LOSS>
 __global__ __launch_bounds__(256, 2) void convT_small_mfma_kernel(const float *__restrict__ x, int ldx,
                                                                   const float *__restrict__ wk,
                                                                   const float *__restrict__ bias, int nbias,
                                                                   float *__restrict__ y, int ldy, int N, int H, int W, int Ci,
-                                                                  int relu_in) {
+                                                                  int relu_in, const ConvTLoss L) {
     using namespace ctm;
     extern __shared__ __attribute__((aligned(16))) float smem[];
     float *Xs = smem;
@@ -1227,6 +1232,27 @@
     const __amdgpu_buffer_rsrc_t ry = __builtin_amdgcn_make_buffer_rsrc(y, 0, N * 4 * H * W * ldy * 4, RSRC_FLAGS);
     const int co = lane & 3;
     const float bvs = (bias && co < nbias) ? bias[co] : 0.f;
+    if (!LOSS) {
+#pragma unroll
+        for (int u = 0; u < 2; ++u)
+#pragma unroll
+            for (int r = 0; r < 4; ++r) {
+                const int pos = (lane & ~3) + r;
+                const int gi = i0 + 4 * wq + 2 * u + (pos >> 5), gj = j0 + (pos & 31);
+                const bool ok = gi < H && gj < W;
+#pragma unroll
+                for (int p = 0; p < 4; ++p) {
+                    const int pix = (n * 2 * H + 2 * gi + (p >> 1)) * (2 * W) + 2 * gj + (p & 1);
+                    __builtin_amdgcn_raw_buffer_store_b32(__float_as_uint(acc[u][p][r] + bvs), ry, ok ? (pix * ldy + co) * 4 : COOB, 0, 0);
+                }
+            }
+        return;
+    }
+    const __amdgpu_buffer_rsrc_t rt = __builtin_amdgcn_make_buffer_rsrc(const_cast<float *>(L.target), 0, N * 4 * H * W * ldy * 4, RSRC_FLAGS);
+    const __amdgpu_buffer_rsrc_t rg = __builtin_amdgcn_make_buffer_rsrc(L.grad, 0, N * 4 * H * W * ldy * 4, RSRC_FLAGS);
+    const float gs = L.coef * (L.gscale ? L.gscale[0] : 1.f);
+    int off[2][4][4];
+    float tv[2][4][4];
 #pragma unroll
     for (int u = 0; u < 2; ++u)
 #pragma unroll
@@ -1237,9 +1263,27 @@
 #pragma unroll
             for (int p = 0; p < 4; ++p) {
                 const int pix = (n * 2 * H + 2 * gi + (p >> 1)) * (2 * W) + 2 * gj + (p & 1);
-                __builtin_amdgcn_raw_buffer_store_b32(__float_as_uint(acc[u][p][r] + bvs), ry, ok ? (pix * ldy + co) * 4 : COOB, 0, 0);
-            }
-        }
+                off[u][r][p] = ok ? (pix * ldy + co) * 4 : COOB;
+                tv[u][r][p] = __uint_as_float(__builtin_amdgcn_raw_buffer_load_b32(rt, off[u][r][p], 0, 0));
+            }
+        }
+    float ssum = 0.f;
+#pragma unroll
+    for (int u = 0; u < 2; ++u)
+#pragma unroll
+        for (int r = 0; r < 4; ++r)
+#pragma unroll
+            for (int p = 0; p < 4; ++p) {
+                const float v = acc[u][p][r] + bvs;
+                const float dlt = off[u][r][p] != COOB ? v - tv[u][r][p] : 0.f;
+                ssum += dlt * dlt;
+                __builtin_amdgcn_raw_buffer_store_b32(__float_as_uint(v), ry, off[u][r][p], 0, 0);
+                __builtin_amdgcn_raw_buffer_store_b32(__float_as_uint(gs * dlt), rg, off[u][r][p], 0, 0);
+            }
+    ssum = wave_sum(ssum);
+    if (lane == 0) smem[wq] = ssum;
+    __syncthreads();
+    if (tid == 0) L.part[blockIdx.x] = (smem[0] + smem[1]) + (smem[2] + smem[3]);
 }
 
 static bool use_convT_small(const vq2_conv_desc *d) {
@@ -1364,8 +1408,41 @@
     return check_launch("pack_single_kernel");
 }
 
+static int conv_fwd_impl(const vq2_conv_desc *d, int flags, const float *x, const float *wp, const float *bias,
+                         const float *residual, int32_t ldres, float *y, const ConvTLoss *loss, vq2_stream_t stream);
+
 extern "C" int vq2_conv_fwd(const vq2_conv_desc *d, int flags, const float *x, const float *wp, const float *bias,
                             const float *residual, int32_t ldres, float *y, vq2_stream_t stream) {
+    return conv_fwd_impl(d, flags, x, wp, bias, residual, ldres, y, nullptr, stream);
+}
+
+static int convT_small_groups(const vq2_conv_desc *d) {
+    return ((d->W + ctm::TW - 1) / ctm::TW) * ((d->H + ctm::TH - 1) / ctm::TH) * d->N;
+}
+
+extern "C" size_t vq2_conv_fwd_mse_workspace_bytes(const vq2_conv_desc *d) {
+    if (check_desc(d) != VQ2_OK || !use_convT_small(d) || d->ldy != 4) return 0;
+    return (size_t)convT_small_groups(d) * sizeof(float);
+}
+
+extern "C" int vq2_conv_fwd_mse(const vq2_conv_desc *d, int flags, const float *x, const float *wp, const float *bias,
+                                float *y, const float *target, int64_t denom, const float *gscale, float *grad, void *ws,
+                                size_t ws_bytes, vq2_stream_t stream) {
+    if (int e = check_desc(d)) return e;
+    if (!use_convT_small(d) || d->ldy != 4)
+        return set_error(VQ2_ERR_UNSUPPORTED, "conv_fwd_mse: only the conv-transpose to <= 3 channels with 4-float pixels "
+                         "(the reconstruction layer) carries the loss epilogue");
+    VQ2_REQUIRE(target && grad && ws && denom > 0, "conv_fwd_mse: bad arguments");
+    VQ2_REQUIRE(aligned16(target) && aligned16(grad), "conv_fwd_mse: pointers must be 16-byte aligned");
+    VQ2_REQUIRE(ws_bytes >= (size_t)convT_small_groups(d) * sizeof(float), "conv_fwd_mse: workspace too small");
+    ConvTLoss L;
+    L.target = target; L.gscale = gscale; L.grad = grad; L.part = static_cast<float *>(ws);
+    L.coef = (float)(2.0 / (double)denom);
+    return conv_fwd_impl(d, flags, x, wp, bias, nullptr, 0, y, &L, stream);
+}
+
+static int conv_fwd_impl(const vq2_conv_desc *d, int flags, const float *x, const float *wp, const float *bias,
+                         const float *residual, int32_t ldres, float *y, const ConvTLoss *loss, vq2_stream_t stream) {
     if (int e = check_desc(d)) return e;
     VQ2_REQUIRE(x && wp && y, "conv_fwd: null pointer");
     VQ2_REQUIRE(aligned16(x) && aligned16(wp) && aligned16(y), "conv_fwd: pointers must be 16-byte aligned");
@@ -1383,10 +1460,16 @@
         if (prof_enabled()) name = prof_label("convT_small|N=%d,H=%d,W=%d,Ci=%d", d->N, d->H, d->W, d->Ci);
         ProfScope prof(name, 2.0 * d->N * d->H * d->W * 16.0 * d->Ci * cor,
                        4.0 * ((double)d->N * d->H * d->W * d->Ci + 4.0 * d->N * d->H * d->W * cor), s);
-        const int g = ((d->W + ctm::TW - 1) / ctm::TW) * ((d->H + ctm::TH - 1) / ctm::TH) * d->N;
-        allow_big_lds(convT_small_mfma_kernel, ctm::LDS_BYTES);
-        hipLaunchKernelGGL(convT_small_mfma_kernel, dim3(g), dim3(256), ctm::LDS_BYTES, s, x, d->ldx, wp, bias, cor, y,
-                           d->ldy, d->N, d->H, d->W, d->Ci, (flags & VQ2_RELU_IN) != 0);
+        const int g = convT_small_groups(d);
+        if (loss) {
+            allow_big_lds(convT_small_mfma_kernel<true>, ctm::LDS_BYTES);
+            hipLaunchKernelGGL(convT_small_mfma_kernel<true>, dim3(g), dim3(256), ctm::LDS_BYTES, s, x, d->ldx, wp, bias, cor,
+                               y, d->ldy, d->N, d->H, d->W, d->Ci, (flags & VQ2_RELU_IN) != 0, *loss);
+        } else {
+            allow_big_lds(convT_small_mfma_kernel<false>, ctm::LDS_BYTES);
+            hipLaunchKernelGGL(convT_small_mfma_kernel<false>, dim3(g), dim3(256), ctm::LDS_BYTES, s, x, d->ldx, wp, bias, cor,
+                               y, d->ldy, d->N, d->H, d->W, d->Ci, (flags & VQ2_RELU_IN) != 0, ConvTLoss{});
+        }
         return check_launch("convT_small_mfma_kernel");
     }
     ConvGemmParams P{};
diff --git a/vq-vae-2-pytorch_amd/csrc/vq2_elem.hip b/vq-vae-2-pytorch_amd/csrc/vq2_elem.hip
--- a/vq-vae-2-pytorch_amd/csrc/vq2_elem.hip
+++ b/vq-vae-2-pytorch_amd/csrc/vq2_elem.hip
@@ -138,18 +138,57 @@
     }
 }
 
+__device__ __forceinline__ float adam_elem(float *__restrict__ p, const float *__restrict__ g, float *__restrict__ m,
+                                           float *__restrict__ v, int64_t i, float w1, float b2, float w2,
+                                           float bc2_sqrt, float eps, float neg_step, float gscale) {
+    const float gi = g[i] * gscale;
+    float mi = m[i], vi = v[i];
+    mi = mi + w1 * (gi - mi);
+    vi = vi * b2 + (w2 * gi) * gi;
+    const float denom = sqrtf(vi) / bc2_sqrt + eps;
+    const float pn = p[i] + neg_step * (mi / denom);
+    p[i] = pn;
+    m[i] = mi;
+    v[i] = vi;
+    return pn;
+}
+
 __global__ void adam_kernel(float *__restrict__ p, const float *__restrict__ g, float *__restrict__ m,
                             float *__restrict__ v, int64_t n, float w1, float b2, float w2, float bc2_sqrt, float eps,
                             float neg_step, float gscale) {
+    for (int64_t i = (int64_t)blockIdx.x * blockDim.x + threadIdx.x; i < n; i += (int64_t)gridDim.x * blockDim.x)
+        adam_elem(p, g, m, v, i, w1, b2, w2, bc2_sqrt, eps, neg_step, gscale);
+}
+
+__device__ __forceinline__ int pack_pos(int mode, int o, int i, int kh, int kw, int Op, int Ip, int KH, int KW) {
+    if (mode == 0) return (o * (KH * KW) + kh * KW + kw) * Ip + i;
+    if (mode == 1) return (i * (KH * KW) + (KH - 1 - kh) * KW + (KW - 1 - kw)) * Op + o;
+    if (mode == 2) {
+        const int rh = 3 - kh, rw = 3 - kw;
+        return (((((rh & 1) * 2 + (rw & 1)) * Ip + i) * 4) + (rh >> 1) * 2 + (rw >> 1)) * Op + o;
+    }
+    return ((kh * 4 + kw) * 4 + i) * Op + o;
+}
+
+__global__ void adam_pack_kernel(float *__restrict__ p, const float *__restrict__ g, float *__restrict__ m,
+                                 float *__restrict__ v, int64_t n, float w1, float b2, float w2, float bc2_sqrt, float eps,
+                                 float neg_step, float gscale, const vq2_adam_pack_range *__restrict__ tab, int nranges) {
     for (int64_t i = (int64_t)blockIdx.x * blockDim.x + threadIdx.x; i < n; i += (int64_t)gridDim.x * blockDim.x) {
-        const float gi = g[i] * gscale;
-        float mi = m[i], vi = v[i];
-        mi = mi + w1 * (gi - mi);
-        vi = vi * b2 + (w2 * gi) * gi;
-        const float denom = sqrtf(vi) / bc2_sqrt + eps;
-        p[i] = p[i] + neg_step * (mi / denom);
-        m[i] = mi;
-        v[i] = vi;
+        const float pn = adam_elem(p, g, m, v, i, w1, b2, w2, bc2_sqrt, eps, neg_step, gscale);
+        int lo = 0, hi = nranges - 1;
+        while (lo < hi) {
+            const int mid = (lo + hi + 1) >> 1;
+            if (tab[mid].begin <= i) lo = mid; else hi = mid - 1;
+        }
+        const int64_t t64 = i - tab[lo].begin;
+        if (t64 < 0 || t64 >= tab[lo].numel) continue;
+        const vq2_adam_pack_range r = tab[lo];
+        const unsigned t = (unsigned)t64, taps = (unsigned)(r.KH * r.KW);
+        const unsigned oi = t / taps, tap = t - oi * taps;
+        const int o = (int)(oi / (unsigned)r.Ir), ii = (int)(oi - (unsigned)o * (unsigned)r.Ir);
+        const int kh = (int)(tap / (unsigned)r.KW), kw = (int)(tap - (unsigned)kh * (unsigned)r.KW);
+        if (r.fwd) r.fwd[pack_pos(r.mode_fwd, o, ii, kh, kw, r.Op, r.Ip, r.KH, r.KW)] = pn;
+        if (r.dgrad) r.dgrad[pack_pos(r.mode_dgrad, o, ii, kh, kw, r.Op, r.Ip, r.KH, r.KW)] = pn;
     }
 }
 
@@ -379,6 +418,51 @@
     return check_launch("adam_kernel");
 }
 
+extern "C" int vq2_adam_pack_range_init(const vq2_pack_job *fwd, const vq2_pack_job *dgrad, int64_t begin,
+                                       vq2_adam_pack_range *r) {
+    VQ2_REQUIRE(r && (fwd || dgrad) && begin >= 0, "adam_pack_range_init: bad arguments");
+    const vq2_pack_job *j = fwd ? fwd : dgrad;
+    if (fwd && dgrad)
+        VQ2_REQUIRE(fwd->Or == dgrad->Or && fwd->Ir == dgrad->Ir && fwd->Op == dgrad->Op && fwd->Ip == dgrad->Ip &&
+                    fwd->KH == dgrad->KH && fwd->KW == dgrad->KW && fwd->w == dgrad->w,
+                    "adam_pack_range_init: the two jobs describe different layers");
+    VQ2_REQUIRE(j->Or > 0 && j->Ir > 0 && j->Or <= j->Op && j->Ir <= j->Ip && j->KH > 0 && j->KW > 0 &&
+                j->numel == (int64_t)j->Op * j->Ip * j->KH * j->KW && j->numel < ((int64_t)1 << 31),
+                "adam_pack_range_init: not a job of vq2_pack_job_init");
+    r->begin = begin;
+    r->numel = (int64_t)j->Or * j->Ir * j->KH * j->KW;
+    r->fwd = fwd ? fwd->packed : nullptr;
+    r->dgrad = dgrad ? dgrad->packed : nullptr;
+    r->Ir = j->Ir; r->Op = j->Op; r->Ip = j->Ip; r->KH = j->KH; r->KW = j->KW;
+    r->mode_fwd = fwd ? fwd->mode : 0;
+    r->mode_dgrad = dgrad ? dgrad->mode : 0;
+    r->reserved = 0;
+    return VQ2_OK;
+}
+
+extern "C" int vq2_adam_step_pack(float *p, const float *g, float *m, float *v, int64_t n, double lr, double beta1,
+                                  double beta2, double eps, int32_t step, double grad_scale,
+                                  const vq2_adam_pack_range *ranges_dev, int32_t nranges, vq2_stream_t stream) {
+    VQ2_REQUIRE(p && g && m && v && n > 0 && step >= 1, "adam: bad arguments");
+    VQ2_REQUIRE(ranges_dev && nranges > 0, "adam_step_pack: empty table (vq2_adam_step is the plain update)");
+    const double bc1 = 1.0 - pow(beta1, (double)step);
+    const double bc2 = 1.0 - pow(beta2, (double)step);
+    const double step_size = lr / bc1;
+    const double bc2_sqrt = sqrt(bc2);
+    hipLaunchKernelGGL(adam_pack_kernel, dim3(grid_for(n)), dim3(256), 0, to_stream(stream), p, g, m, v, n,
+                       (float)(1.0 - beta1), (float)beta2, (float)(1.0 - beta2), (float)bc2_sqrt, (float)eps,
+                       (float)(-step_size), (float)grad_scale, ranges_dev, nranges);
+    return check_launch("adam_pack_kernel");
+}
+
+extern "C" int vq2_mse_finish(const float *partials, int32_t nparts, int64_t denom, const float *latent, float weight,
+                              float *loss, float *total, vq2_stream_t stream) {
+    VQ2_REQUIRE(partials && loss && nparts > 0 && denom > 0 && (!latent || total), "mse_finish: bad arguments");
+    hipLaunchKernelGGL(mse_final_kernel, dim3(1), dim3(256), 0, to_stream(stream), partials, nparts, (float)denom, loss,
+                       latent, weight, total);
+    return check_launch("mse_final_kernel");
+}
+
 extern "C" int vq2_axpby(const float *a, const float *b, float alpha, float *dst, int64_t n, vq2_stream_t stream) {
     VQ2_REQUIRE(a && b && dst && n > 0, "axpby: bad arguments");
     hipLaunchKernelGGL(axpby_kernel, dim3(grid_for(n)), dim3(256), 0, to_stream(stream), a, b, alpha, dst, n);
diff --git a/vq-vae-2-pytorch_amd/ops.py b/vq-vae-2-pytorch_amd/ops.py
--- a/vq-vae-2-pytorch_amd/ops.py
+++ b/vq-vae-2-pytorch_amd/ops.py
@@ -162,15 +162,19 @@
             self.entries.append((spec, weight, which, buf))
             off += numel
         self.total = off
+        self.jobs_host = arr
         raw = np.frombuffer(bytes(arr), dtype=np.uint8).copy()
         self.jobs_dev = torch.from_numpy(raw).to(dev)
         self.njobs = len(jobs)
         self._ptrs = [w.data_ptr() for _, w, _, _ in self.entries]
 
     def run(self):
+        check(lib.vq2_pack_weights_batched(_p(self.jobs_dev), self.njobs, self.total, _stream()), "pack_batched")
+        self.mark_fresh()
+
+    def mark_fresh(self):
         if any(w.data_ptr() != p for (_, w, _, _), p in zip(self.entries, self._ptrs)):
             raise RuntimeError("PackPlan: a parameter was re-allocated; rebuild the plan")
-        check(lib.vq2_pack_weights_batched(_p(self.jobs_dev), self.njobs, self.total, _stream()), "pack_batched")
         for spec, weight, which, buf in self.entries:
             weight.__dict__.setdefault("_vq2_packs", {})[which] = (_pack_version(spec, weight), buf)
 
@@ -187,9 +191,42 @@
     d = _desc(spec, n, h, w, ld_of(x), ld_of(out))
     wp = packed_weight(spec, weight, PACK_FWD)
     ldres = ld_of(residual) if residual is not None else 0
+    req = _RECON_LOSS[0]
+    if req is not None and req.grad is None and residual is None and tuple(out.shape) == tuple(req.target.shape) \
+            and out.is_contiguous():
+        nbytes = lib.vq2_conv_fwd_mse_workspace_bytes(C.byref(d))
+        if nbytes:
+            req.grad = torch.empty_like(out)
+            req.ws = torch.empty(nbytes // 4, device=out.device, dtype=torch.float32)
+            check(lib.vq2_conv_fwd_mse(C.byref(d), flags, _p(x), _p(wp), _p(bias), _p(out), _p(req.target), req.denom, None,
+                                       _p(req.grad), _p(req.ws), nbytes, _stream()), "conv_fwd_mse")
+            req.out_ptr = out.data_ptr()
+            return out
     check(lib.vq2_conv_fwd(C.byref(d), flags, _p(x), _p(wp), _p(bias), _p(residual), ldres, _p(out), _stream()),
           "conv_fwd")
     return out
+
+
+_RECON_LOSS = [None]
+
+
+class ReconLoss:
+
+    def __init__(self, target, denom):
+        if not target.is_contiguous():
+            raise RuntimeError("ReconLoss: contiguous NHWC target expected")
+        self.target, self.denom = target.detach(), int(denom)
+        self.grad = self.ws = self.out_ptr = None
+
+    def __enter__(self):
+        if _RECON_LOSS[0] is not None:
+            raise RuntimeError("ReconLoss: requests do not nest")
+        _RECON_LOSS[0] = self
+        return self
+
+    def __exit__(self, *exc):
+        _RECON_LOSS[0] = None
+        return False
 
 
 def conv_dgrad(spec, xshape, dy, weight, mask=None, residual=None, out=None, mask_after=False):
@@ -883,18 +920,24 @@
     return MseLossFn.apply(a, b)
 
 
-def stage1_loss_and_seeds(dec, diff, img, weight, denom):
+def stage1_loss_and_seeds(dec, diff, img, weight, denom, fused=None):
     dc, ic = dec.detach(), img.detach()
     if not (dc.is_contiguous() and ic.is_contiguous()) or diff.numel() != 1:
         raise RuntimeError("stage1_loss_and_seeds: contiguous dec/img and the [1]-shaped latent loss expected")
     n = dc.numel()
     recon = torch.empty((), device=dc.device, dtype=torch.float32)
     loss = torch.empty((), device=dc.device, dtype=torch.float32)
-    grad = torch.empty_like(dc)
     latent = diff.detach().reshape(())
-    ws = torch.empty(lib.vq2_mse_workspace_bytes(n) // 4, device=dc.device, dtype=torch.float32)
-    check(lib.vq2_stage1_loss(_p(dc), _p(ic), n, int(denom), _p(latent), float(weight), _p(recon), _p(loss), _p(grad),
-                              _p(ws), ws.numel() * 4, _stream()), "stage1_loss")
+    if fused is not None and fused.grad is not None and fused.out_ptr == dc.data_ptr() and fused.denom == int(denom) \
+            and fused.target.data_ptr() == ic.data_ptr():
+        grad = fused.grad
+        check(lib.vq2_mse_finish(_p(fused.ws), fused.ws.numel(), int(denom), _p(latent), float(weight), _p(recon), _p(loss),
+                                 _stream()), "mse_finish")
+    else:
+        grad = torch.empty_like(dc)
+        ws = torch.empty(lib.vq2_mse_workspace_bytes(n) // 4, device=dc.device, dtype=torch.float32)
+        check(lib.vq2_stage1_loss(_p(dc), _p(ic), n, int(denom), _p(latent), float(weight), _p(recon), _p(loss), _p(grad),
+                                  _p(ws), ws.numel() * 4, _stream()), "stage1_loss")
     key = (dc.device, float(weight), tuple(diff.shape))
     seed = _DIFF_SEEDS.get(key)
     if seed is None:
diff --git a/vq-vae-2-pytorch_amd/optim.py b/vq-vae-2-pytorch_amd/optim.py
--- a/vq-vae-2-pytorch_amd/optim.py
+++ b/vq-vae-2-pytorch_amd/optim.py
@@ -4,7 +4,48 @@
 import torch
 
 from . import ops
-from ._lib import lib, check
+from ._lib import lib, check, AdamPackRange
+
+
+def pack_position(mode, o, i, kh, kw, Op, Ip, KH, KW):
+    taps = KH * KW
+    if mode == 0:
+        return (o * taps + kh * KW + kw) * Ip + i
+    if mode == 1:
+        return (i * taps + (KH - 1 - kh) * KW + (KW - 1 - kw)) * Op + o
+    if mode == 2:
+        rh, rw = 3 - kh, 3 - kw
+        return ((((rh & 1) * 2 + (rw & 1)) * Ip + i) * 4 + (rh >> 1) * 2 + (rw >> 1)) * Op + o
+    if mode == 3:
+        return ((kh * 4 + kw) * 4 + i) * Op + o
+    raise ValueError(f"pack_position: unknown mode {mode}")
+
+
+def range_positions(r, t):
+    if not 0 <= t < r.numel:
+        raise IndexError(t)
+    taps = r.KH * r.KW
+    oi, tap = divmod(t, taps)
+    o, i = divmod(oi, r.Ir)
+    kh, kw = divmod(tap, r.KW)
+    pos = lambda mode: pack_position(mode, o, i, kh, kw, r.Op, r.Ip, r.KH, r.KW)
+    return (pos(r.mode_fwd) if r.fwd else None, pos(r.mode_dgrad) if r.dgrad else None)
+
+
+def pack_ranges(layers):
+    rows = sorted(layers, key=lambda e: e[0])
+    arr = (AdamPackRange * len(rows))()
+    end = 0
+    for k, (begin, numel, fwd, dgrad) in enumerate(rows):
+        check(lib.vq2_adam_pack_range_init(C.byref(fwd) if fwd is not None else None,
+                                           C.byref(dgrad) if dgrad is not None else None, begin, C.byref(arr[k])),
+              "adam_pack_range_init")
+        if arr[k].numel != numel:
+            raise RuntimeError(f"pack_ranges: the pack jobs describe {arr[k].numel} weights, the tensor has {numel}")
+        if begin < end:
+            raise RuntimeError("pack_ranges: overlapping arena ranges")
+        end = begin + numel
+    return arr
 
 
 class ParamArena:
@@ -68,6 +109,26 @@
         if arena is not None:
             self._m = torch.zeros(arena.n, device=arena.flat_p.device)
             self._v = torch.zeros(arena.n, device=arena.flat_p.device)
+        self._pack_plan = self._pack_table = None
+
+    def attach_pack_plan(self, plan):
+        if self.arena is None:
+            raise RuntimeError("FusedAdam.attach_pack_plan needs a ParamArena")
+        import numpy as np
+        jobs = {}
+        for (spec, weight, which, _buf), job in zip(plan.entries, plan.jobs_host):
+            if id(weight) in self.arena.offset:
+                slot = jobs.setdefault(id(weight), [weight, None, None])
+                if slot[1 + (which == ops.PACK_DGRAD)] is not None:
+                    raise RuntimeError("FusedAdam.attach_pack_plan: a weight with two panels of one kind (shared by two "
+                                       "layers) has one table range only")
+                slot[1 + (which == ops.PACK_DGRAD)] = job
+        if not jobs:
+            raise RuntimeError("FusedAdam.attach_pack_plan: no weight of the plan lives in the arena")
+        table = pack_ranges([(self.arena.offset[k], w.numel(), f, dg) for k, (w, f, dg) in jobs.items()])
+        self._pack_table = torch.from_numpy(np.frombuffer(bytes(table), dtype=np.uint8).copy()).to(self.arena.flat_p.device)
+        self._pack_ranges = len(table)
+        self._pack_plan = plan
 
     @torch.no_grad()
     def step(self, closure=None):
@@ -85,8 +146,13 @@
                                    "gradient per step (zero_grad() before each backward)")
             self._t += 1
             a = self.arena
-            check(lib.vq2_adam_step(ops._p(a.flat_p), ops._p(a.gp), ops._p(self._m), ops._p(self._v), a.n,
-                                    lr, b1, b2, eps, self._t, self.grad_scale, s), "adam_step")
+            if self._pack_table is not None:
+                check(lib.vq2_adam_step_pack(ops._p(a.flat_p), ops._p(a.gp), ops._p(self._m), ops._p(self._v), a.n,
+                                             lr, b1, b2, eps, self._t, self.grad_scale, ops._p(self._pack_table),
+                                             self._pack_ranges, s), "adam_step_pack")
+            else:
+                check(lib.vq2_adam_step(ops._p(a.flat_p), ops._p(a.gp), ops._p(self._m), ops._p(self._v), a.n,
+                                        lr, b1, b2, eps, self._t, self.grad_scale, s), "adam_step")
         else:
             for group in self.param_groups:
                 lr, (b1, b2), eps = group["lr"], group["betas"], group["eps"]
@@ -104,6 +170,8 @@
                                             ops._p(st["exp_avg_sq"]), p.numel(), lr, b1, b2, eps, st["step"],
                                             self.grad_scale, s), "adam_step")
         ops.touch_weights(p for g in self.param_groups for p in g["params"])
+        if self._pack_table is not None:
+            self._pack_plan.mark_fresh()
         return None
 
 
diff --git a/vq-vae-2-pytorch_amd/train.py b/vq-vae-2-pytorch_amd/train.py
--- a/vq-vae-2-pytorch_amd/train.py
+++ b/vq-vae-2-pytorch_amd/train.py
@@ -48,6 +48,7 @@
             if hasattr(mod, "spec") and hasattr(mod, "weight") and not name.startswith("dec_ir"):
                 layers.append((mod.spec, mod.weight, name != "enc_b.blocks.0"))
         self.pack_plan = ops.PackPlan(layers)
+        self.optimizer.attach_pack_plan(self.pack_plan)
 
         self.world = dist_fn.get_world_size()
         forced = os.environ.get("VQ2_DP_FORCE", "0") != "0" and dist.is_available() and dist.is_initialized()
@@ -134,14 +135,18 @@
         if u8 and hasattr(model, "forward_nhwc"):
             x = self.normalizer(img)
             n, channels, h, w = self.normalizer.out_shape(img)
-            dec, diff = model.forward_nhwc(x)
-            loss, recon, latent, d_dec, d_diff = ops.stage1_loss_and_seeds(dec, diff, x, LATENT_LOSS_WEIGHT, n * channels * h * w)
+            with ops.ReconLoss(x, n * channels * h * w) as req:
+                dec, diff = model.forward_nhwc(x)
+            loss, recon, latent, d_dec, d_diff = ops.stage1_loss_and_seeds(dec, diff, x, LATENT_LOSS_WEIGHT,
+                                                                           n * channels * h * w, fused=req)
             roots, seeds = (dec, diff), (d_dec, d_diff)
         elif hasattr(model, "forward_nhwc"):
             x = ops.to_nhwc(img)
             channels = img.shape[1]
-            dec, diff = model.forward_nhwc(x)
-            loss, recon, latent, d_dec, d_diff = ops.stage1_loss_and_seeds(dec, diff, x, LATENT_LOSS_WEIGHT, img.numel())
+            with ops.ReconLoss(x, img.numel()) as req:
+                dec, diff = model.forward_nhwc(x)
+            loss, recon, latent, d_dec, d_diff = ops.stage1_loss_and_seeds(dec, diff, x, LATENT_LOSS_WEIGHT, img.numel(),
+                                                                           fused=req)
             roots, seeds = (dec, diff), (d_dec, d_diff)
         else:
             if u8:
@@ -171,7 +176,6 @@
         if self.scheduler is not None:
             self.scheduler.step()
         self.optimizer.step()
-        self.pack_plan.run()
         out = {"loss": loss.detach(), "recon": recon, "latent": latent}
         if return_dec:
             d = dec.detach()
```

Result: no change. 5467 images/s (-0.1%).
